# modelscope/FunASR

Hardware: AMD Instinct MI355X
Metric: audio-seconds/sec (RTF^-1) Paraformer-large 30s@bs64 (higher is better)
Workload: dtype f32 (GEMM / self-attention operands split into 2 fp16 planes, 3 fp16 MFMA products, f32 accumulate; all else f32)

## Files before the change

funasr_amd/_lib.py:

```python
from __future__ import annotations

import ctypes as C
import os
import subprocess
import threading

_HERE = os.path.dirname(os.path.abspath(__file__))
LIB_PATH = os.environ.get("PF_LIB_PATH") or os.path.join(_HERE, "libparaformer_hip.so")
CSRC_DIR = os.path.join(_HERE, "csrc")

ABI_VERSION = 5

_lock = threading.Lock()
_lib = None


class HipRuntimeError(RuntimeError):
    """A pf_* entry point returned a non-zero status."""


class pf_frontend_config(C.Structure):
    _fields_ = [
        ("sample_rate", C.c_int32), ("frame_length", C.c_int32), ("frame_shift", C.c_int32),
        ("n_mels", C.c_int32), ("lfr_m", C.c_int32), ("lfr_n", C.c_int32),
# ... 44 lines not shown
               [(n, C.c_double) for n in ("speech_2_noise_ratio", "snr_thres", "decibel_thres", "speech_noise_thres",
                                           "fe_prior_thres")]


class pf_campplus_config(C.Structure):
    _fields_ = [(n, C.c_int32) for n in ("feat_dim", "embedding_size", "growth_rate", "bn_size", "init_channels", "m_channels")] + \
               [("bn_eps", C.c_float)]


class pf_emotion2vec_config(C.Structure):
    _fields_ = [(n, C.c_int32) for n in ("embed_dim", "num_heads", "ffn_dim", "prenet_depth", "depth", "num_extra_tokens",
                                          "num_alibi_heads", "alibi_scale_layers", "alibi_scale_heads", "n_conv")] + \
               [("conv_kernel", C.c_int32 * 8), ("conv_stride", C.c_int32 * 8)] + \
               [(n, C.c_int32) for n in ("conv_pos_depth", "conv_pos_kernel", "conv_pos_groups", "vocab_size", "normalize", "precision")] + \
               [("norm_eps", C.c_float)]


class pf_conformer_config(C.Structure):
    _fields_ = [(n, C.c_int32) for n in ("input_dim", "d_model", "n_heads", "ffn_dim", "n_blocks", "kernel_size", "macaron", "legacy",
                                          "precision")] + [("ln_eps", C.c_float)]


class pf_tdecoder_config(C.Structure):
    _fields_ = [(n, C.c_int32) for n in ("vocab_size", "d_model", "n_heads", "ffn_dim", "n_blocks")] + [("ln_eps", C.c_float)]


class pf_stream_config(C.Structure):
    _fields_ = [(n, C.c_int32) for n in ("n_streams", "chunk_left", "chunk_cur", "chunk_right", "enc_look_back",
                                          "dec_look_back", "max_frames", "max_tokens", "use_graph")]


_vp, _i32, _i64, _f32 = C.c_void_p, C.c_int32, C.c_int64, C.c_float
_pi32 = C.POINTER(C.c_int32)

SIGNATURES = {
    "pf_last_error": (C.c_char_p, []),
    "pf_abi_version": (C.c_int, []),
    "pf_device_count": (C.c_int, []),
    "pf_set_concurrency_guard": (C.c_int, [_i32]),
    "pf_concurrency_guard": (C.c_int, []),
    "pf_frontend_create": (_vp, [C.POINTER(pf_frontend_config)]),
    "pf_frontend_destroy": (None, [_vp]),
    "pf_frontend_set_cmvn": (C.c_int, [_vp, _vp, _vp, _i32]),
    "pf_frontend_set_dither": (C.c_int, [_vp, _f32, C.c_uint64]),
    "pf_frontend_set_verify": (C.c_int, [_vp, _i32]),
    "pf_frontend_faults": (C.c_int, [_vp, C.POINTER(C.c_uint32)]),
    "pf_frontend_fault_log": (C.c_int, [_vp, C.POINTER(C.c_uint32)]),
    "pf_frontend_set_tables": (C.c_int, [_vp, _vp, _vp]),
    "pf_utterance_mvn": (C.c_int, [_vp, _vp, _i32, _i32, _i32, _i32, _i32, _f32, _vp]),
    "pf_global_mvn": (C.c_int, [_vp, _vp, _i32, _i32, _i32, _vp, _vp, _i32, _i32, _vp]),
    "pf_frontend_set_window": (C.c_int, [_vp, C.c_char_p, _f32]),
    "pf_frontend_set_snip_edges": (C.c_int, [_vp, _i32]),
    "pf_frontend_num_fbank_frames": (_i32, [_vp, _i64]),
    "pf_frontend_num_frames": (_i32, [_vp, _i64]),
    "pf_frontend_forward": (C.c_int, [_vp, _vp, _i64, _pi32, _i32, _vp, _i32, _pi32, _vp, _vp]),
    "pf_encoder_create": (_vp, [C.POINTER(pf_encoder_config)]),
    "pf_encoder_destroy": (None, [_vp]),
    "pf_encoder_set_tensor": (C.c_int, [_vp, C.c_char_p, _vp, _i64]),
    "pf_encoder_missing": (C.c_int, [_vp]),
    "pf_encoder_set_precision": (C.c_int, [_vp, _i32]),
    "pf_encoder_set_row_packing": (C.c_int, [_vp, _i32]),
    "pf_encoder_set_option": (C.c_int, [_vp, C.c_char_p, _i32]),
    "pf_encoder_debug_poison": (C.c_int, [_vp, _i32]),
    "pf_decoder_debug_poison": (C.c_int, [_vp, _i32]),
    "pf_predictor_debug_poison": (C.c_int, [_vp, _i32]),
    "pf_encoder_set_vad_mask": (C.c_int, [_vp, _vp, _i32]),
    "pf_encoder_forward": (C.c_int, [_vp, _vp, _pi32, _i32, _i32, _vp, _vp, _i32, _vp]),
    "pf_predictor_create": (_vp, [C.POINTER(pf_predictor_config)]),
    "pf_predictor_destroy": (None, [_vp]),
    "pf_predictor_set_tensor": (C.c_int, [_vp, C.c_char_p, _vp, _i64]),
    "pf_predictor_missing": (C.c_int, [_vp]),
    "pf_predictor_alphas": (C.c_int, [_vp, _vp, _pi32, _i32, _i32, _vp, _vp, _pi32, _vp]),
    "pf_predictor_embeds": (C.c_int, [_vp, _vp, _i32, _i32, _i32, _vp, _vp]),
    "pf_predictor_alphas_begin": (C.c_int, [_vp, _i32, _vp, _pi32, _i32, _i32, _vp, _vp, _vp, _vp]),
    "pf_predictor_embeds_slot": (C.c_int, [_vp, _i32, _vp, _i32, _i32, _i32, _vp, _vp]),
    "pf_predictor_create_v3": (_vp, [C.POINTER(pf_predictor_config), C.POINTER(pf_predictor_v3_config)]),
    "pf_predictor_timestamp": (C.c_int, [_vp, _vp, _pi32, _pi32, _i32, _i32, _vp, _vp, _vp]),
    "pf_decoder_create": (_vp, [C.POINTER(pf_decoder_config)]),
    "pf_decoder_destroy": (None, [_vp]),
    "pf_decoder_set_decoders2": (C.c_int, [_vp, _i32]),
    "pf_decoder_set_tensor": (C.c_int, [_vp, C.c_char_p, _vp, _i64]),
    "pf_decoder_missing": (C.c_int, [_vp]),
    "pf_decoder_set_precision": (C.c_int, [_vp, _i32]),
    "pf_decoder_forward": (C.c_int, [_vp, _vp, _pi32, _vp, _pi32, _i32, _i32, _i32, _vp, _vp, _vp, _vp]),
    "pf_decoder_create_contextual": (_vp, [C.POINTER(pf_decoder_config)]),
    "pf_decoder_forward_contextual": (C.c_int, [_vp, _vp, _pi32, _vp, _pi32, _vp, _i32, _f32, _i32, _i32, _i32, _vp, _vp, _vp, _vp]),
    "pf_decoder_asf_scores": (C.c_int, [_vp, _vp, _pi32, _vp, _pi32, _i32, _i32, _i32, _i32, _vp, _vp]),
    "pf_vad_create": (_vp, [C.POINTER(pf_vad_config)]),
    "pf_vad_destroy": (None, [_vp]),
    "pf_vad_set_tensor": (C.c_int, [_vp, C.c_char_p, _vp, _i64]),
    "pf_vad_missing": (C.c_int, [_vp]),
    "pf_vad_forward": (C.c_int, [_vp, _vp, _i32, _i32, _vp, _pi32, _i32, _vp, _vp, _i32, _vp]),
    "pf_vad_frame_decibel": (C.c_int, [_vp, _i64, _i32, _i32, _i32, _vp, _vp]),
    "pf_vad_decision_create": (_vp, [C.POINTER(pf_vad_options)]),
    "pf_vad_decision_destroy": (None, [_vp]),
    "pf_vad_decision_set_thresholds": (None, [_vp, C.c_double, C.c_double]),
    "pf_vad_decision_state": (C.c_int, [_vp]),
    "pf_vad_decision_push": (C.c_int, [_vp, _vp, _vp, _i32, _i32, _i32, _vp, _i32]),
    "pf_campplus_create": (_vp, [C.POINTER(pf_campplus_config)]),
    "pf_campplus_destroy": (None, [_vp]),
    "pf_campplus_set_tensor": (C.c_int, [_vp, C.c_char_p, _vp, _i64]),
    "pf_campplus_missing": (C.c_int, [_vp]),
    "pf_campplus_set_max_batch": (C.c_int, [_vp, _i32]),
    "pf_campplus_forward": (C.c_int, [_vp, _vp, _i32, _i32, _vp, _vp]),
    "pf_campplus_embed_chunks": (C.c_int, [_vp, _vp, _i64, C.POINTER(C.c_int64), _pi32, _i32, _i32, _vp, _vp]),
    "pf_emotion2vec_create": (_vp, [C.POINTER(pf_emotion2vec_config)]),
    "pf_emotion2vec_destroy": (None, [_vp]),
    "pf_emotion2vec_set_tensor": (C.c_int, [_vp, C.c_char_p, _vp, _i64]),
    "pf_emotion2vec_missing": (C.c_int, [_vp]),
    "pf_emotion2vec_set_label_mask": (C.c_int, [_vp, _pi32, _i32]),
    "pf_emotion2vec_set_max_samples": (C.c_int, [_vp, _i64]),
    "pf_emotion2vec_num_frames": (_i32, [_vp, _i64]),
    "pf_emotion2vec_forward": (C.c_int, [_vp, _vp, C.POINTER(C.c_int64), _i32, _vp, _vp, _vp, _vp]),
    "pf_conformer_create": (_vp, [C.POINTER(pf_conformer_config)]),
    "pf_conformer_destroy": (None, [_vp]),
    "pf_conformer_set_tensor": (C.c_int, [_vp, C.c_char_p, _vp, _i64]),
    "pf_conformer_missing": (C.c_int, [_vp]),
    "pf_conformer_set_precision": (C.c_int, [_vp, _i32]),
    "pf_conformer_num_frames": (_i32, [_vp, _i32, _i32]),
    "pf_conformer_forward": (C.c_int, [_vp, _vp, _pi32, _i32, _i32, _vp, _pi32, _vp]),
    "pf_tdecoder_create": (_vp, [C.POINTER(pf_tdecoder_config)]),
    "pf_tdecoder_destroy": (None, [_vp]),
    "pf_tdecoder_set_tensor": (C.c_int, [_vp, C.c_char_p, _vp, _i64]),
    "pf_tdecoder_missing": (C.c_int, [_vp]),
    "pf_tdecoder_begin": (C.c_int, [_vp, _vp, _i32, _i32, _i32, _vp]),
    "pf_tdecoder_step": (C.c_int, [_vp, _pi32, _i32, _i32, _vp, _vp]),
    "pf_tdecoder_reorder": (C.c_int, [_vp, _pi32, _i32, _vp]),
    "pf_k_relpos_attention": (C.c_int, [_vp, _vp, _vp, _vp, _vp, _i32, _i32, _i32, _i32, _vp, _vp]),
    "pf_k_conformer_glu_dw": (C.c_int, [_vp, _vp, _vp, _vp, _vp, _i32, _i32, _i32, _i32, _vp, _vp]),
    "pf_ctc_create": (_vp, [_i32, _i32]),
    "pf_ctc_destroy": (None, [_vp]),
    "pf_ctc_set_tensor": (C.c_int, [_vp, C.c_char_p, _vp, _i64]),
    "pf_ctc_missing": (C.c_int, [_vp]),
    "pf_ctc_greedy": (C.c_int, [_vp, _vp, _i32, _vp, _vp, _vp]),
    "pf_ctc_set_precision": (C.c_int, [_vp, _i32]),
    "pf_posterior_embed_create": (_vp, [_i32, _i32, _i32]),
    "pf_posterior_embed_destroy": (None, [_vp]),
    "pf_posterior_embed_set_tensor": (C.c_int, [_vp, C.c_char_p, _vp, _i64]),
    "pf_posterior_embed_missing": (C.c_int, [_vp]),
    "pf_posterior_embed_set_precision": (C.c_int, [_vp, _i32]),
    "pf_posterior_embed_set_chunk_rows": (C.c_int, [_vp, _i32]),
    "pf_posterior_embed_debug_poison": (C.c_int, [_vp, _i32]),
    "pf_posterior_embed_runs": (C.c_int, [_vp, _vp, _vp, _pi32, _i32, _i32, _pi32, _vp, _vp]),
    "pf_posterior_embed_embeds": (C.c_int, [_vp, _i32, _i32, _i32, _vp, _vp, _vp]),
    "pf_stream_create": (_vp, [_vp, _vp, _vp, C.POINTER(pf_stream_config)]),
    "pf_stream_destroy": (None, [_vp]),
    "pf_stream_set_pe": (C.c_int, [_vp, _vp, _i32]),
    "pf_stream_reset": (C.c_int, [_vp, _vp]),
    "pf_stream_set_option": (C.c_int, [_vp, C.c_char_p, _i32]),
    "pf_stream_step": (C.c_int, [_vp, _vp, _i32, _i32, _i32, _pi32, _pi32, _vp, _vp]),
    "pf_stream_step_begin": (C.c_int, [_vp, _vp, _i32, _i32, _i32, _vp, _vp]),
    "pf_stream_step_end": (C.c_int, [_vp, _pi32, _pi32]),
    "pf_stream_peek": (C.c_int, [_vp, _vp, _vp, _pi32]),
    "pf_frontend_fbank": (C.c_int, [_vp, _vp, _i64, _vp, _vp]),
    "pf_frontend_lfr_cmvn": (C.c_int, [_vp, _vp, _i32, _i32, _vp, _vp]),
    "pf_set_skinny_max_m": (C.c_int, [_i32]),
    "pf_measurement_build": (C.c_int, []),
    "pf_k_conv1d_gemm_f32": (C.c_int, [_vp, _vp, _vp, _vp, _i32, _i32, _i32, _i32, _i32, _i32, _i32, _vp, _vp]),
    "pf_k_gemm_f32": (C.c_int, [_vp, _i32, _vp, _i32, _vp, _vp, _i32, _vp, _i32, _vp, _i32, _i32, _i32, _i32, _i32, _vp]),
    "pf_k_gemm_bf16": (C.c_int, [_vp, _i32, _vp, _i32, _vp, _vp, _i32, _vp, _i32, _vp, _i32, _i32, _i32, _i32, _i32, _i32, _vp]),
    "pf_k_gemm_bf16_time": (C.c_int, [_vp, _i32, _vp, _i32, _vp, _vp, _i32, _i32, _i32, _i32, _i32, _i32, C.POINTER(C.c_float), _vp]),
    "pf_k_cast_bf16": (C.c_int, [_vp, _vp, _i64, _vp]),
    "pf_k_split3": (C.c_int, [_vp, _i32, _vp, _i32, _i64, _i32, _i32, _vp]),
    "pf_k_gemm_split3": (C.c_int, [_vp, _i32, _i64, _vp, _i32, _i64, _vp, _vp, _i32, _vp, _i32, _vp, _i32, _vp, _i32, _i64,
                                   _i32, _i32, _i32, _i32, _i32, C.POINTER(C.c_float), _vp]),
    "pf_k_split2": (C.c_int, [_vp, _i32, _vp, _i32, _i64, _i32, _i32, _f32, _vp]),
    "pf_k_gemm_f16x2": (C.c_int, [_vp, _i32, _i64, _vp, _i32, _i64, _f32, _vp, _vp, _i32, _vp, _i32, _vp, _i32, _vp, _i32, _i64,
                                  _f32, _i32, _i32, _i32, _i32, _i32, _i32, C.POINTER(C.c_float), _vp]),
    "pf_k_attention_f16x2": (C.c_int, [_vp, _i64, _vp, _i64, _vp, _i32, _i64, _vp, _i64, _vp, _i32, _i32, _i32, _i32, _f32, _f32,
                                       _i32, _i32, C.POINTER(C.c_float), _vp]),
    "pf_k_gemm_f16x2_row": (C.c_int, [_vp, _i32, _i64, _vp, _i32, _i64, _f32, _vp, _vp, _i32, _vp, _i32, _vp, _i32, _vp, _vp, _f32,
                                      _vp, _i64, _f32, _vp, _i32, _i32, _i32, _i32, _i32, C.POINTER(C.c_float), _vp]),
    "pf_k_gemm_skinny_ln": (C.c_int, [_vp, _i32, _vp, _i32, _vp, _vp, _i32, _vp, _i32, _i32, _i32, _i32, _i32, _vp, _vp, _vp, _vp, _f32, _vp, _vp, _vp, _vp]),
    "pf_k_ln_consts": (C.c_int, [_vp, _i32, _i32, _i32, _vp, _vp, _vp, _vp, _vp]),
    "pf_k_ffn_f16x2": (C.c_int, [_vp, _vp, _vp, _vp, _vp, _f32, _f32, _f32, _vp, _vp, _vp, _vp, _f32, _vp, _f32, _vp, _i32, _i32, _i32,
                                 C.POINTER(C.c_float), _vp]),
    "pf_k_gemm_f16x2_row_fsmn": (C.c_int, [_vp, _i32, _i64, _vp, _i32, _i64, _f32, _vp, _vp, _i32, _vp, _vp, _vp, _vp, _i32, _vp, _i32,
                                           _vp, _vp, _f32, _vp, _i64, _f32, _vp, _i32, _i32, _i32, _i32, C.POINTER(C.c_float), _vp]),
    "pf_k_layernorm_planes": (C.c_int, [_vp, _i32, _vp, _vp, _vp, _i32, _i64, _f32, _i32, _i32, _f32, _i32, C.POINTER(C.c_float), _vp]),
    "pf_k_gemm_f16x2_qkv": (C.c_int, [_vp, _i32, _i64, _vp, _i32, _i64, _f32, _vp, _i32, _i32, _i32, _i32, _vp, _vp, _i64, _vp, _vp,
                                      _i32, _i64, _f32, _f32, _f32, _i32, _i32, C.POINTER(C.c_float), _vp]),
    "pf_k_gemm_f16x2_argmax": (C.c_int, [_vp, _i32, _i64, _vp, _i32, _i64, _f32, _vp, _i32, _i32, _i32, _vp, _vp, _vp, _vp]),
    "pf_k_gemm_argmax_f32": (C.c_int, [_vp, _i32, _vp, _i32, _vp, _i32, _i32, _i32, _vp, _vp, _vp, _vp]),
    "pf_k_log_softmax": (C.c_int, [_vp, _i32, _vp, _i32, _i32, _i32, _vp]),
    "pf_k_layernorm": (C.c_int, [_vp, _i32, _vp, _vp, _vp, _i32, _i32, _i32, _i32, _f32, _vp]),
    "pf_k_fsmn": (C.c_int, [_vp, _i32, _vp, _vp, _i32, _vp, _i32, _vp, _i32, _i32, _i32, _i32, _i32, _vp]),
    "pf_k_attention_f32": (C.c_int, [_vp, _i32, _vp, _i32, _vp, _i32, _vp, _i32, _vp, _i32, _i32, _i32, _i32, _f32, _vp]),
    "pf_k_attention_f32_two_source": (C.c_int, [_vp, _i32, _vp, _i32, _vp, _i32, _vp, _i32, _vp, _i32, _vp, _i32, _vp, _i32,
                                                _i32, _i32, _i32, _i32, _i32, _i32, _f32, _vp]),
    "pf_k_attention_small": (C.c_int, [_vp, _i32, _vp, _i32, _vp, _i32, _vp, _i32, _vp, _i32, _i32, _i32, _i32, _i32, _f32, _vp]),
    "pf_k_gather_rows": (C.c_int, [_vp, _i32, _i32, _vp, _vp, _i32, _i32, _vp]),
    "pf_k_attention_split3": (C.c_int, [_vp, _i32, _vp, _i32, _vp, _i32, _vp, _i32, _vp, _i32, _i32, _i32, _i32, _f32, _vp]),
    "pf_k_attention_bf16": (C.c_int, [_vp, _i32, _vp, _i32, _vp, _i32, _vp, _i32, _vp, _i32, _i32, _i32, _i32, _f32, _vp]),
    "pf_k_lstm": (C.c_int, [_vp, _vp, _vp, _vp, _vp, _i32, _i32, _i32, _i32, _i32, _vp, _vp]),
    "pf_k_cif": (C.c_int, [_vp, _vp, _i32, _i32, _i32, _i32, _vp, _vp, _vp, _vp]),
    "pf_k_cif_tail": (C.c_int, [_vp, _vp, _vp, _i32, _i32, _i32, _i32, _f32, _i32, _i32, _vp, _vp, _vp, _vp, _vp, _vp]),
    "pf_k_ctc_runs": (C.c_int, [_vp, _pi32, _i32, _i32, _i32, _vp, _vp, _i32, _vp]),
    "pf_k_argmax_rows": (C.c_int, [_vp, _i32, _i32, _i32, _vp, _vp]),
    "pf_k_gemm_f32_time": (C.c_int, [_vp, _i32, _vp, _i32, _vp, _vp, _i32, _i32, _i32, _i32, _i32, C.POINTER(C.c_float), _vp]),
    "pf_dp_unique_id": (C.c_int, [_vp, _i32]),
    "pf_dp_create": (_vp, [_vp, _i32, _i32, _i32]),
    "pf_dp_destroy": (C.c_int, [_vp]),
    "pf_dp_world": (C.c_int, [_vp]),
    "pf_dp_rank": (C.c_int, [_vp]),
    "pf_dp_broadcast_encoder": (C.c_int, [_vp, _vp, _i32, _vp]),
    "pf_dp_broadcast_predictor": (C.c_int, [_vp, _vp, _i32, _vp]),
    "pf_dp_broadcast_decoder": (C.c_int, [_vp, _vp, _i32, _vp]),
    "pf_dp_broadcast_ctc": (C.c_int, [_vp, _vp, _i32, _vp]),
    "pf_paraformer_create": (_vp, [_vp, _vp, _vp]),
    "pf_paraformer_destroy": (None, [_vp]),
    "pf_paraformer_forward": (C.c_int, [_vp, _vp, _vp, _i32, _i32, _vp, _vp, _i32, _vp, _vp, _vp, _vp]),
    "pf_paraformer_begin": (C.c_int, [_vp, _vp, _vp, _i32, _i32, _vp, _vp]),
    "pf_paraformer_finish": (C.c_int, [_vp, _i32, _vp, _i32, _vp, _vp, _vp, _vp]),
    "pf_paraformer_encoder_out": (_vp, [_vp]),
    "pf_paraformer_embeds": (_vp, [_vp]),
    "pf_dp_gather_ids": (C.c_int, [_vp, _vp, _i64, _vp, _i32, _vp]),
    "pf_dp_broadcast_raw": (C.c_int, [_vp, _vp, _i64, _i32, _vp]),
    "pf_prof_enable": (C.c_int, [C.c_int]),
    "pf_prof_reset": (C.c_int, []),
    "pf_prof_read": (C.c_int, [C.c_int, C.POINTER(C.c_double), C.POINTER(C.c_double), C.POINTER(C.c_int64)]),
    "pf_prof_read_tags": (C.c_int, [C.c_int, C.POINTER(C.c_char_p), C.POINTER(C.c_int), C.POINTER(C.c_double), C.POINTER(C.c_double),
                                    C.POINTER(C.c_int64)]),
}


def build(verbose: bool = False) -> str:
    cmd = ["make", "-C", CSRC_DIR, "-j8"]
    res = subprocess.run(cmd, stdout=subprocess.PIPE, stderr=subprocess.STDOUT, text=True)
    if verbose:
        print(res.stdout)
    if res.returncode != 0:
        raise RuntimeError("building libparaformer_hip.so failed:\n" + res.stdout)
    return LIB_PATH


def load():
    global _lib
    with _lock:
        if _lib is not None:
            return _lib
        if not os.path.exists(LIB_PATH):
            raise ImportError(
                f"{LIB_PATH} not found: the HIP extension is the only implementation of this package. "
                f"Build it with `make -C {CSRC_DIR}` (or `python -c 'import __graft_entry__ as g; g.build()'`)."
            )
        lib = C.CDLL(LIB_PATH)
        for name, (res, args) in SIGNATURES.items():
            fn = getattr(lib, name)
            fn.restype = res
            fn.argtypes = args
        if lib.pf_abi_version() != ABI_VERSION:
            raise ImportError(f"{LIB_PATH} reports ABI version {lib.pf_abi_version()}, this package binds version {ABI_VERSION}: "
                              f"rebuild it (`make -C {CSRC_DIR}`)")
        _lib = lib
        return lib


def last_error() -> str:
    msg = load().pf_last_error()
    return msg.decode("utf-8", "replace") if msg else ""


def check(status: int, what: str) -> None:
    if status != 0:
        raise HipRuntimeError(f"{what} failed with status {status}: {last_error()}")


def check_handle(handle, what: str):
# ... 4 lines not shown
```

funasr_amd/csrc/common.h:

```cpp
#pragma once
#include <hip/hip_runtime.h>
#include <stdint.h>
#include <stdio.h>
#include <string>
#include <atomic>

typedef float floatx16 __attribute__((ext_vector_type(16)));
typedef float floatx4 __attribute__((ext_vector_type(4)));

namespace pf {

inline int current_device_slot() {
    int d = 0;
    if (hipGetDevice(&d) != hipSuccess || d < 0) d = 0;
    return d & 63;
}
struct PerDeviceOnce {
    std::atomic<bool> flag[64];
    PerDeviceOnce() { for (auto& f : flag) f.store(false, std::memory_order_relaxed); }
    bool done() const { return flag[current_device_slot()].load(std::memory_order_acquire); }
    void mark() { flag[current_device_slot()].store(true, std::memory_order_release); }
};
inline int device_cu_count() {
    static std::atomic<int> n[64];
// ... 234 lines not shown
    const float* ln_g; const float* ln_b; float ln_eps; float* ln_y; int ln_ldy; int ln_out; size_t ln_plane; float ln_oscale;
    int kslices;
};
int gemm_f16x2_argmax_parts(int M, int N);
int launch_gemm_f16x2(const Gemm2Args& a, hipStream_t stream);
bool gemm_f16x2_w4_ok(const Gemm2Args& a);
int launch_gemm_f16x2_w4(const Gemm2Args& a, int abl, hipStream_t stream);
bool gemm_f16x2_ps_ok(const Gemm2Args& a);
int launch_gemm_f16x2_ps(const Gemm2Args& a, hipStream_t stream);
struct GemmRowArgs;
bool gemm_f16x2_w4_row_ok(const GemmRowArgs& a);
int launch_gemm_f16x2_w4_row(const GemmRowArgs& a, hipStream_t stream);
struct GemmRowArgs {
    const unsigned short* A; int lda; size_t a_plane;
    const unsigned short* W; int ldw; size_t w_plane;
    float oscale; const float* oscale_dev;
    const float* bias;
    const float* R1; int ldr1;
    const float* R2; int ldr2;
    float* C; int ldc;
    const float* ln_g; const float* ln_b; float ln_eps;
    unsigned short* Y2; int ldy2; size_t y_plane; float yscale;
    float* Yf; int ldyf;
    int M, N, K;
    int relu;
    int a_nt;
    const float* fs_v; int ldfv; const float* fs_w; const int* fs_lo; const int* fs_hi;
    int block_rows;
};
struct FfnArgs {
    const unsigned short* X2; int ldx; size_t x_plane;
    const unsigned short* W1; int ldw1; size_t w1_plane;
    const unsigned short* W2; int ldw2; size_t w2_plane;
    const float* b1; const float* b2;
    float oscale1, hscale, oscale2;
    const float* R; int ldr;
    float* C; int ldc;
    const float* ln_g; const float* ln_b; float ln_eps;
    unsigned short* Y2; int ldy2; size_t y_plane; float yscale;
    float* Yf; int ldyf;
    int M, D, F;
    int abl;
    size_t x_kstep, w1_kstep, w2_kstep;
};
bool ffn_f16x2_applicable(int D, int F);
int launch_ffn_f16x2(const FfnArgs& a, hipStream_t stream);
int launch_gemm_f16x2_row8(const GemmRowArgs& a, int bm, hipStream_t stream);
bool gemm_f16x2_row_applicable(int N, int K);
int launch_gemm_f16x2_row(const GemmRowArgs& a, hipStream_t stream);
int launch_split2(const float* x, int ldx, unsigned short* y, int ldy, size_t plane, int M, int N, float scale,
                  hipStream_t stream, const float* scale_dev = nullptr, int seq_out = 0, int seq_in = 0);
int launch_kv_scales(const float* amax_dev, const float* l1_bmax_dev, int n_layers, float* out, hipStream_t stream);
int launch_pow2_scale(const float* amax_dev, float* sc, hipStream_t stream);
int launch_absmax(const float* x, size_t n, float* out_dev, hipStream_t stream);
int launch_rowl1_bound(const float* W, int rows, int cols, int ld, const float* bias, float in_bound, float* out_dev,
                       hipStream_t stream);

int launch_splitk_reduce_ln(const float* part, int slices, size_t slice_stride, int M, int D, const float* bias, int relu, const float* R1, int ldr1,
                            const float* R2, int ldr2, float* C, int ldc, const float* gamma, const float* beta, float eps, float* y, int ldy, int out_mode,
                            size_t plane, float oscale, hipStream_t stream);
int launch_layernorm(const float* x, int ldx, const float* gamma, const float* beta, float* y, int ldy,
                     int M, int D, int Dpad, float eps, hipStream_t stream, int out_mode = 0, int in_bf16 = 0,
                     size_t plane = 0, float oscale = 1.f, int seq_out = 0, int seq_in = 0, const int* out_map = nullptr);

int launch_scale_cols(float* x, int ld, int M, int N, float sc, hipStream_t stream);
int launch_log_softmax(const float* x, int ldx, float* y, int ldy, int M, int N, hipStream_t stream);
int launch_scale_add_pe(const float* x, const float* pe, float* y, int B, int T, int D, float scale,
                        hipStream_t stream, int Tp = 0);
int launch_scale_add_pe_rows(const float* x, const float* pe, float* y, const int* map, int M, int T, int D, float scale,
                             hipStream_t stream);

struct FsmnArgs {
    const float* in;  int ldin;
    const float* w;
    const float* R;   int ldr;
    float* out;       int ldo;
    const int* lens;
    int B, T, C, K, left_pad;
    int in_bf16;
    const int* offs;
};
int launch_fsmn(const FsmnArgs& a, hipStream_t stream);

struct AttnArgs {
    const float* Q; int ldq;
    const float* K; int ldk;
    const float* V; int ldv;
    float* O;       int ldo;
    const int* klens;
    int B, H, Tq, Tk;
    float scale;
    const float* K2; int ldk2;
    const float* V2; int ldv2;
    int T2, n2;
    const int* n1_dev; int n1_stride;
    unsigned short* O3; size_t o_plane;
    int few_q;
    int app_rows, app_r0; const int* app_wp; int app_wp_stride; const int* app_gate;
    int app_mod;
    int mask_mode; const int* vad_pos;
    const float* fs_in; int fs_ldin; const float* fs_w; float* fs_out; int fs_ldo; int fs_T;
    unsigned short* O2; int ldo2; size_t o2_plane; float o2_scale;
};
inline bool attention_takes_fewq(const AttnArgs& a) { return a.few_q && a.Tq <= 32 && !a.O3; }
inline bool attention_fuses_append(const AttnArgs& a) {
    return a.few_q && a.Tq <= 16 && !a.O3 && a.K2 && a.app_rows > 0 && (a.app_rows < a.Tk ? a.app_rows : a.Tk) <= 16;
}
int launch_attention_f32(const AttnArgs& a, hipStream_t stream);
int launch_attention_bf16(const AttnArgs& a, hipStream_t stream);
int launch_attention_split3(const AttnArgs& a, hipStream_t stream);
struct Attn2Args {
    const unsigned short* Q; int ldq; size_t q_plane;
    const unsigned short* K; int ldk; size_t k_plane;
    const unsigned short* VT; int ldvt; size_t vt_plane;
    unsigned short* O; int ldo; size_t o_plane;
    const int* klens;
    int B, H, Tp;
    int Tq;
    float sscale;
    const float* sscale_dev;
    float oscale;
    int variant;
    const int* qoffs;
    int xcd_nqb;
    const int* koffs;
};
int launch_attention_f16x2(const Attn2Args& a, hipStream_t stream);

int launch_asf_scores(const float* Q, int ldq, const float* K, int ldk, float* P_scratch, float* out, int H, int dk, int N, int T,
                      int klen, float scale, hipStream_t stream);
bool attention_small_applicable(const AttnArgs& a, int dk);
int launch_attention_small(const AttnArgs& a, int dk, hipStream_t stream);
int launch_scatter_i32(const int* in, const int* map, int* out, int n, hipStream_t stream);
int launch_gather_rows(const float* table, int ld, int rows, const int* ids, float* out, int n, int D, hipStream_t stream);

int launch_vad_fsmn(const float* x, int ldx, const float* w, const float* cache_in, float* cache_out, float* y, int ldy,
                    int B, int T, int C, int L, int S, hipStream_t stream);
int launch_vad_softmax_sil(const float* x, int ldx, int M, int N, const int* ids, int n_ids, float* p_sil, float* probs,
                           int ldp, hipStream_t stream);
int launch_frame_decibel(const float* wav, int n_frames, int flen, int shift, float* out, hipStream_t stream);

}
```

funasr_amd/csrc/engine_decoder.hip:

```cpp
#include "engine_internal.h"

namespace pf {

std::string dec_layer_prefix(bool contextual, int n_blocks, int i) {
    return (contextual && i == n_blocks - 1) ? std::string("last_decoder.") : "decoders." + std::to_string(i) + ".";
}


static int decoder_resolve(Decoder* d) {
    if (d->tt.require_all("decoder")) return -3;
    d->layers.clear();
    for (int i = 0; i < d->cfg.n_blocks; ++i) {
        const std::string p = dec_layer_prefix(d->contextual, d->cfg.n_blocks, i);
        DecLayerW w;
        w.n1g = d->tt.get(p + "norm1.weight"); w.n1b = d->tt.get(p + "norm1.bias");
        w.w1 = d->tt.get(p + "feed_forward.w_1.weight"); w.b1 = d->tt.get(p + "feed_forward.w_1.bias");
        w.fng = d->tt.get(p + "feed_forward.norm.weight"); w.fnb = d->tt.get(p + "feed_forward.norm.bias");
        w.w2 = d->tt.get(p + "feed_forward.w_2.weight");
        w.n2g = d->tt.get(p + "norm2.weight"); w.n2b = d->tt.get(p + "norm2.bias");
        w.fsmn_w = d->tt.get(p + "self_attn.fsmn_block.weight");
        w.n3g = d->tt.get(p + "norm3.weight"); w.n3b = d->tt.get(p + "norm3.bias");
        w.q_w = d->tt.get(p + "src_attn.linear_q.weight"); w.q_b = d->tt.get(p + "src_attn.linear_q.bias");
        w.kv_w = d->tt.get(p + "src_attn.linear_k_v.weight"); w.kv_b = d->tt.get(p + "src_attn.linear_k_v.bias");
        w.o_w = d->tt.get(p + "src_attn.linear_out.weight"); w.o_b = d->tt.get(p + "src_attn.linear_out.bias");
// ... 584 lines not shown
    for (int i = 0; i < c.n_blocks; ++i) {
        const std::string p = dec_layer_prefix(contextual, c.n_blocks, i);
        add_ffn(p);
        rc |= d->tt.add(p + "norm2.weight", D);
        rc |= d->tt.add(p + "norm2.bias", D);
        rc |= d->tt.add(p + "self_attn.fsmn_block.weight", (int64_t)D * c.kernel_size);
        rc |= d->tt.add(p + "norm3.weight", D);
        rc |= d->tt.add(p + "norm3.bias", D);
        rc |= d->tt.add(p + "src_attn.linear_q.weight", (int64_t)D * D);
        rc |= d->tt.add(p + "src_attn.linear_q.bias", D);
        rc |= d->tt.add(p + "src_attn.linear_k_v.weight", (int64_t)2 * D * D);
        rc |= d->tt.add(p + "src_attn.linear_k_v.bias", 2 * D);
        rc |= d->tt.add(p + "src_attn.linear_out.weight", (int64_t)D * D);
        rc |= d->tt.add(p + "src_attn.linear_out.bias", D);
    }
    if (contextual) {
        rc |= d->tt.add("bias_decoder.norm3.weight", D);
        rc |= d->tt.add("bias_decoder.norm3.bias", D);
        rc |= d->tt.add("bias_decoder.src_attn.linear_q.weight", (int64_t)D * D);
        rc |= d->tt.add("bias_decoder.src_attn.linear_q.bias", D);
        rc |= d->tt.add("bias_decoder.src_attn.linear_k_v.weight", (int64_t)2 * D * D);
        rc |= d->tt.add("bias_decoder.src_attn.linear_k_v.bias", 2 * D);
        rc |= d->tt.add("bias_decoder.src_attn.linear_out.weight", (int64_t)D * D);
        rc |= d->tt.add("bias_decoder.src_attn.linear_out.bias", D);
        rc |= d->tt.add("bias_output.weight", (int64_t)D * 2 * D);
    }
    add_ffn("decoders3.0.");
    rc |= d->tt.add("after_norm.weight", D);
    rc |= d->tt.add("after_norm.bias", D);
    if (c.vocab_size > 0) {
        rc |= d->tt.add("output_layer.weight", (int64_t)c.vocab_size * D);
        rc |= d->tt.add("output_layer.bias", c.vocab_size);
    }
    if (rc) return nullptr;
    return reinterpret_cast<pf_decoder*>(d.release());
}
void pf_decoder_destroy(pf_decoder* d) { delete reinterpret_cast<Decoder*>(d); }
int pf_decoder_set_decoders2(pf_decoder* dh, int32_t n_layers) {
    Decoder* d = reinterpret_cast<Decoder*>(dh);
    PF_REQUIRE(d && n_layers >= 0 && n_layers <= 64, "decoder_set_decoders2: null handle or layer count out of range");
    PF_REQUIRE(d->n_blocks2 == 0 || d->n_blocks2 == n_layers, "decoder_set_decoders2: already set");
    if (d->n_blocks2 == n_layers) return 0;
    const int D = d->cfg.d_model, F = d->cfg.ffn_dim;
    int rc = 0;
    for (int i = 0; i < n_layers; ++i) {
        const std::string p = "decoders2." + std::to_string(i) + ".";
        rc |= d->tt.add(p + "norm1.weight", D);
        rc |= d->tt.add(p + "norm1.bias", D);
        rc |= d->tt.add(p + "feed_forward.w_1.weight", (int64_t)F * D);
        rc |= d->tt.add(p + "feed_forward.w_1.bias", F);
        rc |= d->tt.add(p + "feed_forward.norm.weight", F);
        rc |= d->tt.add(p + "feed_forward.norm.bias", F);
        rc |= d->tt.add(p + "feed_forward.w_2.weight", (int64_t)D * F);
        rc |= d->tt.add(p + "norm2.weight", D);
        rc |= d->tt.add(p + "norm2.bias", D);
        rc |= d->tt.add(p + "self_attn.fsmn_block.weight", (int64_t)D * d->cfg.kernel_size);
    }
    if (rc) return -2;
    d->n_blocks2 = n_layers;
    ++d->tt.version;
    return 0;
}
int pf_decoder_set_tensor(pf_decoder* dh, const char* name, const float* data, int64_t numel) {
    Decoder* d = reinterpret_cast<Decoder*>(dh);
    PF_REQUIRE(d && name && data, "decoder_set_tensor: null");
    return d->tt.set(name, data, numel);
}
int pf_decoder_set_precision(pf_decoder* dh, int32_t mode) {
    Decoder* d = reinterpret_cast<Decoder*>(dh);
    PF_REQUIRE(d && mode >= 0 && mode <= 3, "decoder_set_precision: mode must be 0 (fp32 MFMA), 1 (bf16 operands), 2 (fp32 via bf16x3) or 3 (fp32 via f16x2)");
    PF_REQUIRE(mode == 0 || d->cfg.d_model / d->cfg.n_heads == 128, "decoder_set_precision: heads of d_k <= 64 exist in the fp32 mode only (attention_small.hip)");
    d->precision = mode;
    return 0;
}
int pf_decoder_missing(const pf_decoder* dh) {
    const Decoder* d = reinterpret_cast<const Decoder*>(dh);
    return d ? d->tt.missing() : -1;
}

static int decoder_forward_impl(Decoder* d, const float* memory, const int32_t* mem_lens, const float* embeds,
                                const int32_t* tok_lens, int32_t B, int32_t T, int32_t N, float* logits, int32_t* ids,
                                float* hidden_out, hipStream_t s, int asf_layer, float* asf_scores, const DecCtxArgs* cx = nullptr);

int pf_decoder_forward(pf_decoder* dh, const float* memory, const int32_t* mem_lens, const float* embeds,
                       const int32_t* tok_lens, int32_t B, int32_t T, int32_t N, float* logits, int32_t* ids,
                       float* hidden_out, void* stream) {
    return decoder_forward_impl(reinterpret_cast<Decoder*>(dh), memory, mem_lens, embeds, tok_lens, B, T, N, logits, ids,
                                hidden_out, reinterpret_cast<hipStream_t>(stream), -1, nullptr);
}
int pf_decoder_asf_scores(pf_decoder* dh, const float* memory, const int32_t* mem_lens, const float* embeds,
                          const int32_t* tok_lens, int32_t B, int32_t T, int32_t N, int32_t n_blocks_before,
                          float* scores_dev, void* stream) {
    Decoder* d = reinterpret_cast<Decoder*>(dh);
    PF_REQUIRE(d && scores_dev && n_blocks_before >= 0 && n_blocks_before < d->cfg.n_blocks, "decoder_asf_scores: bad block index");
    return decoder_forward_impl(d, memory, mem_lens, embeds, tok_lens, B, T, N, nullptr, nullptr, nullptr,
                                reinterpret_cast<hipStream_t>(stream), n_blocks_before, scores_dev);
}

int pf_decoder_forward_contextual(pf_decoder* dh, const float* memory, const int32_t* mem_lens, const float* embeds,
                                  const int32_t* tok_lens, const float* contextual_dev, int32_t n_hot, float clas_scale,
                                  int32_t B, int32_t T, int32_t N, float* logits, int32_t* ids, float* hidden_out, void* stream) {
    Decoder* d = reinterpret_cast<Decoder*>(dh);
    PF_REQUIRE(d && d->contextual && contextual_dev && n_hot >= 1, "decoder_forward_contextual: needs a contextual decoder and >= 1 hotword row");
    DecCtxArgs cx{contextual_dev, n_hot, clas_scale};
    return decoder_forward_impl(d, memory, mem_lens, embeds, tok_lens, B, T, N, logits, ids, hidden_out,
                                reinterpret_cast<hipStream_t>(stream), -1, nullptr, &cx);
}

static int decoder_forward_impl(Decoder* d, const float* memory, const int32_t* mem_lens, const float* embeds,
                                const int32_t* tok_lens, int32_t B, int32_t T, int32_t N, float* logits, int32_t* ids,
                                float* hidden_out, hipStream_t s, int asf_layer, float* asf_scores, const DecCtxArgs* cx) {
    PF_REQUIRE(d && memory && mem_lens && embeds && tok_lens && B > 0 && T > 0 && N > 0, "decoder_forward: null/empty");
    for (int b = 0; b < B; ++b) {
        PF_REQUIRE(mem_lens[b] >= 1 && mem_lens[b] <= T, "decoder_forward: memory lens out of range");
        PF_REQUIRE(tok_lens[b] >= 0 && tok_lens[b] <= N, "decoder_forward: token lens out of range");
    }
    PF_REQUIRE(d->precision == 0 || d->cfg.d_model / d->cfg.n_heads == 128, "decoder_forward: heads of d_k <= 64 exist in the fp32 mode only");
    int rc;
    if ((rc = decoder_prepare(d, d->precision == 3 && asf_layer < 0 && !cx, s))) return rc;
    const pf_decoder_config& c = d->cfg;
    const int D = c.d_model, F = c.ffn_dim, V = c.vocab_size;
    int Mq = B * N;
    const int Mq_pad = B * N, Mk = B * T;
    if (d->x.ensure(sizeof(float) * (size_t)Mq * D) || d->t1.ensure(sizeof(float) * (size_t)Mq * D) ||
        d->t2.ensure(sizeof(float) * (size_t)Mq * D) || d->ffn.ensure(sizeof(float) * (size_t)Mq * F) ||
        d->ffn2.ensure(sizeof(float) * (size_t)Mq * F) || d->q.ensure(sizeof(float) * (size_t)Mq * D) ||
        d->kv.ensure(sizeof(float) * (size_t)Mk * 2 * D) || d->ctx.ensure(sizeof(float) * (size_t)Mq * D) ||
        d->hid.ensure(sizeof(float) * (size_t)Mq * D))
        return -2;
    if ((rc = upload_lens(d->mem_lens, mem_lens, B, s))) return rc;
    if ((rc = upload_lens(d->tok_lens, tok_lens, B, s))) return rc;
    float* x = d->x.as<float>();
    float* t1 = d->t1.as<float>();
    float* t2 = d->t2.as<float>();
    const bool may_pack = d->precision == 3 && asf_layer < 0 && !cx && ids && !logits && !hidden_out && V > 0;
    if (!may_pack) PF_HIP_TRY(hipMemcpyAsync(x, embeds, sizeof(float) * (size_t)Mq * D, hipMemcpyDeviceToDevice, s));
    const int left_pad = (c.kernel_size - 1) / 2 + (c.sanm_shift > 0 ? c.sanm_shift : 0);
    if (V == 0 && asf_layer < 0) PF_REQUIRE(!logits && !ids && hidden_out && d->precision != 1,
                           "decoder_forward: a decoder without output layer returns hidden states only (fp32 / bf16x3)");
    if (d->precision == 1 && !logits && asf_layer < 0 && !cx) return decoder_forward_bf16(d, memory, B, T, N, ids, hidden_out, s);
    PF_REQUIRE(d->contextual == (cx != nullptr) || asf_layer >= 0, "decoder_forward: a contextual decoder runs through pf_decoder_forward_contextual");
    const bool x3 = d->precision == 2 && asf_layer < 0 && !cx;
    const bool x2 = d->precision == 3 && asf_layer < 0 && !cx;
    const int Tp = round_up(T, 16), Mkp = B * Tp;
    double mem_rows = 0, tok_mem = 0;
    for (int b = 0; b < B; ++b) { mem_rows += mem_lens[b]; tok_mem += (double)mem_lens[b] * tok_lens[b]; }
    const unsigned short* mem3 = nullptr;
    const unsigned short* mem2 = nullptr;
    float* dsc = nullptr;
    if (x2) {
        const size_t cap_k = d->k2.cap, cap_v = d->vt2.cap;
        if (d->t16.ensure(sizeof(unsigned short) * 2 * (size_t)Mq * D) || d->ffn16.ensure(sizeof(unsigned short) * 2 * (size_t)Mq * F) ||
            d->q16.ensure(sizeof(unsigned short) * 2 * (size_t)Mq * D) || d->ctx16.ensure(sizeof(unsigned short) * 2 * (size_t)Mq * D) ||
            d->mem16.ensure(sizeof(unsigned short) * 2 * (size_t)Mkp * D) || d->dsc.ensure(sizeof(float) * 4) ||
            d->k2.ensure(sizeof(unsigned short) * 2 * ((size_t)Mkp + 32) * D) || d->vt2.ensure(sizeof(unsigned short) * 2 * D * ((size_t)Mkp + 64)) ||
            d->dscl.ensure(sizeof(float) * 4 * c.n_blocks))
            return -2;
        if (d->k2.cap != cap_k) PF_HIP_TRY(hipMemsetAsync(d->k2.p, 0, d->k2.cap, s));
        if (d->vt2.cap != cap_v) PF_HIP_TRY(hipMemsetAsync(d->vt2.p, 0, d->vt2.cap, s));
        dsc = d->dsc.as<float>();
        if ((rc = launch_absmax(memory, (size_t)Mk * D, dsc, s))) return rc;
        if ((rc = launch_pow2_scale(dsc, dsc + 1, s))) return rc;
        if ((rc = launch_kv_scales(dsc, d->dlb.as<float>(), c.n_blocks, d->dscl.as<float>(), s))) return rc;
        if ((rc = launch_split2(memory, D, d->mem16.as<unsigned short>(), D, (size_t)Mkp * D, Mkp, D, 1.f, s, dsc + 1, Tp, T))) return rc;
        mem2 = d->mem16.as<unsigned short>();
    }
    bool pack = false;
    const int* offs_dev = nullptr;
    if (may_pack) {
        int total = 0;
        d->h_offs.assign((size_t)B + 1, 0);
        for (int b = 0; b < B; ++b) { d->h_offs[b] = total; total += tok_lens[b]; }
        d->h_offs[B] = total;
        if (total > 0 && total < Mq_pad) {
            d->h_map.resize((size_t)total);
            for (int b = 0; b < B; ++b) for (int t = 0; t < tok_lens[b]; ++t) d->h_map[(size_t)d->h_offs[b] + t] = b * N + t;
            if (d->offs_dev.ensure(sizeof(int32_t) * ((size_t)B + 1)) || d->map_dev.ensure(sizeof(int32_t) * (size_t)Mq_pad) ||
                d->ids_packed.ensure(sizeof(int32_t) * (size_t)Mq_pad)) return -2;
            if (upload_h2d(d->offs_dev.p, d->h_offs.data(), sizeof(int32_t) * ((size_t)B + 1), s) ||
                upload_h2d(d->map_dev.p, d->h_map.data(), sizeof(int32_t) * (size_t)total, s)) return -2;
            if ((rc = launch_gather_rows(embeds, D, Mq_pad, d->map_dev.as<int>(), x, total, D, s))) return rc;
            pack = true; offs_dev = d->offs_dev.as<int>(); Mq = total;
        }
    }
    if (may_pack && !pack) PF_HIP_TRY(hipMemcpyAsync(x, embeds, sizeof(float) * (size_t)Mq * D, hipMemcpyDeviceToDevice, s));
    if (x3) {
        if (d->t16.ensure(sizeof(unsigned short) * 3 * (size_t)Mq * D) || d->mem16.ensure(sizeof(unsigned short) * 3 * (size_t)Mk * D))
            return -2;
        if ((rc = launch_split3(memory, D, d->mem16.as<unsigned short>(), D, (size_t)Mk * D, Mk, D, s))) return rc;
        mem3 = d->mem16.as<unsigned short>();
    }
    auto w3 = [&](const std::string& name, int rows, int cols) { return x3 ? d->tt.get_split3(name, rows, cols, s) : nullptr; };
    for (int l = 0; l < c.n_blocks; ++l) {
        const DecLayerW& w = d->layers[l];
        const std::string lp = dec_layer_prefix(d->contextual, c.n_blocks, l);
        const unsigned short* w1_3 = w3(lp + "feed_forward.w_1.weight", F, D);
        if (x3 && !w1_3) return -2;
        if (x2) rc = dec_ffn_x2(d, w, x, t2, Mq, s);
        else rc = dec_ffn(d, w, x, t2, Mq, s, w1_3);
        if (rc) return rc;
        if ((rc = layernorm(t2, D, w.n2g, w.n2b, t1, D, Mq, D, D, c.ln_eps, s))) return rc;
        FsmnArgs fa{};
        fa.in = t1; fa.ldin = D; fa.w = w.fsmn_w; fa.R = x; fa.ldr = D; fa.out = x; fa.ldo = D;
        fa.lens = d->tok_lens.as<int>(); fa.B = B; fa.T = N; fa.C = D; fa.K = c.kernel_size; fa.left_pad = left_pad;
        fa.offs = offs_dev;
        if ((rc = fsmn(fa, s))) return rc;
        if (x2) {
            unsigned short* t2p = d->t16.as<unsigned short>();
            {
                ProfScope ps(PROF_LN, 8.0 * Mq * (double)D, s);
                if ((rc = launch_layernorm(x, D, w.n3g, w.n3b, reinterpret_cast<float*>(t2p), D, Mq, D, D, c.ln_eps, s, 3, 0,
                                           (size_t)Mq * D, pow2f(w.e_n3)))) return rc;
            }
            Gemm2Args g{};
            g.A = t2p; g.lda = D; g.a_plane = (size_t)Mq * D; g.W = w.q_2; g.ldw = D; g.w_plane = (size_t)D * D;
            g.oscale = pow2f(-(w.e_n3 + w.ew_q)); g.bias = w.q_b; g.C2 = d->q16.as<unsigned short>(); g.ldc2 = D;
            g.c_plane = (size_t)Mq * D; g.cscale = powf((float)(D / c.n_heads), -0.5f) * pow2f(w.e_q);
            g.M = Mq; g.N = D; g.K = D;
            ProfScope ps(PROF_GEMM3, 2.0 * Mq * (double)D * D, s);
            if ((rc = launch_gemm_f16x2(g, s))) return rc;
        } else {
            if ((rc = layernorm(x, D, w.n3g, w.n3b, t1, D, Mq, D, D, c.ln_eps, s))) return rc;
            if ((rc = gemm_simple(t1, D, w.q_w, D, w.q_b, d->q.as<float>(), D, Mq, D, D, 0, nullptr, 0, nullptr, 0, s)))
                return rc;
        }
        if (x2) {
            const float* lsc = d->dscl.as<float>() + 4 * l;
            unsigned short* k2 = d->k2.as<unsigned short>();
            unsigned short* vt2 = d->vt2.as<unsigned short>();
            {
                Gemm2Args g{};
                g.A = mem2; g.lda = D; g.a_plane = (size_t)Mkp * D; g.W = w.kv_2; g.ldw = D; g.w_plane = (size_t)2 * D * D;
                g.oscale = pow2f(-w.ew_kv); g.oscale_dev = dsc + 2; g.bias = w.kv_b; g.M = Mkp; g.N = 2 * D; g.K = D;
                g.qkv_D = D; g.kv_form = 1; g.Kp = k2; g.qk_plane = ((size_t)Mkp + 32) * D; g.VT = vt2; g.ldvt = Mkp + 64;
                g.vt_plane = (size_t)D * (Mkp + 64); g.k_mul = 1.f; g.v_mul = 1.f; g.kv_mul_dev = lsc;
                ProfScope ps(PROF_GEMM3, 2.0 * mem_rows * 2.0 * D * D, s);
                if ((rc = launch_gemm_f16x2(g, s))) return rc;
            }
            {
                Attn2Args aa{};
                aa.Q = d->q16.as<unsigned short>(); aa.ldq = D; aa.q_plane = (size_t)Mq * D;
                aa.K = k2; aa.ldk = D; aa.k_plane = ((size_t)Mkp + 32) * D; aa.VT = vt2; aa.ldvt = Mkp + 64;
                aa.vt_plane = (size_t)D * (Mkp + 64); aa.O = d->ctx16.as<unsigned short>(); aa.ldo = D; aa.o_plane = (size_t)Mq * D;
                aa.klens = d->mem_lens.as<int>(); aa.B = B; aa.H = c.n_heads; aa.Tp = Tp; aa.Tq = N; aa.qoffs = offs_dev;
                aa.sscale = pow2f(-w.e_q); aa.sscale_dev = lsc + 2; aa.oscale = pow2f(-10);
                aa.variant = 3;
                ProfScope ps(PROF_ATTN, 4.0 * tok_mem * D, s);
                if ((rc = launch_attention_f16x2(aa, s))) return rc;
            }
            if ((rc = gemm2_simple(d->ctx16.as<unsigned short>(), D, Mq, 0, w.o_2, w.ew_o, w.o_b, x, D, D, D, 0, x, D, s, lsc + 3)))
                return rc;
            continue;
        } else if (x3) {
            if ((rc = gemm3_simple(mem3, D, Mk, w3(lp + "src_attn.linear_k_v.weight", 2 * D, D), w.kv_b, d->kv.as<float>(),
                                   2 * D, 2 * D, D, 0, s))) return rc;
        } else if ((rc = gemm_simple(memory, D, w.kv_w, D, w.kv_b, d->kv.as<float>(), 2 * D, Mk, 2 * D, D, 0, nullptr, 0,
                                     nullptr, 0, s))) return rc;
        const bool ctx_block = cx && l == c.n_blocks - 1;
        if (ctx_block) {
            if (d->xself.ensure(sizeof(float) * (size_t)Mq * D) || d->xcat.ensure(sizeof(float) * (size_t)Mq * 2 * D)) return -2;
            PF_HIP_TRY(hipMemcpyAsync(d->xself.p, x, sizeof(float) * (size_t)Mq * D, hipMemcpyDeviceToDevice, s));
        }
        if (l == asf_layer) {
            if (d->asf_p.ensure(sizeof(float) * (size_t)c.n_heads * N * T)) return -2;
            return launch_asf_scores(d->q.as<float>(), D, d->kv.as<float>(), 2 * D, d->asf_p.as<float>(), asf_scores, c.n_heads,
                                     D / c.n_heads, N, T, mem_lens[0], powf((float)(D / c.n_heads), -0.5f), s);
        }
        AttnArgs aa{};
        aa.Q = d->q.as<float>(); aa.ldq = D; aa.K = d->kv.as<float>(); aa.ldk = 2 * D;
        aa.V = d->kv.as<float>() + D; aa.ldv = 2 * D; aa.O = d->ctx.as<float>(); aa.ldo = D;
        aa.klens = d->mem_lens.as<int>(); aa.B = B; aa.H = c.n_heads; aa.Tq = N; aa.Tk = T;
        aa.scale = powf((float)(D / c.n_heads), -0.5f);
        if ((rc = attention(aa, 4.0 * B * (double)N * T * D, s, false, D / c.n_heads))) return rc;
        if (ctx_block) {
            float* xcat = d->xcat.as<float>();
            const float* xs = d->xself.as<float>();
            if ((rc = gemm_simple(d->ctx.as<float>(), D, w.o_w, D, w.o_b, xcat, 2 * D, Mq, D, D, 0, nullptr, 0, nullptr, 0, s)))
                return rc;
            const int Mh = B * cx->n_hot;
            if (d->kv.ensure(sizeof(float) * (size_t)(Mh > Mk ? Mh : Mk) * 2 * D)) return -2;
            std::vector<int32_t> hl((size_t)B, cx->n_hot);
            if ((rc = upload_lens(d->ctx_lens, hl.data(), B, s))) return rc;
            PF_HIP_TRY(hipStreamSynchronize(s));
            if ((rc = layernorm(xs, D, d->tt.get("bias_decoder.norm3.weight"), d->tt.get("bias_decoder.norm3.bias"), t1, D, Mq, D, D,
                                c.ln_eps, s))) return rc;
            if ((rc = gemm_simple(t1, D, d->tt.get("bias_decoder.src_attn.linear_q.weight"), D,
                                  d->tt.get("bias_decoder.src_attn.linear_q.bias"), d->q.as<float>(), D, Mq, D, D, 0, nullptr, 0, nullptr, 0, s))) return rc;
            if ((rc = gemm_simple(cx->info, D, d->tt.get("bias_decoder.src_attn.linear_k_v.weight"), D,
                                  d->tt.get("bias_decoder.src_attn.linear_k_v.bias"), d->kv.as<float>(), 2 * D, Mh, 2 * D, D, 0, nullptr, 0,
                                  nullptr, 0, s))) return rc;
            AttnArgs ab{};
            ab.Q = d->q.as<float>(); ab.ldq = D; ab.K = d->kv.as<float>(); ab.ldk = 2 * D; ab.V = d->kv.as<float>() + D; ab.ldv = 2 * D;
// ... 127 lines not shown
```

funasr_amd/csrc/engine_internal.h:

```cpp
#pragma once
#include <math.h>
#include <string.h>

#include <cmath>
#include <map>
#include <memory>
#include <mutex>
#include <string>
#include <vector>

#include "../../include/paraformer_hip.h"
#include "cif.h"
#include "lstm.h"
#include "common.h"
#include "frontend.h"
#include "stream.h"
#include "engine_tables.h"


namespace pf {

void set_error(const std::string& msg);
const char* get_error();

// ... 352 lines not shown
    DevBuf fs_grp;
    std::vector<int32_t> h_fs;
    const int* cur_fs = nullptr; int cur_fs_groups = 0;
    int attn_variant = 3;
    int row_nt = 1;
    double prof_rows = 0, prof_sq = 0;
    int gemm_tile = 0;
};


static inline int exp_for_bound(float bound) {
    if (!(bound > 0.f)) return 15;
    int e = (int)floorf(log2f(32768.f / bound));
    return e > 15 ? 15 : e;
}
static inline float pow2f(int e) { return ldexpf(1.f, e); }

static inline bool encoder_w2_row_form(const Encoder* e, int M) {
    if (e->w2_row != 2) return e->w2_row == 1;
    const int n_cu = device_cu_count();
    const int blocks = ceil_div(M, 256) * (e->cfg.d_model / 256), rounds = ceil_div(blocks, n_cu);
    return !(e->cfg.d_model % 256 == 0 && blocks >= (int)(0.65 * rounds * n_cu));
}

void note_concurrent_streams();

struct EncChunkCtx {
    float* ring; int cap; const StreamDev* st; int append_rows;
    const int* lens;
    int mod = 0;
    bool x2 = false;
    float* ln_stats = nullptr;
    bool ln_in_ready = false;
    const float* ln_c_qkv = nullptr;
    const float* ln_c_w1 = nullptr;
    const EncLayerW* x2_out_next = nullptr;
    bool x2_in_ready = false;
    int x2_short_k = 0;
    bool x2_fold = false;
    bool x2_attn_planes = false;
    bool fsmn_rides = false;
    const EncLayerW* next = nullptr;
};

struct Predictor {
    pf_predictor_config cfg;
    TensorTable tt;
    DevBuf col, conv, zero_row;
    struct CifState { DevBuf lens, alphas, peaks, rems, flags, nfires, curs, ntok; int B = 0, T = 0; } st[2];
    bool v3 = false;
    pf_predictor_v3_config c3{};
    DevBuf up, x_tm, pre, lstm_out, h_a, h_b, cell, tok_dev, ulens, pack, ts_lens;
    unsigned long long packed_for = TensorTable::NOT_PREPARED;
    std::vector<int32_t> ul_host;
};

int predictor_alphas_enqueue(Predictor* p, int slot, const float* hidden, const int32_t* lens_host, int B, int T, hipStream_t s);
const int32_t* predictor_counts_dev(Predictor* p, int slot);
const float* predictor_alphas_dev(Predictor* p, int slot);
const float* predictor_peaks_dev(Predictor* p, int slot);
int predictor_embeds_slot(Predictor* p, int slot, const float* hidden, int B, int T, int N, float* embeds, hipStream_t s);

struct DecLayerW {
    const float *n1g, *n1b, *w1, *b1, *fng, *fnb, *w2, *n2g, *n2b, *fsmn_w, *n3g, *n3b, *q_w, *q_b, *kv_w, *kv_b,
        *o_w, *o_b;
    const unsigned short *w1_2 = nullptr, *w2_2 = nullptr, *q_2 = nullptr, *kv_2 = nullptr, *o_2 = nullptr;
    int ew_1 = 0, ew_2 = 0, ew_q = 0, ew_kv = 0, ew_o = 0, e_n1 = 0, e_fn = 0, e_n3 = 0, e_q = 0;
    float kv_l1b[4] = {0.f, 0.f, 0.f, 0.f};
};


struct Decoder {
    pf_decoder_config cfg;
    bool contextual = false;
    DevBuf xself, xcat, ctx_lens;
    TensorTable tt;
    std::vector<DecLayerW> layers;
    int n_blocks2 = 0;
    std::vector<DecLayerW> layers2;
    DecLayerW last;
    unsigned long long resolved_for = TensorTable::NOT_PREPARED, x2_for = TensorTable::NOT_PREPARED;
    DevBuf x, t1, t2, ffn, ffn2, q, kv, ctx, mem_lens, tok_lens, pval, pidx, hid;
    int precision = 0;
    DevBuf t16, ffn16, ffn2_16, q16, kv16, ctx16, mem16, hid16;
    DevBuf dsc;
    DevBuf dscl, dlb;
    DevBuf k2, vt2;
    DevBuf splitk;
    int e_an = 0;
    DevBuf asf_p;
    DevBuf offs_dev, map_dev, ids_packed;
    std::vector<int32_t> h_offs, h_map;
};


struct Ctc {
    int d_model, vocab;
    TensorTable tt;
    DevBuf pval, pidx;
    int precision = 0;
    DevBuf h2, dsc;
};

struct Stream {
    Encoder* e = nullptr; Predictor* p = nullptr; Decoder* d = nullptr;
    pf_stream_config cfg{};
    int S = 1, keep = 5, Wmax = 0, Nmax = 0, enc_cap = 0, dec_cap = 0, pe_rows = 0;
    int enc_mod = 0;
    DevBuf dev_state, cache_feats, feats_in, win, enc_ring, dec_ring, dec_fsmn, cif_hidden, cif_alpha, dec_valid, dec_wp,
        n_fired, pe, lensW, enc_out, embeds, ids, alphas;
    int32_t* h_ids = nullptr; int32_t* h_n = nullptr;
    hipStream_t stream = nullptr;
    hipEvent_t ev = nullptr;
    int start_idx = 0;
    std::map<int, hipGraphExec_t> graphs;
    std::map<int, int> seen;
    unsigned long long graph_epoch = 0;
    bool use_graph = true;
    bool x2 = false;
    int ln_carry = 2;
    bool fsmn_rides = true;
    DevBuf ln_stats;
    bool pending = false; int pending_rows = 0;
    bool wide_k = false;
    DevBuf ws_part, ws_count;
    DevBuf ln_consts;
    unsigned long long ln_ver_e = TensorTable::NOT_PREPARED, ln_ver_d = TensorTable::NOT_PREPARED;
    DevBuf dec_ln_a, dec_ln_b, dec_ln_f;
    int short_k = 3;
    bool ln_folded = true;
    DevBuf kvcat_w, kvcat_b, kvcat_2;
    int kvcat_e = 0;
    bool kv_batched = true;
    unsigned long long ver_e = TensorTable::NOT_PREPARED, ver_d = TensorTable::NOT_PREPARED;
    int e_mem = 0;
    std::vector<int> e_ctx;
    DevBuf mem2;
    ~Stream() {
        for (auto& kv : graphs) (void)hipGraphExecDestroy(kv.second);
        if (h_ids) (void)hipHostFree(h_ids);
        if (h_n) (void)hipHostFree(h_n);
        if (ev) (void)hipEventDestroy(ev);
        if (stream) (void)hipStreamDestroy(stream);
    }
};

struct Vad {
    pf_vad_config cfg;
    TensorTable tt;
    DevBuf a, b, c, cache_tmp, ids;
    size_t zeroed_for = 0;
};
static inline int vad_pad(int k) { return round_up(k, 32); }
struct LstmW { const float* w_ih[2]; const float* w_hh; const float* b_ih; const float* b_hh; };
struct DecCtxArgs { const float* info; int n_hot; float clas_scale; };

int check_device();
int upload_h2d(void* dst, const void* src, size_t bytes, hipStream_t s);
int upload_lens(DevBuf& buf, const int32_t* host, int B, hipStream_t s);
int gemm(const GemmArgs& a, hipStream_t s);
int gemm_simple(const float* A, int lda, const float* W, int ldw, const float* bias, float* C, int ldc,
                       int M, int N, int K, int relu, const float* R1, int ldr1, const float* R2, int ldr2,
                       hipStream_t s);
int layernorm(const float* x, int ldx, const float* g, const float* b, float* y, int ldy, int M, int D,
                     int Dpad, float eps, hipStream_t s);
int fsmn(const FsmnArgs& a, hipStream_t s);
// ... 48 lines not shown
```

funasr_amd/csrc/engine_kernels.hip:

```cpp
#include "engine_internal.h"

using namespace pf;

extern "C" {

int pf_k_gemm_skinny_ln(const float* A, int32_t lda, const float* W, int32_t ldw, const float* bias, const float* R2, int32_t ldr2,
                        float* Cout, int32_t ldc, int32_t M, int32_t N, int32_t K, int32_t relu, float* stats_out,
                        const float* stats_in, const float* ln_g, const float* ln_c, float ln_eps, const float* out_gamma, float* ws_part,
                        int32_t* ws_count, void* stream) {
    GemmArgs g{};
    g.ws_part = ws_part; g.ws_count = ws_count; g.ln_c1 = ln_c; g.ln_c2 = ln_c ? ln_c + N : nullptr; g.out_gamma = out_gamma;
    g.A = A; g.lda = lda; g.W = W; g.ldw = ldw; g.bias = bias; g.R2 = R2; g.ldr2 = ldr2; g.C = Cout; g.ldc = ldc;
    g.M = M; g.N = N; g.K = K; g.relu = relu; g.ln_stats_out = stats_out; g.ln_stats_in = stats_in; g.ln_g = ln_g; g.ln_eps = ln_eps;
    PF_REQUIRE(gemm_skinny_applicable(g), "gemm_skinny_ln: K % 16");
    return launch_gemm_skinny(g, reinterpret_cast<hipStream_t>(stream));
}
int pf_k_ln_consts(const float* W, int32_t ldw, int32_t N, int32_t K, const float* gamma, const float* beta, const float* bias, float* c,
                   void* stream) {
    return launch_ln_consts(W, ldw, N, K, gamma, beta, bias, c, c + N, reinterpret_cast<hipStream_t>(stream));
}
int pf_set_skinny_max_m(int32_t m) { g_skinny_max_m = m; return 0; }

int pf_k_gemm_f32(const float* A, int32_t lda, const float* W, int32_t ldw, const float* bias, const float* R1,
                  int32_t ldr1, const float* R2, int32_t ldr2, float* C, int32_t ldc, int32_t M, int32_t N, int32_t K,
// ... 191 lines not shown
    set_error("pf_k_ffn_f16x2: the one-launch feed-forward is in the measurement library only (make -C funasr_amd/csrc measure)");
    return -1;
}
#endif
int pf_k_gemm_f16x2_row_fsmn(const void* A2, int32_t lda, int64_t a_plane, const void* W2, int32_t ldw, int64_t w_plane, float oscale,
                             const float* bias, const float* fs_v, int32_t ldfv, const float* fs_w, const int32_t* fs_lo,
                             const int32_t* fs_hi, const float* R2, int32_t ldr2, float* C, int32_t ldc, const float* ln_g,
                             const float* ln_b, float ln_eps, void* Y2, int64_t y_plane, float yscale, float* Yf, int32_t M, int32_t K,
                             int32_t a_nt, int32_t iters, float* ms_out, void* stream) {
    hipStream_t s = reinterpret_cast<hipStream_t>(stream);
    GemmRowArgs g{};
    g.A = reinterpret_cast<const unsigned short*>(A2); g.lda = lda; g.a_plane = (size_t)a_plane;
    g.W = reinterpret_cast<const unsigned short*>(W2); g.ldw = ldw; g.w_plane = (size_t)w_plane; g.oscale = oscale;
    g.bias = bias; g.fs_v = fs_v; g.ldfv = ldfv; g.fs_w = fs_w; g.fs_lo = fs_lo; g.fs_hi = fs_hi; g.R2 = R2; g.ldr2 = ldr2;
    g.C = C; g.ldc = ldc; g.ln_g = ln_g; g.ln_b = ln_b; g.ln_eps = ln_eps; g.Y2 = reinterpret_cast<unsigned short*>(Y2); g.ldy2 = 512;
    g.y_plane = (size_t)y_plane; g.yscale = yscale; g.Yf = Yf; g.ldyf = 512; g.M = M; g.N = 512; g.K = K;
    g.a_nt = a_nt & 3; g.block_rows = a_nt >> 8;
    if (iters <= 0 || !ms_out) return launch_gemm_f16x2_row(g, s);
    return time_launches([&] { return launch_gemm_f16x2_row(g, s); }, iters, ms_out, s);
}
int pf_k_layernorm_planes(const float* x, int32_t ldx, const float* gamma, const float* beta, void* y2, int32_t ldy, int64_t plane,
                          float scale, int32_t M, int32_t D, float eps, int32_t iters, float* ms_out, void* stream) {
    hipStream_t s = reinterpret_cast<hipStream_t>(stream);
    auto fn = [&] { return launch_layernorm(x, ldx, gamma, beta, reinterpret_cast<float*>(y2), ldy, M, D, ldy, eps, s, 3, 0, (size_t)plane, scale); };
    if (iters <= 0 || !ms_out) return fn();
    return time_launches(fn, iters, ms_out, s);
}
int pf_k_gemm_f16x2_qkv(const void* A2, int32_t lda, int64_t a_plane, const void* W2, int32_t ldw, int64_t w_plane, float oscale,
                        const float* bias, int32_t M, int32_t D, int32_t K, int32_t kv_form, void* Qp, void* Kp, int64_t qk_plane,
                        float* Vf, void* VT, int32_t ldvt, int64_t vt_plane, float q_mul, float k_mul, float v_mul, int32_t tile,
                        int32_t iters, float* ms_out, void* stream) {
    hipStream_t s = reinterpret_cast<hipStream_t>(stream);
    Gemm2Args g{};
    g.A = reinterpret_cast<const unsigned short*>(A2); g.lda = lda; g.a_plane = (size_t)a_plane;
    g.W = reinterpret_cast<const unsigned short*>(W2); g.ldw = ldw; g.w_plane = (size_t)w_plane; g.oscale = oscale; g.bias = bias;
    g.C = Vf; g.ldc = D; g.M = M; g.N = (kv_form ? 2 : 3) * D; g.K = K; g.qkv_D = D; g.kv_form = kv_form;
    g.Qp = reinterpret_cast<unsigned short*>(Qp); g.Kp = reinterpret_cast<unsigned short*>(Kp); g.qk_plane = (size_t)qk_plane;
    g.VT = reinterpret_cast<unsigned short*>(VT); g.ldvt = ldvt; g.vt_plane = (size_t)vt_plane;
    g.q_mul = q_mul; g.k_mul = k_mul; g.v_mul = v_mul; g.tile = tile;
    if (iters <= 0 || !ms_out) return launch_gemm_f16x2(g, s);
    return time_launches([&] { return launch_gemm_f16x2(g, s); }, iters, ms_out, s);
}
int pf_k_gemm_f16x2_argmax(const void* A2, int32_t lda, int64_t a_plane, const void* W2, int32_t ldw, int64_t w_plane, float oscale,
                           const float* bias, int32_t M, int32_t N, int32_t K, int32_t* ids, float* sval, int32_t* sidx,
                           void* stream) {
    hipStream_t s = reinterpret_cast<hipStream_t>(stream);
    PF_REQUIRE(ids && sval && sidx, "gemm_f16x2_argmax: scratch required");
    Gemm2Args g{};
    g.A = reinterpret_cast<const unsigned short*>(A2); g.lda = lda; g.a_plane = (size_t)a_plane;
    g.W = reinterpret_cast<const unsigned short*>(W2); g.ldw = ldw; g.w_plane = (size_t)w_plane; g.oscale = oscale; g.bias = bias;
    g.M = M; g.N = N; g.K = K; g.amax_val = sval; g.amax_idx = sidx; g.amax_ld = gemm_f16x2_argmax_parts(M, N);
    int rc;
    if ((rc = launch_gemm_f16x2(g, s))) return rc;
    return launch_argmax_reduce(sval, sidx, g.amax_ld, g.amax_ld, ids, nullptr, M, s);
}
int pf_k_cast_bf16(const float* x, void* y, int64_t n, void* stream) {
    return launch_cast_bf16(x, reinterpret_cast<unsigned short*>(y), (size_t)n, reinterpret_cast<hipStream_t>(stream));
}
int pf_k_gemm_argmax_f32(const float* A, int32_t lda, const float* W, int32_t ldw, const float* bias, int32_t M,
                         int32_t N, int32_t K, int32_t* ids, float* sval, int32_t* sidx, void* stream) {
    hipStream_t s = reinterpret_cast<hipStream_t>(stream);
    PF_REQUIRE(ids && sval && sidx, "gemm_argmax: scratch [M, 2*ceil(N/128)] required");
    const int nparts = 2 * ceil_div(N, 128);
    GemmArgs g{};
    g.A = A; g.lda = lda; g.W = W; g.ldw = ldw; g.bias = bias; g.M = M; g.N = N; g.K = K;
    g.amax_val = sval; g.amax_idx = sidx; g.amax_ld = nparts;
    int rc;
    if ((rc = gemm(g, s))) return rc;
    return launch_argmax_reduce(sval, sidx, nparts, nparts, ids, nullptr, M, s);
}
int pf_k_log_softmax(const float* x, int32_t ldx, float* y, int32_t ldy, int32_t M, int32_t N, void* stream) {
    return launch_log_softmax(x, ldx, y, ldy, M, N, reinterpret_cast<hipStream_t>(stream));
}
int pf_k_layernorm(const float* x, int32_t ldx, const float* gamma, const float* beta, float* y, int32_t ldy,
                   int32_t M, int32_t D, int32_t Dpad, float eps, void* stream) {
    return layernorm(x, ldx, gamma, beta, y, ldy, M, D, Dpad, eps, reinterpret_cast<hipStream_t>(stream));
}
int pf_k_fsmn(const float* in, int32_t ldin, const float* w, const float* R, int32_t ldr, float* out, int32_t ldo,
              const int32_t* lens_dev, int32_t B, int32_t T, int32_t C, int32_t K, int32_t left_pad, void* stream) {
    FsmnArgs fa{};
    fa.in = in; fa.ldin = ldin; fa.w = w; fa.R = R; fa.ldr = ldr; fa.out = out; fa.ldo = ldo; fa.lens = lens_dev;
    fa.B = B; fa.T = T; fa.C = C; fa.K = K; fa.left_pad = left_pad;
    return fsmn(fa, reinterpret_cast<hipStream_t>(stream));
}
int pf_k_attention_f32(const float* Q, int32_t ldq, const float* K, int32_t ldk, const float* V, int32_t ldv,
                       float* O, int32_t ldo, const int32_t* klens_dev, int32_t B, int32_t H, int32_t Tq, int32_t Tk,
                       float scale, void* stream) {
    AttnArgs aa{};
    aa.Q = Q; aa.ldq = ldq; aa.K = K; aa.ldk = ldk; aa.V = V; aa.ldv = ldv; aa.O = O; aa.ldo = ldo;
    aa.klens = klens_dev; aa.B = B; aa.H = H; aa.Tq = Tq; aa.Tk = Tk; aa.scale = scale;
    return attention(aa, 4.0 * B * (double)Tq * Tk * H * 128, reinterpret_cast<hipStream_t>(stream));
}
int pf_k_attention_f32_two_source(const float* Q, int32_t ldq, const float* K, int32_t ldk, const float* V, int32_t ldv,
                                  const float* K2, int32_t ldk2, const float* V2, int32_t ldv2, float* O, int32_t ldo,
                                  const int32_t* n1_dev, int32_t n1_stride, int32_t B, int32_t H, int32_t Tq, int32_t Tk,
                                  int32_t T2, int32_t n2, float scale, void* stream) {
    PF_REQUIRE(K2 && V2 && n1_dev && n2 > 0 && n2 <= T2 && ldk2 % 4 == 0 && ldv2 % 4 == 0, "attention_two_source: bad second source");
    AttnArgs aa{};
    aa.Q = Q; aa.ldq = ldq; aa.K = K; aa.ldk = ldk; aa.V = V; aa.ldv = ldv; aa.O = O; aa.ldo = ldo;
    aa.K2 = K2; aa.ldk2 = ldk2; aa.V2 = V2; aa.ldv2 = ldv2; aa.T2 = T2; aa.n2 = n2; aa.n1_dev = n1_dev; aa.n1_stride = n1_stride;
    aa.B = B; aa.H = H; aa.Tq = Tq; aa.Tk = Tk; aa.scale = scale;
    return attention(aa, 4.0 * B * (double)Tq * (Tk + n2) * H * 128, reinterpret_cast<hipStream_t>(stream));
}
int pf_k_attention_split3(const float* Q, int32_t ldq, const float* K, int32_t ldk, const float* V, int32_t ldv, float* O,
                          int32_t ldo, const int32_t* klens_dev, int32_t B, int32_t H, int32_t Tq, int32_t Tk, float scale,
                          void* stream) {
    AttnArgs aa{};
    aa.Q = Q; aa.ldq = ldq; aa.K = K; aa.ldk = ldk; aa.V = V; aa.ldv = ldv; aa.O = O; aa.ldo = ldo; aa.klens = klens_dev;
    aa.B = B; aa.H = H; aa.Tq = Tq; aa.Tk = Tk; aa.scale = scale;
    return launch_attention_split3(aa, reinterpret_cast<hipStream_t>(stream));
}
int pf_k_attention_small(const float* Q, int32_t ldq, const float* K, int32_t ldk, const float* V, int32_t ldv, float* O,
                         int32_t ldo, const int32_t* klens_dev, int32_t B, int32_t H, int32_t d_k, int32_t Tq, int32_t Tk,
                         float scale, void* stream) {
    AttnArgs aa{};
    aa.Q = Q; aa.ldq = ldq; aa.K = K; aa.ldk = ldk; aa.V = V; aa.ldv = ldv; aa.O = O; aa.ldo = ldo; aa.klens = klens_dev;
    aa.B = B; aa.H = H; aa.Tq = Tq; aa.Tk = Tk; aa.scale = scale;
    return launch_attention_small(aa, d_k, reinterpret_cast<hipStream_t>(stream));
}
int pf_k_gather_rows(const float* table, int32_t ld, int32_t rows, const int32_t* ids_dev, float* out, int32_t n, int32_t D,
                     void* stream) {
    PF_REQUIRE(table && ids_dev && out, "gather_rows: null");
    return launch_gather_rows(table, ld, rows, ids_dev, out, n, D, reinterpret_cast<hipStream_t>(stream));
}
int pf_k_lstm(const float* x, const float* w_ih, const float* w_hh, const float* b_ih, const float* b_hh, int32_t B, int32_t T,
              int32_t D, int32_t H, int32_t ndir, float* out, void* stream) {
    hipStream_t s = reinterpret_cast<hipStream_t>(stream);
    PF_REQUIRE(x && w_ih && w_hh && b_ih && b_hh && out && B > 0 && T > 0 && D > 0 && H > 0 && (ndir == 1 || ndir == 2),
               "k_lstm: null/empty argument");
    if (check_device()) return -2;
    DevBuf x_tm, pre, h_a, h_b, cell;
    if (x_tm.ensure(sizeof(float) * (size_t)B * T * D)) return -2;
    int rc;
    if ((rc = launch_rows_bt_to_tb(x, x_tm.as<float>(), B, T, D, s))) return rc;
    LstmW w{};
    w.w_ih[0] = w_ih; w.w_ih[1] = w_ih + (size_t)4 * H * D; w.w_hh = w_hh; w.b_ih = b_ih; w.b_hh = b_hh;
    if ((rc = lstm_forward(w, x_tm.as<float>(), T, B, D, H, ndir, out, 0, pre, h_a, h_b, cell, s))) return rc;
    PF_HIP_TRY(hipStreamSynchronize(s));
    return 0;
}
int pf_k_attention_bf16(const void* Q, int32_t ldq, const void* K, int32_t ldk, const void* V, int32_t ldv, void* O,
                        int32_t ldo, const int32_t* klens_dev, int32_t B, int32_t H, int32_t Tq, int32_t Tk, float scale,
                        void* stream) {
    AttnArgs aa{};
    aa.Q = reinterpret_cast<const float*>(Q); aa.ldq = ldq; aa.K = reinterpret_cast<const float*>(K); aa.ldk = ldk;
    aa.V = reinterpret_cast<const float*>(V); aa.ldv = ldv; aa.O = reinterpret_cast<float*>(O); aa.ldo = ldo;
    aa.klens = klens_dev; aa.B = B; aa.H = H; aa.Tq = Tq; aa.Tk = Tk; aa.scale = scale;
    return launch_attention_bf16(aa, reinterpret_cast<hipStream_t>(stream));
}
int pf_k_cif(const float* alphas, const float* hidden, int32_t B, int32_t T, int32_t D, int32_t N, float* peaks,
             int32_t* n_fires, float* embeds, void* stream) {
    hipStream_t s = reinterpret_cast<hipStream_t>(stream);
    PF_REQUIRE(alphas && hidden && peaks && n_fires && embeds && B > 0 && T > 0 && D > 0, "k_cif: null/empty");
    static DevBuf al, pk, rm, ff, ln;
    const int Te = T + 1;
    if (al.ensure(sizeof(float) * (size_t)B * Te) || pk.ensure(sizeof(float) * (size_t)B * Te) ||
        rm.ensure(sizeof(float) * (size_t)B * Te) || ff.ensure(sizeof(int) * (size_t)B * Te) ||
        ln.ensure(sizeof(int) * (size_t)B)) return -2;
    std::vector<int> lens(B, T);
    if (upload_h2d(ln.p, lens.data(), sizeof(int) * B, s)) return -2;
    PF_HIP_TRY(hipMemcpy2DAsync(al.p, sizeof(float) * Te, alphas, sizeof(float) * T, sizeof(float) * T, B,
                                hipMemcpyDeviceToDevice, s));
    CifScanArgs sa{};
    sa.alphas = al.as<float>(); sa.peaks = pk.as<float>(); sa.rems = rm.as<float>(); sa.fire_flag = ff.as<int>();
    sa.n_fires = n_fires; sa.lens = ln.as<int>(); sa.B = B; sa.T = T; sa.tail_threshold = 0.f; sa.tail_mask = 1;
    int rc;
// ... 73 lines not shown
```

funasr_amd/csrc/gemm_f16x2.hip:

```cpp
#include "common.h"
#include <cstdlib>
#include <type_traits>
#include "gemm_f16x2_epilogue.h"

namespace pf {

namespace {

typedef _Float16 f16x8 __attribute__((ext_vector_type(8)));

template <int WM, int WN, int WGM = 4, int KS_ = 32> struct Geo2 {
    static constexpr int NW = WGM * 2;
    static constexpr int BM = WGM * WM * 32, BN = 2 * WN * 32;
    static constexpr int KS = KS_, ROWB = 2 * KS, CPR = ROWB / 16, RPP = 1024 / ROWB;
    static constexpr int SWZ = CPR == 4 ? 2 : 3;
    static constexpr int A_PLANE_B = BM * ROWB, B_PLANE_B = BN * ROWB;
    static constexpr int STAGE_B = 2 * (A_PLANE_B + B_PLANE_B);
    static constexpr int NSTG = KS == 16 ? (WGM == 4 ? (163840 / STAGE_B > 6 ? 6 : 163840 / STAGE_B) : 3) : 2;
    static constexpr int NPIECE = STAGE_B / 1024;
    static constexpr int A_PIECES = 2 * BM / RPP;
    static constexpr int PPW = NPIECE / NW;
    static constexpr int ELD = WN * 32 + 4;
    static constexpr int SLAB_B = NW * 32 * ELD * 4;
    static constexpr int LDS_B = NSTG * STAGE_B > SLAB_B ? NSTG * STAGE_B : SLAB_B;
// ... 204 lines not shown
            PF_LOAD(0)
            {
#define a a1
#define b b1
                PF_LOAD(1)
#undef a
#undef b
            }
            if constexpr (SCHED == 2) { PF_PIECE(0); PF_PIECE(1); PF_PIECE(2); PF_PIECE(3); }
            PF_PROD(1, 0); if constexpr (SCHED == 1) { PF_PIECE(0); PF_PIECE(1); } else { PF_PIECE(4); PF_PIECE(5); }
            PF_PROD(0, 1); if constexpr (SCHED == 1) { PF_PIECE(2); PF_PIECE(3); } else { PF_PIECE(6); PF_PIECE(7); }
            PF_PROD(0, 0); if constexpr (SCHED == 1) { PF_PIECE(4); }
#define a a1
#define b b1
            PF_PROD(1, 0); if constexpr (SCHED == 1) { PF_PIECE(5); PF_PIECE(6); }
            PF_PROD(0, 1); if constexpr (SCHED == 1) { PF_PIECE(7); }
            PF_PROD(0, 0);
#undef a
#undef b
        }
#undef PF_PROD
#undef PF_LOAD
#undef PF_PIECE
    }
    }

    gemm2_epilogue<WM, WN, G::NW, MODE, OUT, ABL>(p, acc, smem, m0, n0, nblk, wave, wr, wc, lane);
}
template <int WM, int WN, int MODE, int OUT, int ABL = 0, int SCHED = 0, int WGM = 4, int KS_ = 32>
__global__ __launch_bounds__(WGM * 128, 2) void gemm_f16x2_kernel(Gemm2Args p, int nM, int nN) {
    typedef Geo2<WM, WN, WGM, KS_> G;
    constexpr int BM = G::BM, BN = G::BN;
    extern __shared__ __attribute__((aligned(16))) unsigned char smem[];

    const int L = blockIdx.x;
    const int xcd = L & 7, j8 = L >> 3;
    const int mblk = (j8 / nN) * 8 + xcd, nblk = j8 % nN;
    if (mblk >= nM) return;
    const int m0 = mblk * BM, n0 = nblk * BN;
    if constexpr (OUT == 0 && MODE == 0) {
        if (p.kslices > 1) {
            const size_t z = blockIdx.y;
            p.A += z * (size_t)p.K;
            p.W += z * (size_t)p.K;
            p.C += z * (size_t)p.M * (size_t)p.ldc;
        }
    }

    gemm2_tile_body<WM, WN, MODE, OUT, ABL, SCHED, WGM, KS_>(p, m0, n0, nblk, smem);
}


__global__ __launch_bounds__(256) void split2_kernel(const float* __restrict__ x, int ldx, unsigned short* __restrict__ y,
                                                     int ldy, size_t plane, int M, int N, float scale,
                                                     const float* __restrict__ scale_dev, int seq_out, int seq_in) {
    if (scale_dev) scale *= *scale_dev;
    const int c4n = ldy >> 2;
    const size_t total = (size_t)M * c4n;
    const bool wide_st = ldy % 8 == 0 && plane % 8 == 0 && ((uintptr_t)y & 15) == 0;
    for (size_t i = (size_t)blockIdx.x * 256 + threadIdx.x; i < total; i += (size_t)gridDim.x * 256) {
        const int row = (int)(i / c4n), c = (int)(i % c4n) * 4;
        int xrow = row;
        bool pad = false;
        if (seq_out > 0) {
            const int b = row / seq_out, t = row % seq_out;
            pad = t >= seq_in;
            xrow = b * seq_in + t;
        }
        float v[4] = {0.f, 0.f, 0.f, 0.f};
        if (pad) {
        } else if (c + 3 < N) {
            const float4 t = *reinterpret_cast<const float4*>(x + (size_t)xrow * ldx + c);
            v[0] = t.x; v[1] = t.y; v[2] = t.z; v[3] = t.w;
        } else {
#pragma unroll
            for (int e = 0; e < 4; ++e) if (c + e < N) v[e] = x[(size_t)xrow * ldx + c + e];
        }
        if (wide_st) store_split2x4_pair(y + (size_t)row * ldy + c, plane, v, scale, threadIdx.x);
        else store_split2x4(y + (size_t)row * ldy + c, plane, v, scale);
    }
}

__global__ __launch_bounds__(256) void absmax_kernel(const float* __restrict__ x, size_t n, unsigned* __restrict__ out) {
    float m = 0.f;
    for (size_t i = (size_t)blockIdx.x * 256 + threadIdx.x; i < n; i += (size_t)gridDim.x * 256) m = fmaxf(m, fabsf(x[i]));
    m = wave_max(m);
    if ((threadIdx.x & 63) == 0) atomicMax(out, __builtin_bit_cast(unsigned, m));
}

__global__ __launch_bounds__(256) void rowl1_bound_kernel(const float* __restrict__ W, int rows, int cols, int ld,
                                                          const float* __restrict__ bias, float in_bound, unsigned* __restrict__ out) {
    const int row = blockIdx.x * 4 + (threadIdx.x >> 6), lane = threadIdx.x & 63;
    if (row >= rows) return;
    float a = 0.f;
    for (int k = lane; k < cols; k += 64) a += fabsf(W[(size_t)row * ld + k]);
    a = wave_sum(a);
    const float bnd = (in_bound * a) * 1.0001f + (bias ? fabsf(bias[row]) : 0.f);
    if (lane == 0) atomicMax(out, __builtin_bit_cast(unsigned, bnd));
}

__global__ __launch_bounds__(256) void splitk_reduce_kernel(const float* __restrict__ part, int slices, size_t slice_stride, int M, int N,
                                                            const float* __restrict__ bias, int relu, const float* R1, int ldr1,
                                                            const float* R2, int ldr2, float* C, int ldc, unsigned short* C2, int ldc2,
                                                            size_t c_plane, float cscale) {
    const int n4 = N >> 2;
    const size_t total = (size_t)M * n4;
    for (size_t i = (size_t)blockIdx.x * 256 + threadIdx.x; i < total; i += (size_t)gridDim.x * 256) {
        const int row = (int)(i / n4), col = (int)(i % n4) * 4;
        const float* src = part + (size_t)row * N + col;
        float4 v = *reinterpret_cast<const float4*>(src);
        for (int z = 1; z < slices; ++z) {
            const float4 t = *reinterpret_cast<const float4*>(src + (size_t)z * slice_stride);
            v.x += t.x; v.y += t.y; v.z += t.z; v.w += t.w;
        }
        if (bias) {
            const float4 b = *reinterpret_cast<const float4*>(bias + col);
            v.x += b.x; v.y += b.y; v.z += b.z; v.w += b.w;
        }
        if (relu) { v.x = fmaxf(v.x, 0.f); v.y = fmaxf(v.y, 0.f); v.z = fmaxf(v.z, 0.f); v.w = fmaxf(v.w, 0.f); }
        if (R1) {
            const float4 r = *reinterpret_cast<const float4*>(R1 + (size_t)row * ldr1 + col);
            v.x = v.x + r.x; v.y = v.y + r.y; v.z = v.z + r.z; v.w = v.w + r.w;
        }
        if (R2) {
            const float4 r = *reinterpret_cast<const float4*>(R2 + (size_t)row * ldr2 + col);
            v.x = r.x + v.x; v.y = r.y + v.y; v.z = r.z + v.z; v.w = r.w + v.w;
        }
        if (C2) {
            const float o[4] = {v.x, v.y, v.z, v.w};
            store_split2x4(C2 + (size_t)row * ldc2 + col, c_plane, o, cscale);
        } else {
            *reinterpret_cast<float4*>(C + (size_t)row * ldc + col) = v;
        }
    }
}

template <int WM, int WN, int MODE, int OUT, int ABL = 0, int SCHED = 0, int WGM = 4, int KS_ = 32>
int launch_tile(const Gemm2Args& a, hipStream_t stream) {
    typedef Geo2<WM, WN, WGM, KS_> G;
    static PerDeviceOnce configured;
    if (!configured.done()) {
        PF_HIP_TRY(hipFuncSetAttribute(reinterpret_cast<const void*>(&gemm_f16x2_kernel<WM, WN, MODE, OUT, ABL, SCHED, WGM, KS_>),
                                       hipFuncAttributeMaxDynamicSharedMemorySize, G::LDS_B));
        configured.mark();
    }
    const int nM = ceil_div(a.M, G::BM), nN = ceil_div(a.N, G::BN);
    const int nMpad = (nM + 7) / 8 * 8;
    const unsigned gy = (OUT == 0 && MODE == 0 && a.kslices > 1) ? (unsigned)a.kslices : 1u;
    hipLaunchKernelGGL((gemm_f16x2_kernel<WM, WN, MODE, OUT, ABL, SCHED, WGM, KS_>), dim3((unsigned)nMpad * nN, gy), dim3(WGM * 128), G::LDS_B, stream, a, nM, nN);
    PF_HIP_TRY(hipGetLastError());
    return 0;
}
#if defined(PF_MEASUREMENT_KERNELS)
template <int MODE, int OUT>
int launch_pair(const Gemm2Args& a, hipStream_t stream) { return launch_tile<2, 4, MODE, OUT, 0, 0, 2, 16>(a, stream); }
template <int MODE, int OUT>
int launch_ring(const Gemm2Args& a, hipStream_t stream) { return launch_tile<2, 4, MODE, OUT, 0, 0, 4, 16>(a, stream); }
#endif
template <int MODE, int OUT>
int launch_one(const Gemm2Args& a, hipStream_t stream) {
    if constexpr (OUT == 1) {
        if (a.tile == 3) return launch_tile<2, 2, MODE, 1, 0, 0, 2>(a, stream);
    }
    if constexpr (OUT == 0) {
        if (a.tile == 3) return launch_tile<2, 2, MODE, 0, 0, 0, 2>(a, stream);
    }
#if defined(PF_MEASUREMENT_KERNELS)
    if constexpr (OUT == 0) {
        if (a.tile >= 256) return (a.tile >> 8) == 1 ? launch_tile<2, 4, MODE, 0, 0, 1>(a, stream) : launch_tile<2, 4, MODE, 0, 0, 2>(a, stream);
    }
    if constexpr (MODE == 0 && OUT == 0) {
        if (a.tile == 0x82) return launch_tile<2, 2, 0, 0, 2, 0, 2>(a, stream);
        if (a.tile == 0x83) return launch_tile<2, 2, 0, 0, 3, 0, 2>(a, stream);
        if (a.tile >= 16) {
            switch (a.tile >> 4) {
                case 1: return launch_tile<2, 4, 0, 0, 1>(a, stream);
                case 2: return launch_tile<2, 4, 0, 0, 2>(a, stream);
                case 3: return launch_tile<2, 4, 0, 0, 3>(a, stream);
                default: return launch_tile<2, 4, 0, 0, 4>(a, stream);
            }
        }
    }
#endif
    const int n_cu = device_cu_count();
    const long m_tiles = ceil_div(a.M, 256);
    const long wide_blocks = m_tiles * (a.N / 256), narrow_blocks = m_tiles * ceil_div(a.N, 128);
    const double cost_wide = (double)((wide_blocks + n_cu - 1) / n_cu), cost_narrow = 0.57 * (double)((narrow_blocks + n_cu - 1) / n_cu);
    const bool wide = a.tile == 2 || a.tile == 8 || a.tile == 9 || (a.tile == 0 && a.N % 256 == 0 && cost_wide <= cost_narrow);
    if constexpr (OUT == 0) {
        const long small_blocks = (long)ceil_div(a.M, 128) * ceil_div(a.N, 128);
        const double cost_small = 0.55 * (double)((small_blocks + 2 * n_cu - 1) / (2 * n_cu));
        if (a.tile == 0 && cost_small < (wide ? cost_wide : cost_narrow)) return launch_tile<2, 2, MODE, 0, 0, 0, 2>(a, stream);
    }
    if constexpr (OUT == 1) {
        if (a.tile == 0 && 2 * narrow_blocks <= n_cu) return launch_tile<2, 2, MODE, 1, 0, 0, 2>(a, stream);
    }
#if defined(PF_MEASUREMENT_KERNELS)
    if (wide && a.tile == 8) return launch_tile<2, 4, MODE, OUT, 0, 2>(a, stream);
    if (wide && a.tile == 9) return launch_tile<2, 4, MODE, OUT, 0, 3>(a, stream);
#endif
    return wide ? launch_tile<2, 4, MODE, OUT, 0, 0>(a, stream) : launch_tile<2, 2, MODE, OUT>(a, stream);
}

}

__global__ void pow2_scale_kernel(const float* __restrict__ amax, float* __restrict__ sc) {
    const float a = *amax;
    int e = a > 0.f ? (int)floorf(log2f(32768.f / a)) : 0;
    e = e > 100 ? 100 : (e < -100 ? -100 : e);
    sc[0] = ldexpf(1.f, e);
    sc[1] = ldexpf(1.f, -e);
}

int launch_pow2_scale(const float* amax_dev, float* sc, hipStream_t stream) {
    hipLaunchKernelGGL(pow2_scale_kernel, dim3(1), dim3(1), 0, stream, amax_dev, sc);
    PF_HIP_TRY(hipGetLastError());
    return 0;
}

__global__ void kv_scales_kernel(const float* __restrict__ amax, const float* __restrict__ lb, int n, float* __restrict__ out) {
    const int i = blockIdx.x * 64 + threadIdx.x;
    if (i >= 2 * n) return;
    const float bound = *amax * lb[2 * i] + lb[2 * i + 1];
    int e = bound > 0.f ? (int)floorf(log2f(32768.f / bound)) : 0;
    e = e > 60 ? 60 : (e < -60 ? -60 : e);
    out[4 * (i >> 1) + (i & 1)] = ldexpf(1.f, e);
    out[4 * (i >> 1) + 2 + (i & 1)] = ldexpf(1.f, -e);
}

int launch_kv_scales(const float* amax_dev, const float* l1_bmax_dev, int n_layers, float* out, hipStream_t stream) {
    hipLaunchKernelGGL(kv_scales_kernel, dim3(ceil_div(2 * n_layers, 64)), dim3(64), 0, stream, amax_dev, l1_bmax_dev, n_layers, out);
    PF_HIP_TRY(hipGetLastError());
    return 0;
}

int launch_split2(const float* x, int ldx, unsigned short* y, int ldy, size_t plane, int M, int N, float scale,
                  hipStream_t stream, const float* scale_dev, int seq_out, int seq_in) {
    PF_REQUIRE(M > 0 && N > 0 && ldy >= N && ldy % 4 == 0, "split2: ldy must cover N and be a multiple of 4");
    PF_REQUIRE(ldx % 4 == 0 && ((uintptr_t)x & 15) == 0 && ((uintptr_t)y & 7) == 0 && plane % 4 == 0, "split2: alignment");
    const size_t total = (size_t)M * (ldy >> 2);
    const unsigned blocks = (unsigned)((total + 255) / 256 < 8192 ? (total + 255) / 256 : 8192);
    hipLaunchKernelGGL(split2_kernel, dim3(blocks), dim3(256), 0, stream, x, ldx, y, ldy, plane, M, N, scale, scale_dev, seq_out, seq_in);
    PF_HIP_TRY(hipGetLastError());
    return 0;
}

int launch_absmax(const float* x, size_t n, float* out_dev, hipStream_t stream) {
    PF_HIP_TRY(hipMemsetAsync(out_dev, 0, sizeof(float), stream));
    const unsigned blocks = (unsigned)((n + 255) / 256 < 2048 ? (n + 255) / 256 : 2048);
    hipLaunchKernelGGL(absmax_kernel, dim3(blocks ? blocks : 1), dim3(256), 0, stream, x, n, reinterpret_cast<unsigned*>(out_dev));
    PF_HIP_TRY(hipGetLastError());
    return 0;
}

int launch_rowl1_bound(const float* W, int rows, int cols, int ld, const float* bias, float in_bound, float* out_dev,
                       hipStream_t stream) {
    PF_HIP_TRY(hipMemsetAsync(out_dev, 0, sizeof(float), stream));
    hipLaunchKernelGGL(rowl1_bound_kernel, dim3(ceil_div(rows, 4)), dim3(256), 0, stream, W, rows, cols, ld, bias, in_bound,
                       reinterpret_cast<unsigned*>(out_dev));
    PF_HIP_TRY(hipGetLastError());
    return 0;
}

static bool qkv_form_prefers_ps(const Gemm2Args& a) {
    static const int mode = [] { const char* e = getenv("PF_QKV_PS"); return e ? atoi(e) : 2; }();
    if (mode == 0 || !gemm_f16x2_ps_ok(a)) return false;
    if (mode == 1) return true;
    const int n_cu = device_cu_count();
    const long blocks = (long)ceil_div(a.M, 256) * (a.N / 256);
    if (blocks < n_cu) return false;
    const double rounds = (double)blocks / n_cu, whole = (double)((blocks + n_cu - 1) / n_cu);
    return whole / rounds > 1.15;
}

int gemm_f16x2_argmax_parts(int M, int N) { (void)M; return 2 * ceil_div(N, 256); }

int launch_gemm_f16x2(const Gemm2Args& a, hipStream_t stream) {
    PF_REQUIRE(a.M > 0 && a.N > 0 && a.K > 0, "gemm_f16x2: empty problem");
    if (a.ksplit > 1) {
        PF_REQUIRE((a.C || a.C2 || a.ln_g) && a.part && !a.amax_val && a.qkv_D <= 0 && a.a_kstep <= 0 && a.w_kstep <= 0 &&
                   a.K % (32 * a.ksplit) == 0 && a.N % 4 == 0 && ((uintptr_t)a.part & 15) == 0,
                   "gemm_f16x2: the split-K form needs K % (32 ksplit) == 0 and a partial buffer [ksplit][M][N]");
        if (a.C2) PF_REQUIRE(!a.ln_g && a.ldc2 % 4 == 0 && a.c_plane % 4 == 0 && ((uintptr_t)a.C2 & 7) == 0, "gemm_f16x2: split-K plane output alignment");
        else PF_REQUIRE((a.ln_g && !a.C) || (a.ldc % 4 == 0 && ((uintptr_t)a.C & 15) == 0), "gemm_f16x2: split-K output alignment");
        PF_REQUIRE(a.lda % 8 == 0 && a.ldw % 8 == 0 && a.a_plane % 8 == 0 && a.w_plane % 8 == 0 && ((uintptr_t)a.A & 15) == 0 &&
                   ((uintptr_t)a.W & 15) == 0 && (a.K / a.ksplit) % 8 == 0, "gemm_f16x2: operand alignment");
        if (a.bias) PF_REQUIRE(((uintptr_t)a.bias & 15) == 0, "gemm_f16x2: bias alignment");
        if (a.R1) PF_REQUIRE(a.ldr1 % 4 == 0 && ((uintptr_t)a.R1 & 15) == 0, "gemm_f16x2: R1 alignment");
        if (a.R2) PF_REQUIRE(a.ldr2 % 4 == 0 && ((uintptr_t)a.R2 & 15) == 0, "gemm_f16x2: R2 alignment");
        Gemm2Args p = a;
        p.ksplit = 0; p.kslices = a.ksplit; p.K = a.K / a.ksplit;
        p.C = a.part; p.ldc = a.N; p.C2 = nullptr; p.bias = nullptr; p.relu = 0; p.R1 = nullptr; p.R2 = nullptr; p.tile = 0;
        int rc = launch_tile<2, 2, 0, 0, 0, 0, 2>(p, stream);
        if (rc) return rc;
        if (a.ln_g) {
            PF_REQUIRE(a.ln_b && a.ln_y, "gemm_f16x2: the split-K + LayerNorm form needs beta and an output");
            return launch_splitk_reduce_ln(a.part, a.ksplit, (size_t)a.M * a.N, a.M, a.N, a.bias, a.relu, a.R1, a.ldr1, a.R2, a.ldr2, a.C, a.ldc, a.ln_g, a.ln_b,
                                           a.ln_eps, a.ln_y, a.ln_ldy, a.ln_out, a.ln_plane, a.ln_oscale, stream);
        }
        const size_t total = (size_t)a.M * (a.N >> 2);
        const unsigned blocks = (unsigned)((total + 255) / 256 < 4096 ? (total + 255) / 256 : 4096);
        hipLaunchKernelGGL(splitk_reduce_kernel, dim3(blocks), dim3(256), 0, stream, a.part, a.ksplit, (size_t)a.M * a.N, a.M, a.N,
                           a.bias, a.relu, a.R1, a.ldr1, a.R2, a.ldr2, a.C, a.ldc, a.C2, a.ldc2, a.c_plane, a.cscale);
        PF_HIP_TRY(hipGetLastError());
        return 0;
    }
    if (a.amax_val) {
        PF_REQUIRE(a.amax_idx && a.amax_ld >= gemm_f16x2_argmax_parts(a.M, a.N) && !a.R1 && !a.R2 && !a.relu && a.qkv_D <= 0,
                   "gemm_f16x2: the arg-max form takes bias only and needs amax_ld >= 2 ceil(N / 256)");
        PF_REQUIRE(a.K % 32 == 0 && a.lda % 8 == 0 && a.ldw % 8 == 0 && ((uintptr_t)a.A & 15) == 0 && ((uintptr_t)a.W & 15) == 0,
                   "gemm_f16x2: operand alignment");
        return launch_tile<2, 4, 0, 3, 0, 0>(a, stream);
    }
    PF_REQUIRE(a.K % 32 == 0, "gemm_f16x2: K must be a multiple of 32 (pad the planes with zeros)");
    PF_REQUIRE(a.lda % 8 == 0 && a.ldw % 8 == 0 && a.a_plane % 8 == 0 && a.w_plane % 8 == 0, "gemm_f16x2: operand strides % 8");
    PF_REQUIRE(((uintptr_t)a.A & 15) == 0 && ((uintptr_t)a.W & 15) == 0, "gemm_f16x2: operands must be 16-B aligned");
    PF_REQUIRE(a.N % 4 == 0, "gemm_f16x2: N % 4");
    if (a.C2 && a.qkv_D <= 0) PF_REQUIRE(a.ldc2 % 4 == 0 && a.c_plane % 4 == 0 && ((uintptr_t)a.C2 & 7) == 0, "gemm_f16x2: plane output alignment");
    else if (a.qkv_D <= 0 || a.C) PF_REQUIRE(a.C && a.ldc % 4 == 0 && ((uintptr_t)a.C & 15) == 0, "gemm_f16x2: output alignment");
    if (a.bias) PF_REQUIRE(((uintptr_t)a.bias & 15) == 0, "gemm_f16x2: bias alignment");
    if (a.R1) PF_REQUIRE(a.ldr1 % 4 == 0 && ((uintptr_t)a.R1 & 15) == 0, "gemm_f16x2: R1 alignment");
    if (a.R2) PF_REQUIRE(a.ldr2 % 4 == 0 && ((uintptr_t)a.R2 & 15) == 0, "gemm_f16x2: R2 alignment");
    const int mode = (a.R1 ? 1 : 0) | (a.R2 ? 2 : 0);
    if (a.qkv_D > 0) {
        PF_REQUIRE(mode == 0 && !a.relu && a.N == (a.kv_form ? 2 : 3) * a.qkv_D && a.qkv_D % 256 == 0 && a.M % 16 == 0,
                   "gemm_f16x2: the QKV / KV form needs N == 3 D (2 D), D % 256 == 0, M % 16 == 0, no residuals");
        PF_REQUIRE((a.kv_form || (a.Qp && a.C)) && a.Kp && a.VT && a.ldvt % 8 == 0 && a.vt_plane % 8 == 0 && a.qk_plane % 8 == 0 &&
                   ((uintptr_t)a.Qp & 15) == 0 && ((uintptr_t)a.Kp & 15) == 0 && ((uintptr_t)a.VT & 15) == 0,
                   "gemm_f16x2: QKV outputs");
    }
    if ((a.tile & 15) == 10 || (a.tile & 15) == 12) {
        if (gemm_f16x2_ps_ok(a)) return launch_gemm_f16x2_ps(a, stream);
// ... 89 lines not shown
```

funasr_amd/csrc/rowwise.hip:

```cpp
#include "common.h"

namespace pf {

namespace {

__device__ __forceinline__ float4 load4(const float* base, size_t off, bool bf16) {
    if (!bf16) return *reinterpret_cast<const float4*>(base + off);
    const uint2 u = *reinterpret_cast<const uint2*>(reinterpret_cast<const unsigned short*>(base) + off);
    float4 v;
    v.x = bf16_to_f32((unsigned short)(u.x & 0xffffu)); v.y = bf16_to_f32((unsigned short)(u.x >> 16));
    v.z = bf16_to_f32((unsigned short)(u.y & 0xffffu)); v.w = bf16_to_f32((unsigned short)(u.y >> 16));
    return v;
}

template <int NV, int OUT>
__global__ __launch_bounds__(256) void layernorm_kernel(const float* __restrict__ x, int ldx,
                                                        const float* __restrict__ gamma,
                                                        const float* __restrict__ beta, float* __restrict__ y,
                                                        int ldy, int M, int D, int Dpad, float eps, int in_bf16,
                                                        size_t plane, float oscale, int seq_out, int seq_in,
                                                        const int* __restrict__ out_map) {
    const int lane = threadIdx.x & 63;
    const int xr0 = blockIdx.x * 4 + (threadIdx.x >> 6);
    if (xr0 >= M) return;
// ... 204 lines not shown
            o.y = __fadd_rn(__fmul_rn(a.y, scale), p.y);
            o.z = __fadd_rn(__fmul_rn(a.z, scale), p.z);
            o.w = __fadd_rn(__fmul_rn(a.w, scale), p.w);
        }
        reinterpret_cast<float4*>(y)[i] = o;
    }
}

__global__ __launch_bounds__(256) void scale_add_pe_rows_kernel(const float* __restrict__ x, const float* __restrict__ pe,
                                                                float* __restrict__ y, const int* __restrict__ map, int T,
                                                                int D4, float scale, size_t total4) {
    size_t i = (size_t)blockIdx.x * 256 + threadIdx.x;
    const size_t stride = (size_t)gridDim.x * 256;
    for (; i < total4; i += stride) {
        const int r = (int)(i / D4), c = (int)(i % D4);
        const int src = map[r];
        float4 o = make_float4(0.f, 0.f, 0.f, 0.f);
        if (src >= 0) {
            const float4 a = reinterpret_cast<const float4*>(x)[(size_t)src * D4 + c];
            const float4 p = reinterpret_cast<const float4*>(pe)[(size_t)(src % T) * D4 + c];
            o.x = __fadd_rn(__fmul_rn(a.x, scale), p.x);
            o.y = __fadd_rn(__fmul_rn(a.y, scale), p.y);
            o.z = __fadd_rn(__fmul_rn(a.z, scale), p.z);
            o.w = __fadd_rn(__fmul_rn(a.w, scale), p.w);
        }
        reinterpret_cast<float4*>(y)[i] = o;
    }
}

constexpr int FSMN_TT = 8;
template <int KS, int LP>
__global__ __launch_bounds__(256) void fsmn_kernel(FsmnArgs p) {
    const int b = blockIdx.y;
    const int t0 = blockIdx.x * FSMN_TT;
    const int c4 = threadIdx.x;
    if (c4 * 4 >= p.C) return;
    const int len = p.lens[b];
    const size_t base = p.offs ? (size_t)p.offs[b] : (size_t)b * p.T;
    const int rows = p.offs ? p.offs[b + 1] - p.offs[b] : p.T;
    if (t0 >= rows) return;
    float4 w[KS];
    {
        const float* wp = p.w + (size_t)c4 * 4 * KS;
#pragma unroll
        for (int j = 0; j < KS; ++j) {
            w[j].x = wp[j];
            w[j].y = wp[KS + j];
            w[j].z = wp[2 * KS + j];
            w[j].w = wp[3 * KS + j];
        }
    }
    float4 win[KS + FSMN_TT - 1];
#pragma unroll
    for (int i = 0; i < KS + FSMN_TT - 1; ++i) {
        const int tt = t0 - LP + i;
        if (tt >= 0 && tt < p.T && tt < len)
            win[i] = load4(p.in, (base + tt) * p.ldin + c4 * 4, p.in_bf16 != 0);
        else
            win[i] = make_float4(0.f, 0.f, 0.f, 0.f);
    }
#pragma unroll
    for (int i = 0; i < FSMN_TT; ++i) {
        const int t = t0 + i;
        if (t < rows) {
            float4 o = make_float4(0.f, 0.f, 0.f, 0.f);
            if (t < len) {
                float4 acc = make_float4(0.f, 0.f, 0.f, 0.f);
#pragma unroll
                for (int j = 0; j < KS; ++j) {
                    acc.x = fmaf(w[j].x, win[i + j].x, acc.x);
                    acc.y = fmaf(w[j].y, win[i + j].y, acc.y);
                    acc.z = fmaf(w[j].z, win[i + j].z, acc.z);
                    acc.w = fmaf(w[j].w, win[i + j].w, acc.w);
                }
                const float4 c = win[i + LP];
                o.x = acc.x + c.x; o.y = acc.y + c.y; o.z = acc.z + c.z; o.w = acc.w + c.w;
            }
            const size_t row = base + t;
            if (p.R) {
                const float4 r = *reinterpret_cast<const float4*>(p.R + row * p.ldr + c4 * 4);
                o.x = r.x + o.x; o.y = r.y + o.y; o.z = r.z + o.z; o.w = r.w + o.w;
            }
            *reinterpret_cast<float4*>(p.out + row * p.ldo + c4 * 4) = o;
        }
    }
}

__global__ __launch_bounds__(256) void cast_bf16_kernel(const float* __restrict__ x, unsigned short* __restrict__ y, size_t n4) {
    for (size_t i = (size_t)blockIdx.x * 256 + threadIdx.x; i < n4; i += (size_t)gridDim.x * 256) {
        const float4 v = reinterpret_cast<const float4*>(x)[i];
        uint2 pk;
        pk.x = (unsigned)f32_to_bf16(v.x) | ((unsigned)f32_to_bf16(v.y) << 16);
        pk.y = (unsigned)f32_to_bf16(v.z) | ((unsigned)f32_to_bf16(v.w) << 16);
        reinterpret_cast<uint2*>(y)[i] = pk;
    }
}

}

int launch_cast_bf16(const float* x, unsigned short* y, size_t n, hipStream_t stream) {
    PF_REQUIRE(n % 4 == 0, "cast_bf16: n % 4");
    const size_t n4 = n / 4;
    const int blocks = (int)((n4 + 255) / 256 < 8192 ? (n4 + 255) / 256 : 8192);
    hipLaunchKernelGGL(cast_bf16_kernel, dim3(blocks > 0 ? blocks : 1), dim3(256), 0, stream, x, y, n4);
    PF_HIP_TRY(hipGetLastError());
    return 0;
}

int launch_layernorm(const float* x, int ldx, const float* gamma, const float* beta, float* y, int ldy, int M,
                     int D, int Dpad, float eps, hipStream_t stream, int out_mode, int in_bf16, size_t plane,
                     float oscale, int seq_out, int seq_in, const int* out_map) {
    PF_REQUIRE(M > 0 && D > 0 && D % 4 == 0 && D <= 2048, "layernorm: D must be a multiple of 4 and <= 2048");
    PF_REQUIRE(Dpad >= D && Dpad % 4 == 0 && Dpad <= 2048 && ldy >= Dpad, "layernorm: bad Dpad/ldy");
    PF_REQUIRE(ldx % 4 == 0 && ldy % 4 == 0, "layernorm: strides must be multiples of 4");
    PF_REQUIRE(((uintptr_t)y & 15) == 0, "layernorm: output must be 16-B aligned");
    dim3 grid(ceil_div(M, 4)), block(256);
    const int nv = ceil_div(Dpad / 4, 64);
#define PF_LN(NV_)                                                                                                 \
    do {                                                                                                          \
        if (out_mode == 3) hipLaunchKernelGGL((layernorm_kernel<NV_, 3>), grid, block, 0, stream, x, ldx, gamma, beta, y, ldy, M, D, Dpad, eps, in_bf16, plane, oscale, seq_out, seq_in, out_map); \
        else if (out_mode == 2) hipLaunchKernelGGL((layernorm_kernel<NV_, 2>), grid, block, 0, stream, x, ldx, gamma, beta, y, ldy, M, D, Dpad, eps, in_bf16, plane, oscale, seq_out, seq_in, out_map); \
        else if (out_mode == 1) hipLaunchKernelGGL((layernorm_kernel<NV_, 1>), grid, block, 0, stream, x, ldx, gamma, beta, y, ldy, M, D, Dpad, eps, in_bf16, plane, oscale, seq_out, seq_in, out_map); \
        else hipLaunchKernelGGL((layernorm_kernel<NV_, 0>), grid, block, 0, stream, x, ldx, gamma, beta, y, ldy, M, D, Dpad, eps, in_bf16, plane, oscale, seq_out, seq_in, out_map);         \
    } while (0)
    if (nv <= 2) PF_LN(2);
    else if (nv <= 3) PF_LN(3);
    else PF_LN(8);
#undef PF_LN
    PF_HIP_TRY(hipGetLastError());
    return 0;
}

int launch_splitk_reduce_ln(const float* part, int slices, size_t slice_stride, int M, int D, const float* bias, int relu, const float* R1, int ldr1,
                            const float* R2, int ldr2, float* C, int ldc, const float* gamma, const float* beta, float eps, float* y, int ldy,
                            int out_mode, size_t plane, float oscale, hipStream_t stream) {
    PF_REQUIRE(M > 0 && D > 0 && D % 4 == 0 && D <= 2048 && slices >= 1 && part && y && gamma && beta, "splitk_reduce_ln: D % 4, D <= 2048");
    PF_REQUIRE((!C || ldc % 4 == 0) && ldy % 4 == 0 && (!R2 || ldr2 % 4 == 0) && (!R1 || (ldr1 % 4 == 0 && ((uintptr_t)R1 & 15) == 0)) &&
                   slice_stride % 4 == 0 && (out_mode == 0 || out_mode == 3),
               "splitk_reduce_ln: strides % 4; fp32 or two-plane output");
    PF_REQUIRE(((uintptr_t)part & 15) == 0 && ((uintptr_t)C & 15) == 0 && ((uintptr_t)y & 15) == 0 && (!bias || ((uintptr_t)bias & 15) == 0) &&
               (!R2 || ((uintptr_t)R2 & 15) == 0), "splitk_reduce_ln: operands must be 16-B aligned");
    dim3 grid(ceil_div(M, 4)), block(256);
#define PF_RLN(NV_, OUT_) hipLaunchKernelGGL((splitk_reduce_ln_kernel<NV_, OUT_>), grid, block, 0, stream, part, slices, slice_stride, M, D, bias, relu, \
                                             R1, ldr1, R2, ldr2, C, ldc, gamma, beta, eps, y, ldy, plane, oscale)
    const int nv = ceil_div(D / 4, 64);
    PF_REQUIRE(nv <= 2 || nv > 3, "splitk_reduce_ln: widths of 513 .. 768 columns are not instantiated");
    if (nv <= 2) { if (out_mode == 3) PF_RLN(2, 3); else PF_RLN(2, 0); }
    else { if (out_mode == 3) PF_RLN(8, 3); else PF_RLN(8, 0); }
#undef PF_RLN
    PF_HIP_TRY(hipGetLastError());
    return 0;
}

int launch_ln_consts(const float* W, int ldw, int N, int K, const float* gamma, const float* beta, const float* bias, float* c1, float* c2,
                     hipStream_t stream) {
    PF_REQUIRE(W && gamma && beta && c1 && c2 && N > 0 && K > 0 && K % 4 == 0 && ldw % 4 == 0 && ((uintptr_t)W & 15) == 0 &&
               ((uintptr_t)gamma & 15) == 0 && ((uintptr_t)beta & 15) == 0, "ln_consts: K % 4, 16-B aligned operands");
    hipLaunchKernelGGL(ln_consts_kernel, dim3(ceil_div(N, 4)), dim3(256), 0, stream, W, ldw, N, K, gamma, beta, bias, c1, c2);
    PF_HIP_TRY(hipGetLastError());
    return 0;
}

__global__ __launch_bounds__(256) void scale_cols_kernel(float* __restrict__ x, int ld, int M, int N4, float sc) {
    const size_t total = (size_t)M * N4;
    for (size_t i = (size_t)blockIdx.x * 256 + threadIdx.x; i < total; i += (size_t)gridDim.x * 256) {
        float4* p = reinterpret_cast<float4*>(x + (i / N4) * (size_t)ld) + i % N4;
        float4 v = *p;
        v.x *= sc; v.y *= sc; v.z *= sc; v.w *= sc;
        *p = v;
    }
}
int launch_scale_cols(float* x, int ld, int M, int N, float sc, hipStream_t stream) {
    PF_REQUIRE(M > 0 && N > 0 && N % 4 == 0 && ld % 4 == 0 && ((uintptr_t)x & 15) == 0, "scale_cols: alignment");
    const size_t total = (size_t)M * (N / 4);
    const unsigned blocks = (unsigned)((total + 255) / 256 < 2048 ? (total + 255) / 256 : 2048);
    hipLaunchKernelGGL(scale_cols_kernel, dim3(blocks), dim3(256), 0, stream, x, ld, M, N / 4, sc);
    PF_HIP_TRY(hipGetLastError());
    return 0;
}

__global__ __launch_bounds__(256) void scatter_i32_kernel(const int* __restrict__ in, const int* __restrict__ map, int* __restrict__ out, int n) {
    const int i = blockIdx.x * 256 + threadIdx.x;
    if (i < n) out[map[i]] = in[i];
}
int launch_scatter_i32(const int* in, const int* map, int* out, int n, hipStream_t stream) {
    if (n <= 0) return 0;
    hipLaunchKernelGGL(scatter_i32_kernel, dim3(ceil_div(n, 256)), dim3(256), 0, stream, in, map, out, n);
    PF_HIP_TRY(hipGetLastError());
    return 0;
}

int launch_log_softmax(const float* x, int ldx, float* y, int ldy, int M, int N, hipStream_t stream) {
    PF_REQUIRE(M > 0 && N > 0 && ldx >= N && ldy >= N, "log_softmax: bad shape");
    hipLaunchKernelGGL(log_softmax_kernel, dim3(ceil_div(M, 4)), dim3(256), 0, stream, x, ldx, y, ldy, M, N);
    PF_HIP_TRY(hipGetLastError());
    return 0;
}

int launch_scale_add_pe(const float* x, const float* pe, float* y, int B, int T, int D, float scale,
                        hipStream_t stream, int Tp) {
    PF_REQUIRE(B > 0 && T > 0 && D % 4 == 0, "scale_add_pe: D must be a multiple of 4");
    if (Tp > T) {
        const size_t tot = (size_t)B * Tp * (D / 4);
        const int nb = (int)((tot + 255) / 256 < 4096 ? (tot + 255) / 256 : 4096);
        hipLaunchKernelGGL(scale_add_pe_pad_kernel, dim3(nb), dim3(256), 0, stream, x, pe, y, T, Tp, D / 4, scale, tot);
        PF_HIP_TRY(hipGetLastError());
        return 0;
    }
    const size_t total4 = (size_t)B * T * (D / 4);
    const int blocks = (int)((total4 + 255) / 256 < 4096 ? (total4 + 255) / 256 : 4096);
    hipLaunchKernelGGL(scale_add_pe_kernel, dim3(blocks), dim3(256), 0, stream, x, pe, y, T, D / 4, scale, total4);
    PF_HIP_TRY(hipGetLastError());
    return 0;
}

int launch_scale_add_pe_rows(const float* x, const float* pe, float* y, const int* map, int M, int T, int D, float scale,
                             hipStream_t stream) {
    PF_REQUIRE(M > 0 && T > 0 && D % 4 == 0 && map, "scale_add_pe_rows: bad arguments");
    const size_t tot = (size_t)M * (D / 4);
    const int nb = (int)((tot + 255) / 256 < 4096 ? (tot + 255) / 256 : 4096);
    hipLaunchKernelGGL(scale_add_pe_rows_kernel, dim3(nb), dim3(256), 0, stream, x, pe, y, map, T, D / 4, scale, tot);
    PF_HIP_TRY(hipGetLastError());
    return 0;
}

int launch_fsmn(const FsmnArgs& a, hipStream_t stream) {
    PF_REQUIRE(a.B > 0 && a.T > 0 && a.C % 4 == 0 && a.C <= 1024, "fsmn: C must be a multiple of 4 and <= 1024");
    PF_REQUIRE(a.ldin % 4 == 0 && a.ldo % 4 == 0 && (a.R == nullptr || a.ldr % 4 == 0), "fsmn: strides % 4");
    dim3 grid(ceil_div(a.T, FSMN_TT), a.B), block(a.C / 4);
    if (a.K == 11 && a.left_pad == 5)
        hipLaunchKernelGGL((fsmn_kernel<11, 5>), grid, block, 0, stream, a);
    else if (a.K == 11 && a.left_pad == 10)
        hipLaunchKernelGGL((fsmn_kernel<11, 10>), grid, block, 0, stream, a);
    else if (a.K == 21 && a.left_pad == 10)
        hipLaunchKernelGGL((fsmn_kernel<21, 10>), grid, block, 0, stream, a);
    else {
        set_error("fsmn: built for kernel_size 11 with left padding 5 (offline) or 10 (sanm_shfit 5) and kernel_size 21 "
                  "with left padding 10");
        return -1;
    }
    PF_HIP_TRY(hipGetLastError());
    return 0;
}

}
```

funasr_amd/ops.py:

```python
from __future__ import annotations

import ctypes as C

import torch

from . import _lib


def _stream() -> int:
    return torch.cuda.current_stream().cuda_stream


def _ptr(t):
    return None if t is None else t.data_ptr()


def _f32c(t: torch.Tensor, name: str) -> torch.Tensor:
    if not t.is_cuda:
        raise RuntimeError(f"{name}: expected a tensor in GPU memory (there is no CPU path)")
    if t.dtype != torch.float32:
        raise TypeError(f"{name}: expected float32, got {t.dtype}")
    return t


# ... 383 lines not shown
        else:
            yf = torch.empty(M, 512, device=dev, dtype=torch.float32)
    ms = C.c_float(0)
    _lib.check(lib.pf_k_gemm_f16x2_row(_ptr(a2), K, M * K, _ptr(w2), K, 512 * K, float(2.0 ** -scale_exp), _ptr(bias),
                                       _ptr(add1), add1.stride(0) if add1 is not None else 0,
                                       _ptr(add2), add2.stride(0) if add2 is not None else 0,
                                       _ptr(c), 512, _ptr(g), _ptr(b), float(eps), _ptr(y2), M * 512, float(2.0 ** out_scale_exp),
                                       _ptr(yf), M, K, int(relu), (int(a_nt) & 3) | (int(block_rows) << 8), int(time_iters),
                                       C.byref(ms), _stream()),
               "pf_k_gemm_f16x2_row")
    y = y2 if y2 is not None else yf
    return (c, y, float(ms.value)) if time_iters > 0 else (c, y)


def ffn_f16x2(x2: torch.Tensor, w1: torch.Tensor, w2: torch.Tensor, b1: torch.Tensor, b2, resid: torch.Tensor, e_x: int, e_w1: int,
              e_h: int, e_w2: int, ln=None, out_scale_exp: int = 0, ln_planes: bool = True, want_c: bool = True,
              in_place: bool = False, time_iters: int = 0, abl: int = 0, w_kblocked: bool = False):
    lib = _lib.load()
    for t_ in (x2, w1, w2):
        assert t_.dtype == torch.float16 and t_.is_contiguous()
    _, M, D = x2.shape
    if w_kblocked:
        F = w1.shape[2]
        assert D == 512 and tuple(w1.shape) == (2, 16, F, 32) and tuple(w2.shape) == (2, F // 32, 512, 32)
    else:
        F = w1.shape[1]
        assert D == 512 and tuple(w1.shape) == (2, F, 512) and tuple(w2.shape) == (2, 512, F)
    assert resid.dtype == torch.float32 and tuple(resid.shape) == (M, 512) and resid.is_contiguous()
    dev = x2.device
    c = resid if in_place else (torch.empty(M, 512, device=dev, dtype=torch.float32) if (want_c or ln is None) else None)
    y2 = yf = g = b = None
    eps = 0.0
    if ln is not None:
        g, b, eps = ln
        if ln_planes:
            y2 = torch.empty(2, M, 512, device=dev, dtype=torch.float16)
        else:
            yf = torch.empty(M, 512, device=dev, dtype=torch.float32)
    ms = C.c_float(0)
    _lib.check(lib.pf_k_ffn_f16x2(_ptr(x2), _ptr(w1), _ptr(w2), _ptr(b1), _ptr(b2), float(2.0 ** -(e_x + e_w1)), float(2.0 ** e_h),
                                  float(2.0 ** -(e_h + e_w2)), _ptr(resid), _ptr(c), _ptr(g), _ptr(b), float(eps), _ptr(y2),
                                  float(2.0 ** out_scale_exp), _ptr(yf), M, F | (int(abl) << 24) | (int(bool(w_kblocked)) << 28), int(time_iters), C.byref(ms), _stream()),
               "pf_k_ffn_f16x2")
    y = y2 if y2 is not None else yf
    return (c, y, float(ms.value)) if time_iters > 0 else (c, y)


def gemm_f16x2_row_fsmn(a2: torch.Tensor, w2: torch.Tensor, bias, v: torch.Tensor, taps: torch.Tensor, lo: torch.Tensor,
                        hi: torch.Tensor, add2=None, scale_exp: int = 0, ln=None, out_scale_exp: int = 0, ln_planes: bool = True,
                        want_c: bool = True, a_nt: bool = False, time_iters: int = 0, block_rows: int = 0):
    lib = _lib.load()
    assert a2.dtype == torch.float16 and w2.dtype == torch.float16 and a2.is_contiguous() and w2.is_contiguous()
    _, M, K = a2.shape
    assert w2.shape[1] == 512 and w2.shape[2] == K and M % 16 == 0 and ln is not None
    assert v.dtype == torch.float32 and v.shape == (M, 512) and v.stride(1) == 1 and taps.shape == (512, 11) and taps.is_contiguous()
    assert lo.dtype == torch.int32 and hi.dtype == torch.int32 and lo.numel() == M // 16 and hi.numel() == M // 16
    dev = a2.device
    c = torch.empty(M, 512, device=dev, dtype=torch.float32) if want_c else None
    g, b, eps = ln
    y2 = torch.empty(2, M, 512, device=dev, dtype=torch.float16) if ln_planes else None
    yf = None if ln_planes else torch.empty(M, 512, device=dev, dtype=torch.float32)
    ms = C.c_float(0)
    _lib.check(lib.pf_k_gemm_f16x2_row_fsmn(_ptr(a2), K, M * K, _ptr(w2), K, 512 * K, float(2.0 ** -scale_exp), _ptr(bias),
                                            _ptr(v), v.stride(0), _ptr(taps), _ptr(lo), _ptr(hi),
                                            _ptr(add2), add2.stride(0) if add2 is not None else 0, _ptr(c), 512, _ptr(g), _ptr(b),
                                            float(eps), _ptr(y2), M * 512, float(2.0 ** out_scale_exp), _ptr(yf), M, K,
                                            (int(a_nt) & 3) | (int(block_rows) << 8), int(time_iters), C.byref(ms), _stream()),
               "pf_k_gemm_f16x2_row_fsmn")
    y = y2 if y2 is not None else yf
    return (c, y, float(ms.value)) if time_iters > 0 else (c, y)


def layernorm_planes(x: torch.Tensor, gamma, beta, eps: float, scale_exp: int = 0, time_iters: int = 0):
    lib = _lib.load()
    M, D = x.shape
    assert x.stride(1) == 1
    y = torch.empty(2, M, D, device=x.device, dtype=torch.float16)
    ms = C.c_float(0)
    _lib.check(lib.pf_k_layernorm_planes(_ptr(x), x.stride(0), _ptr(gamma), _ptr(beta), _ptr(y), D, M * D, float(2.0 ** scale_exp),
                                         M, D, float(eps), int(time_iters), C.byref(ms), _stream()), "pf_k_layernorm_planes")
    return (y, float(ms.value)) if time_iters > 0 else y


def vt_columns(m: torch.Tensor) -> torch.Tensor:
    return (m & ~12) | ((m & 4) << 1) | ((m & 8) >> 1)


def gemm_f16x2_qkv(a2: torch.Tensor, w2: torch.Tensor, bias, D: int, scale_exp: int, q_mul: float, k_mul: float, v_mul: float,
                   kv_form: bool = False, tile: int = 0, time_iters: int = 0):
    lib = _lib.load()
    _, M, K = a2.shape
    dev = a2.device
    nseg = 2 if kv_form else 3
    assert w2.shape[1] == nseg * D and M % 16 == 0
    q2 = None if kv_form else torch.zeros(2, M + 32, D, device=dev, dtype=torch.float16)
    k2 = torch.zeros(2, M + 32, D, device=dev, dtype=torch.float16)
    v = None if kv_form else torch.empty(M, D, device=dev, dtype=torch.float32)
    ldvt = M + 64
    vt = torch.zeros(2, D, ldvt, device=dev, dtype=torch.float16)
    ms = C.c_float(0)
    _lib.check(lib.pf_k_gemm_f16x2_qkv(_ptr(a2), K, M * K, _ptr(w2), K, nseg * D * K, float(2.0 ** -scale_exp), _ptr(bias), M, D, K,
                                       int(kv_form), _ptr(q2), _ptr(k2), (M + 32) * D, _ptr(v), _ptr(vt), ldvt, D * ldvt,
                                       float(q_mul), float(k_mul), float(v_mul), int(tile), int(time_iters), C.byref(ms), _stream()),
               "pf_k_gemm_f16x2_qkv")
    out = dict(q2=q2, k2=k2, v=v, vt=vt)
    if time_iters > 0:
        out["ms"] = float(ms.value)
    return out


def gemm_f16x2_argmax(a2: torch.Tensor, w2: torch.Tensor, bias, scale_exp: int = 0) -> torch.Tensor:
    lib = _lib.load()
    _, M, K = a2.shape
    N = w2.shape[1]
    nparts = 2 * ((N + 255) // 256)
    dev = a2.device
    ids = torch.empty(M, device=dev, dtype=torch.int32)
    sval = torch.empty(M, nparts, device=dev, dtype=torch.float32)
    sidx = torch.empty(M, nparts, device=dev, dtype=torch.int32)
    _lib.check(lib.pf_k_gemm_f16x2_argmax(_ptr(a2), K, M * K, _ptr(w2), K, N * K, float(2.0 ** -scale_exp), _ptr(bias), M, N, K,
                                          _ptr(ids), _ptr(sval), _ptr(sidx), _stream()), "pf_k_gemm_f16x2_argmax")
    return ids


def attention_f16x2(q, k, v, klens, n_heads: int, scale: float, eq: int = 6, ek: int = 6, ev: int = 6, variant: int = 0,
                    time_iters: int = 0):
    lib = _lib.load()
    B, Tq, D = q.shape
    Tp = k.shape[1]
    assert Tp % 16 == 0 and D == n_heads * 128
    dev = q.device
    q2 = split2((q * scale).reshape(B * Tq, D).contiguous(), eq)
    k2 = torch.zeros(2, B * Tp + 32, D, device=dev, dtype=torch.float16)
    k2[:, : B * Tp] = split2(k.reshape(B * Tp, D).contiguous(), ek)
    v2 = split2(v.reshape(B * Tp, D).contiguous(), ev)
    col = vt_columns(torch.arange(B * Tp, device=dev))
    ldvt = B * Tp + 64
    vt = torch.zeros(2, D, ldvt, device=dev, dtype=torch.float16)
    vt[:, :, col] = v2.transpose(1, 2)
    o2 = torch.empty(2, B * Tq, D, device=dev, dtype=torch.float16)
    ms = C.c_float(0)
    _lib.check(lib.pf_k_attention_f16x2(_ptr(q2), B * Tq * D, _ptr(k2), (B * Tp + 32) * D, _ptr(vt), ldvt, D * ldvt, _ptr(o2), B * Tq * D,
                                        _ptr(klens), B, n_heads, Tp, Tq, float(2.0 ** -(eq + ek)), float(2.0 ** -10), int(variant),
                                        int(time_iters), C.byref(ms), _stream()), "pf_k_attention_f16x2")
    out = ((o2[0].float() + o2[1].float()) * 2.0 ** -ev).view(B, Tq, D)
    return (out, float(ms.value)) if time_iters > 0 else out


def attention_bf16(q, k, v, klens, n_heads: int, scale: float):
    lib = _lib.load()
    B, Tq, D = q.shape
    Tk = k.shape[1]
    assert q.dtype == torch.bfloat16 and q.stride(2) == 1 and k.stride(2) == 1 and v.stride(2) == 1
    out = torch.empty(B, Tq, D, device=q.device, dtype=torch.bfloat16)
    _lib.check(lib.pf_k_attention_bf16(_ptr(q), q.stride(1), _ptr(k), k.stride(1), _ptr(v), v.stride(1), _ptr(out), D,
                                       _ptr(klens), B, n_heads, Tq, Tk, float(scale), _stream()), "pf_k_attention_bf16")
    return out
```

funasr_amd/paraformer_decoder.py:

```python
from __future__ import annotations

from typing import List

import torch
import torch.nn as nn

from . import _lib
from .hip_module import Holder, HipModule, ParamHolder, depthwise, device_lens, host_i32, layer_norm, linear, stream_ptr
from .register import tables


def _ffn(block, d_model, ffn):
    block.norm1 = layer_norm(d_model)
    block.feed_forward = Holder()
    block.feed_forward.w_1 = linear(ffn, d_model)
    block.feed_forward.norm = layer_norm(ffn)
    block.feed_forward.w_2 = linear(d_model, ffn, bias=False)


def _block2(d_model, ffn, kernel_size):
    b = Holder()
    _ffn(b, d_model, ffn)
    b.norm2 = layer_norm(d_model)
    b.self_attn = Holder()
    b.self_attn.fsmn_block = depthwise(d_model, kernel_size)
    return b


def _block(d_model, ffn, kernel_size):
    b = Holder()
    _ffn(b, d_model, ffn)
    b.norm2 = layer_norm(d_model)
    b.self_attn = Holder()
    b.self_attn.fsmn_block = depthwise(d_model, kernel_size)
    b.norm3 = layer_norm(d_model)
    b.src_attn = Holder()
    b.src_attn.linear_q = linear(d_model, d_model)
    b.src_attn.linear_k_v = linear(2 * d_model, d_model)
    b.src_attn.linear_out = linear(d_model, d_model)
    return b


@tables.register("decoder_classes", "ParaformerSANMDecoder")
class ParaformerSANMDecoder(HipModule):
    _prefix = "pf_decoder"
    _skip_keys = ("embed.",)

    def __init__(self, vocab_size: int, encoder_output_size: int, attention_heads: int = 4, linear_units: int = 2048,
                 num_blocks: int = 6, dropout_rate: float = 0.1, positional_dropout_rate: float = 0.1,
                 self_attention_dropout_rate: float = 0.0, src_attention_dropout_rate: float = 0.0,
                 input_layer: str = "embed", use_output_layer: bool = True, wo_input_layer: bool = False,
                 pos_enc_class=None, normalize_before: bool = True, concat_after: bool = False,
                 att_layer_num: int = 6, kernel_size: int = 21, sanm_shfit: int = 0, lora_list: List[str] = None,
                 lora_rank: int = 8, lora_alpha: int = 16, lora_dropout: float = 0.1,
                 chunk_multiply_factor: tuple = (1,), tf2torch_tensor_name_prefix_torch: str = "decoder",
                 tf2torch_tensor_name_prefix_tf: str = "seq2seq/decoder", **kwargs):
        super().__init__()
        if not normalize_before or concat_after or lora_list:
            raise NotImplementedError("ParaformerSANMDecoder(HIP): normalize_before, no concat_after, no LoRA is built")
        if sanm_shfit is None:
            sanm_shfit = (kernel_size - 1) // 2
        D = encoder_output_size
        self.vocab_size, self.d_model, self.attention_heads, self.linear_units = vocab_size, D, attention_heads, linear_units
        self.att_layer_num, self.num_blocks, self.kernel_size, self.sanm_shfit = att_layer_num, num_blocks, kernel_size, sanm_shfit
        if not wo_input_layer and input_layer == "embed":
            self.embed = nn.ModuleList([ParamHolder((vocab_size, D), None)])
        self.decoders = nn.ModuleList([_block(D, linear_units, kernel_size) for _ in range(att_layer_num)])
        self.decoders2 = (nn.ModuleList([_block2(D, linear_units, kernel_size) for _ in range(num_blocks - att_layer_num)])
                          if num_blocks - att_layer_num > 0 else None)
        last = Holder()
        _ffn(last, D, linear_units)
        self.decoders3 = nn.ModuleList([last])
        self.after_norm = layer_norm(D)
        self.output_layer = linear(vocab_size, D) if use_output_layer else None

    def _default_precision(self) -> str:
        ok = self.d_model % 256 == 0 and self.d_model // self.attention_heads == 128 and self.linear_units % 256 == 0
        return "f16x2" if ok else "fp32"

    def _mode(self) -> str:
        return getattr(self, "_precision", None) or self._default_precision()

    def set_precision(self, mode=None):
        if mode is not None and mode not in ("fp32", "bf16", "bf16x3", "f16x2"):
            raise ValueError("precision must be 'fp32', 'bf16', 'bf16x3' or 'f16x2'")
        self._precision = mode
        return self

    def _make_config(self):
        return _lib.pf_decoder_config(self.vocab_size if self.output_layer is not None else 0, self.d_model, self.attention_heads, self.linear_units,
                                      self.att_layer_num, self.kernel_size, self.sanm_shfit, 1e-12)

    def _after_create(self, lib, handle):
        if self.decoders2 is not None:
            _lib.check(lib.pf_decoder_set_decoders2(handle, len(self.decoders2)), "pf_decoder_set_decoders2")

    def _apply_settings(self):
        lib, h = self._ensure_handle()
        _lib.check(lib.pf_decoder_set_precision(h, {"fp32": 0, "bf16": 1, "bf16x3": 2, "f16x2": 3}[self._mode()]),
                   "pf_decoder_set_precision")
        return lib, h

    def _run(self, hs_pad, hlens, ys_in_pad, ys_in_lens, want_logits: bool, want_ids: bool, want_hidden: bool = False):
        lib, h = self._apply_settings()
        dev = self._handle_device
        mem = hs_pad.to(device=dev, dtype=torch.float32).contiguous()
        emb = ys_in_pad.to(device=dev, dtype=torch.float32).contiguous()
        B, T, D = mem.shape
        N = emb.shape[1]
        mlen_c, _ = host_i32(hlens, B)
        tlen_c, tlens = host_i32(ys_in_lens, B)
        logits = torch.empty(B, N, self.vocab_size, device=dev, dtype=torch.float32) if want_logits else None
        ids = torch.empty(B, N, device=dev, dtype=torch.int32) if want_ids else None
        hid = torch.empty(B, N, D, device=dev, dtype=torch.float32) if want_hidden else None
        with torch.cuda.device(dev):
            _lib.check(lib.pf_decoder_forward(h, mem.data_ptr(), mlen_c, emb.data_ptr(), tlen_c, B, T, N,
                                              logits.data_ptr() if want_logits else None,
                                              ids.data_ptr() if want_ids else None,
                                              hid.data_ptr() if want_hidden else None, stream_ptr()),
                       "pf_decoder_forward")
        olens = device_lens(tlens, dev, torch.int64)
        return logits, ids, hid, olens

    def forward_asf6(self, hs_pad, hlens, ys_in_pad, ys_in_lens, n_blocks_before: int = 5) -> torch.Tensor:
        lib, h = self._ensure_handle()
        dev = self._handle_device
        mem = hs_pad.to(device=dev, dtype=torch.float32).contiguous()
        emb = ys_in_pad.to(device=dev, dtype=torch.float32).contiguous()
        B, T, _ = mem.shape
        N = emb.shape[1]
        mlen_c, _ = host_i32(hlens, B)
        tlen_c, _ = host_i32(ys_in_lens, B)
        scores = torch.empty(T, device=dev, dtype=torch.float32)
        with torch.cuda.device(dev):
            _lib.check(lib.pf_decoder_asf_scores(h, mem.data_ptr(), mlen_c, emb.data_ptr(), tlen_c, B, T, N, n_blocks_before,
                                                 scores.data_ptr(), stream_ptr()), "pf_decoder_asf_scores")
        return scores

    def forward(self, hs_pad, hlens, ys_in_pad, ys_in_lens, chunk_mask=None, return_hidden: bool = False,
                return_both: bool = False):
        if chunk_mask is not None:
            raise NotImplementedError("chunk_mask is a training/streaming feature")
        if self.output_layer is None:
            _, _, hid, olens = self._run(hs_pad, hlens, ys_in_pad, ys_in_lens, want_logits=False, want_ids=False, want_hidden=True)
            return hid, olens
        logits, _, hid, olens = self._run(hs_pad, hlens, ys_in_pad, ys_in_lens, want_logits=not return_hidden or return_both,
                                          want_ids=False, want_hidden=return_hidden or return_both)
        if return_both:
            return logits, hid, olens
        if return_hidden:
            return hid, olens
        return logits, olens

    def greedy(self, hs_pad, hlens, ys_in_pad, ys_in_lens):
        _, ids, _, olens = self._run(hs_pad, hlens, ys_in_pad, ys_in_lens, want_logits=False, want_ids=True)
        return ids, olens
```

include/paraformer_hip.h:

```cpp
#ifndef PARAFORMER_HIP_H_
#define PARAFORMER_HIP_H_

#include <stdint.h>

#ifdef __cplusplus
extern "C" {
#endif

#define PF_ABI_VERSION 5

const char* pf_last_error(void);
int pf_abi_version(void);
int pf_device_count(void);

int pf_set_concurrency_guard(int32_t on);
int pf_concurrency_guard(void);

typedef struct pf_frontend pf_frontend;

typedef struct pf_frontend_config {
    int32_t sample_rate;
    int32_t frame_length;
    int32_t frame_shift;
    int32_t n_mels;
// ... 28 lines not shown

typedef struct pf_encoder pf_encoder;

typedef struct pf_encoder_config {
    int32_t input_dim;
    int32_t d_model;
    int32_t n_heads;
    int32_t ffn_dim;
    int32_t n_blocks;
    int32_t tp_blocks;
    int32_t kernel_size;
    int32_t sanm_shift;
    float ln_eps;
} pf_encoder_config;

pf_encoder* pf_encoder_create(const pf_encoder_config* cfg);
void pf_encoder_destroy(pf_encoder* e);
int pf_encoder_set_tensor(pf_encoder* e, const char* name, const float* data, int64_t numel);
int pf_encoder_missing(const pf_encoder* e);
int pf_encoder_set_precision(pf_encoder* e, int32_t mode);
int pf_encoder_set_row_packing(pf_encoder* e, int32_t extra_rows);
int pf_encoder_set_option(pf_encoder* e, const char* key, int32_t value);
int pf_encoder_set_vad_mask(pf_encoder* e, const int32_t* vad_pos_host, int32_t B);
int pf_encoder_forward(pf_encoder* e, const float* xs_dev, const int32_t* lens_host, int32_t B, int32_t T,
                       const float* pe_dev, float* out_dev, int32_t run_blocks, void* stream);

typedef struct pf_predictor pf_predictor;

typedef struct pf_predictor_config {
    int32_t d_model;
    int32_t l_order;
    int32_t r_order;
    float threshold;
    float smooth_factor;
    float noise_threshold;
    float tail_threshold;
    int32_t tail_mask;
} pf_predictor_config;

pf_predictor* pf_predictor_create(const pf_predictor_config* cfg);
void pf_predictor_destroy(pf_predictor* p);
int pf_predictor_set_tensor(pf_predictor* p, const char* name, const float* data, int64_t numel);
int pf_predictor_missing(const pf_predictor* p);
int pf_predictor_alphas(pf_predictor* p, const float* hidden_dev, const int32_t* lens_host, int32_t B, int32_t T,
                        float* alphas_dev, float* peaks_dev, int32_t* token_num_host, void* stream);
int pf_predictor_embeds(pf_predictor* p, const float* hidden_dev, int32_t B, int32_t T, int32_t N,
                        float* embeds_dev, void* stream);
int pf_predictor_alphas_begin(pf_predictor* p, int32_t slot, const float* hidden_dev, const int32_t* lens_host, int32_t B, int32_t T,
                              float* alphas_dev, float* peaks_dev, int32_t* counts_pinned_host, void* stream);
int pf_predictor_embeds_slot(pf_predictor* p, int32_t slot, const float* hidden_dev, int32_t B, int32_t T, int32_t N,
                             float* embeds_dev, void* stream);

typedef struct pf_predictor_v3_config {
    int32_t upsample_times;
    int32_t upsample_type;
    int32_t use_cif1_cnn;
    float smooth_factor2;
    float noise_threshold2;
} pf_predictor_v3_config;
pf_predictor* pf_predictor_create_v3(const pf_predictor_config* cfg, const pf_predictor_v3_config* cfg3);
int pf_predictor_timestamp(pf_predictor* p, const float* hidden_dev, const int32_t* lens_host,
                           const int32_t* token_num_host, int32_t B, int32_t T, float* us_alphas_dev, float* us_peaks_dev,
                           void* stream);

typedef struct pf_decoder pf_decoder;

typedef struct pf_decoder_config {
    int32_t vocab_size;
    int32_t d_model;
    int32_t n_heads;
    int32_t ffn_dim;
    int32_t n_blocks;
    int32_t kernel_size;
    int32_t sanm_shift;
    float ln_eps;
} pf_decoder_config;

pf_decoder* pf_decoder_create(const pf_decoder_config* cfg);
void pf_decoder_destroy(pf_decoder* d);
int pf_decoder_set_decoders2(pf_decoder* d, int32_t n_layers);
int pf_decoder_set_tensor(pf_decoder* d, const char* name, const float* data, int64_t numel);
int pf_decoder_missing(const pf_decoder* d);
int pf_decoder_set_precision(pf_decoder* d, int32_t mode);
int pf_decoder_forward(pf_decoder* d, const float* memory_dev, const int32_t* mem_lens_host,
                       const float* embeds_dev, const int32_t* tok_lens_host, int32_t B, int32_t T, int32_t N,
                       float* logits_dev, int32_t* ids_dev, float* hidden_dev, void* stream);
typedef struct pf_paraformer pf_paraformer;
pf_paraformer* pf_paraformer_create(pf_encoder* e, pf_predictor* p, pf_decoder* d);
void pf_paraformer_destroy(pf_paraformer* m);
int pf_paraformer_forward(pf_paraformer* m, const float* feats_dev, const int32_t* lens_host, int32_t B, int32_t T,
                          const float* pe_dev, int32_t* ids_dev, int32_t ids_ld, int32_t* token_num_host,
                          float* alphas_dev, float* peaks_dev, void* stream);
int pf_paraformer_begin(pf_paraformer* m, const float* feats_dev, const int32_t* lens_host, int32_t B, int32_t T,
                        const float* pe_dev, void* stream);
int pf_paraformer_finish(pf_paraformer* m, int32_t ticket, int32_t* ids_dev, int32_t ids_ld, int32_t* token_num_host,
                         float* alphas_dev, float* peaks_dev, void* stream);
const float* pf_paraformer_encoder_out(const pf_paraformer* m);
const float* pf_paraformer_embeds(const pf_paraformer* m);

int pf_decoder_asf_scores(pf_decoder* d, const float* memory_dev, const int32_t* mem_lens_host, const float* embeds_dev,
                          const int32_t* tok_lens_host, int32_t B, int32_t T, int32_t N, int32_t n_blocks_before,
                          float* scores_dev, void* stream);
pf_decoder* pf_decoder_create_contextual(const pf_decoder_config* cfg);
int pf_decoder_forward_contextual(pf_decoder* d, const float* memory_dev, const int32_t* mem_lens_host, const float* embeds_dev,
                                  const int32_t* tok_lens_host, const float* contextual_dev, int32_t n_hot, float clas_scale,
                                  int32_t B, int32_t T, int32_t N, float* logits_dev, int32_t* ids_dev, float* hidden_dev,
                                  void* stream);

typedef struct pf_vad pf_vad;
typedef struct pf_vad_config {
    int32_t input_dim, input_affine_dim, fsmn_layers, linear_dim, proj_dim, lorder, rorder, lstride, rstride,
        output_affine_dim, output_dim;
} pf_vad_config;
pf_vad* pf_vad_create(const pf_vad_config* cfg);
void pf_vad_destroy(pf_vad* v);
int pf_vad_set_tensor(pf_vad* v, const char* name, const float* data, int64_t numel);
int pf_vad_missing(const pf_vad* v);
int pf_vad_forward(pf_vad* v, const float* feats_dev, int32_t B, int32_t T, float* cache_dev, const int32_t* sil_ids_host,
                   int32_t n_sil, float* p_sil_dev, float* probs_dev, int32_t small_m, void* stream);
int pf_vad_frame_decibel(const float* wav_dev, int64_t n_samples, int32_t n_frames, int32_t frame_len, int32_t frame_shift,
                         float* out_dev, void* stream);

typedef struct pf_vad_decision pf_vad_decision;
typedef struct pf_vad_options {
    int32_t sample_rate, detect_mode, max_end_silence_time, max_start_silence_time, window_size_ms,
        sil_to_speech_time_thres, speech_to_sil_time_thres, do_extend, lookback_time_start_point,
        lookahead_time_end_point, max_single_segment_time, noise_frame_num_used_for_snr, frame_in_ms, frame_length_ms;
    double speech_2_noise_ratio, snr_thres, decibel_thres, speech_noise_thres, fe_prior_thres;
} pf_vad_options;
pf_vad_decision* pf_vad_decision_create(const pf_vad_options* opts);
void pf_vad_decision_destroy(pf_vad_decision* d);
void pf_vad_decision_set_thresholds(pf_vad_decision* d, double max_end_sil_ms, double speech_noise_thres);
int pf_vad_decision_state(const pf_vad_decision* d);
int pf_vad_decision_push(pf_vad_decision* d, const float* sil_scores, const float* decibels, int32_t n_frames,
                         int32_t is_final, int32_t streaming_events, int32_t* segments_out, int32_t capacity);

typedef struct pf_campplus pf_campplus;
typedef struct pf_campplus_config {
    int32_t feat_dim, embedding_size, growth_rate, bn_size, init_channels, m_channels;
    float bn_eps;
} pf_campplus_config;
pf_campplus* pf_campplus_create(const pf_campplus_config* cfg);
void pf_campplus_destroy(pf_campplus* h);
int pf_campplus_set_tensor(pf_campplus* h, const char* name, const float* data, int64_t numel);
int pf_campplus_missing(const pf_campplus* h);
int pf_campplus_set_max_batch(pf_campplus* h, int32_t max_chunks);
int pf_campplus_forward(pf_campplus* h, const float* feats_dev, int32_t B, int32_t T, float* emb_dev, void* stream);
int pf_campplus_embed_chunks(pf_campplus* h, const float* wav_dev, int64_t n_samples, const int64_t* starts_host,
                             const int32_t* valid_host, int32_t N, int32_t chunk_len, float* emb_dev, void* stream);

typedef struct pf_emotion2vec pf_emotion2vec;
typedef struct pf_emotion2vec_config {
    int32_t embed_dim, num_heads, ffn_dim, prenet_depth, depth;
    int32_t num_extra_tokens, num_alibi_heads;
    int32_t alibi_scale_layers;
    int32_t alibi_scale_heads;
    int32_t n_conv, conv_kernel[8], conv_stride[8];
    int32_t conv_pos_depth, conv_pos_kernel, conv_pos_groups;
    int32_t vocab_size;
    int32_t normalize;
    int32_t precision;
    float norm_eps;
} pf_emotion2vec_config;
pf_emotion2vec* pf_emotion2vec_create(const pf_emotion2vec_config* cfg);
void pf_emotion2vec_destroy(pf_emotion2vec* h);
int pf_emotion2vec_set_tensor(pf_emotion2vec* h, const char* name, const float* data, int64_t numel);
// ... 87 lines not shown
int pf_stream_peek(pf_stream* s, float* cif_alpha_host, float* cif_hidden_host, int32_t* start_idx_host);

typedef struct pf_dp pf_dp;
int pf_dp_unique_id(void* id_out, int32_t cap);
pf_dp* pf_dp_create(const void* unique_id, int32_t id_bytes, int32_t world, int32_t rank);
int pf_dp_destroy(pf_dp* dp);
int pf_dp_world(const pf_dp* dp);
int pf_dp_rank(const pf_dp* dp);
int pf_dp_broadcast_encoder(pf_dp* dp, pf_encoder* e, int32_t root, void* stream);
int pf_dp_broadcast_predictor(pf_dp* dp, pf_predictor* p, int32_t root, void* stream);
int pf_dp_broadcast_decoder(pf_dp* dp, pf_decoder* d, int32_t root, void* stream);
int pf_dp_broadcast_ctc(pf_dp* dp, pf_ctc* c, int32_t root, void* stream);
int pf_dp_broadcast_raw(pf_dp* dp, void* buf_dev, int64_t bytes, int32_t root, void* stream);
int pf_dp_gather_ids(pf_dp* dp, const int32_t* ids_dev, int64_t count, int32_t* out_dev, int32_t root, void* stream);

int pf_frontend_fbank(pf_frontend* f, const float* wav_dev, int64_t n_samples, float* fbank_dev, void* stream);
int pf_frontend_lfr_cmvn(pf_frontend* f, const float* frames_dev, int32_t T, int32_t rows, float* out_dev, void* stream);

int pf_encoder_debug_poison(pf_encoder* e, int32_t byte);
int pf_decoder_debug_poison(pf_decoder* d, int32_t byte);
int pf_predictor_debug_poison(pf_predictor* p, int32_t byte);
int pf_k_gemm_skinny_ln(const float* A, int32_t lda, const float* W, int32_t ldw, const float* bias, const float* R2, int32_t ldr2,
                        float* Cout, int32_t ldc, int32_t M, int32_t N, int32_t K, int32_t relu, float* stats_out,
                        const float* stats_in, const float* ln_g, const float* ln_c, float ln_eps, const float* out_gamma, float* ws_part,
                        int32_t* ws_count, void* stream);
int pf_k_ln_consts(const float* W, int32_t ldw, int32_t N, int32_t K, const float* gamma, const float* beta, const float* bias, float* c,
                   void* stream);
int pf_set_skinny_max_m(int32_t m);
int pf_k_gemm_f32(const float* A, int32_t lda, const float* W, int32_t ldw, const float* bias, const float* R1,
                  int32_t ldr1, const float* R2, int32_t ldr2, float* C, int32_t ldc, int32_t M, int32_t N,
                  int32_t K, int32_t relu, void* stream);
int pf_measurement_build(void);
int pf_k_conv1d_gemm_f32(const float* hidden, const float* W, const float* bias, float* C, int32_t B, int32_t T, int32_t D,
                         int32_t N, int32_t taps, int32_t left, int32_t relu, const float* zero_dev, void* stream);
int pf_k_gemm_bf16(const void* A, int32_t lda, const void* W, int32_t ldw, const float* bias, const float* R1,
                   int32_t ldr1, const float* R2, int32_t ldr2, void* C, int32_t ldc, int32_t M, int32_t N, int32_t K,
                   int32_t relu, int32_t c_bf16, void* stream);
int pf_k_gemm_bf16_time(const void* A, int32_t lda, const void* W, int32_t ldw, const float* bias, void* C, int32_t ldc,
                        int32_t M, int32_t N, int32_t K, int32_t c_bf16, int32_t iters, float* ms_out, void* stream);
int pf_k_split3(const float* x, int32_t ldx, void* y3, int32_t ldy, int64_t plane, int32_t M, int32_t N, void* stream);
int pf_k_gemm_split3(const void* A3, int32_t lda, int64_t a_plane, const void* W3, int32_t ldw, int64_t w_plane,
                     const float* bias, const float* R1, int32_t ldr1, const float* R2, int32_t ldr2, float* C,
                     int32_t ldc, void* C3, int32_t ldc3, int64_t c_plane, int32_t M, int32_t N, int32_t K,
                     int32_t relu, int32_t iters, float* ms_out, void* stream);
int pf_k_gemm_f16x2_row(const void* A2, int32_t lda, int64_t a_plane, const void* W2, int32_t ldw, int64_t w_plane, float oscale,
                        const float* bias, const float* R1, int32_t ldr1, const float* R2, int32_t ldr2, float* C, int32_t ldc,
                        const float* ln_g, const float* ln_b, float ln_eps, void* Y2, int64_t y_plane, float yscale, float* Yf,
                        int32_t M, int32_t K, int32_t relu, int32_t a_nt, int32_t iters, float* ms_out, void* stream);
int pf_k_ffn_f16x2(const void* X2, const void* W1, const void* W2, const float* b1, const float* b2, float oscale1, float hscale,
                   float oscale2, const float* R, float* Cout, const float* ln_g, const float* ln_b, float ln_eps, void* Y2,
                   float yscale, float* Yf, int32_t M, int32_t F, int32_t iters, float* ms_out, void* stream);
int pf_k_gemm_f16x2_row_fsmn(const void* A2, int32_t lda, int64_t a_plane, const void* W2, int32_t ldw, int64_t w_plane, float oscale,
                             const float* bias, const float* fs_v, int32_t ldfv, const float* fs_w, const int32_t* fs_lo,
                             const int32_t* fs_hi, const float* R2, int32_t ldr2, float* C, int32_t ldc, const float* ln_g,
                             const float* ln_b, float ln_eps, void* Y2, int64_t y_plane, float yscale, float* Yf, int32_t M, int32_t K,
                             int32_t a_nt, int32_t iters, float* ms_out, void* stream);
int pf_k_layernorm_planes(const float* x, int32_t ldx, const float* gamma, const float* beta, void* y2, int32_t ldy, int64_t plane,
                          float scale, int32_t M, int32_t D, float eps, int32_t iters, float* ms_out, void* stream);
int pf_k_gemm_f16x2_qkv(const void* A2, int32_t lda, int64_t a_plane, const void* W2, int32_t ldw, int64_t w_plane, float oscale,
                        const float* bias, int32_t M, int32_t D, int32_t K, int32_t kv_form, void* Qp, void* Kp, int64_t qk_plane,
                        float* Vf, void* VT, int32_t ldvt, int64_t vt_plane, float q_mul, float k_mul, float v_mul, int32_t tile,
                        int32_t iters, float* ms_out, void* stream);
int pf_k_gemm_f16x2_argmax(const void* A2, int32_t lda, int64_t a_plane, const void* W2, int32_t ldw, int64_t w_plane, float oscale,
                           const float* bias, int32_t M, int32_t N, int32_t K, int32_t* ids, float* scratch_val,
                           int32_t* scratch_idx, void* stream);
int pf_k_split2(const float* x, int32_t ldx, void* y2, int32_t ldy, int64_t plane, int32_t M, int32_t N, float scale,
                void* stream);
int pf_k_gemm_f16x2(const void* A2, int32_t lda, int64_t a_plane, const void* W2, int32_t ldw, int64_t w_plane,
                    float oscale, const float* bias, const float* R1, int32_t ldr1, const float* R2, int32_t ldr2,
                    float* C, int32_t ldc, void* C2, int32_t ldc2, int64_t c_plane, float cscale, int32_t M, int32_t N,
                    int32_t K, int32_t relu, int32_t tile, int32_t iters, float* ms_out, void* stream);
int pf_k_attention_f16x2(const void* Q2, int64_t q_plane, const void* K2, int64_t k_plane, const void* VT2, int32_t ldvt,
                         int64_t vt_plane, void* O2, int64_t o_plane, const int32_t* klens_dev, int32_t B, int32_t H,
                         int32_t Tp, int32_t Tq, float sscale, float oscale, int32_t variant, int32_t iters, float* ms_out,
                         void* stream);
int pf_k_cast_bf16(const float* x, void* y, int64_t n, void* stream);
int pf_k_gemm_argmax_f32(const float* A, int32_t lda, const float* W, int32_t ldw, const float* bias, int32_t M,
                         int32_t N, int32_t K, int32_t* ids, float* scratch_val, int32_t* scratch_idx, void* stream);
int pf_k_log_softmax(const float* x, int32_t ldx, float* y, int32_t ldy, int32_t M, int32_t N, void* stream);
int pf_k_layernorm(const float* x, int32_t ldx, const float* gamma, const float* beta, float* y, int32_t ldy,
                   int32_t M, int32_t D, int32_t Dpad, float eps, void* stream);
int pf_k_fsmn(const float* in, int32_t ldin, const float* w, const float* R, int32_t ldr, float* out, int32_t ldo,
              const int32_t* lens_dev, int32_t B, int32_t T, int32_t C, int32_t K, int32_t left_pad, void* stream);
int pf_k_attention_f32(const float* Q, int32_t ldq, const float* K, int32_t ldk, const float* V, int32_t ldv,
                       float* O, int32_t ldo, const int32_t* klens_dev, int32_t B, int32_t H, int32_t Tq,
                       int32_t Tk, float scale, void* stream);
int pf_k_attention_f32_two_source(const float* Q, int32_t ldq, const float* K, int32_t ldk, const float* V, int32_t ldv,
                                  const float* K2, int32_t ldk2, const float* V2, int32_t ldv2, float* O, int32_t ldo,
                                  const int32_t* n1_dev, int32_t n1_stride, int32_t B, int32_t H, int32_t Tq,
                                  int32_t Tk, int32_t T2, int32_t n2, float scale, void* stream);
int pf_k_attention_small(const float* Q, int32_t ldq, const float* K, int32_t ldk, const float* V, int32_t ldv,
                         float* O, int32_t ldo, const int32_t* klens_dev, int32_t B, int32_t H, int32_t d_k,
                         int32_t Tq, int32_t Tk, float scale, void* stream);
int pf_k_gather_rows(const float* table, int32_t ld, int32_t rows, const int32_t* ids_dev, float* out, int32_t n,
                     int32_t D, void* stream);
int pf_k_attention_split3(const float* Q, int32_t ldq, const float* K, int32_t ldk, const float* V, int32_t ldv,
                          float* O, int32_t ldo, const int32_t* klens_dev, int32_t B, int32_t H, int32_t Tq,
                          int32_t Tk, float scale, void* stream);
int pf_k_attention_bf16(const void* Q, int32_t ldq, const void* K, int32_t ldk, const void* V, int32_t ldv, void* O,
                        int32_t ldo, const int32_t* klens_dev, int32_t B, int32_t H, int32_t Tq, int32_t Tk, float scale,
                        void* stream);
int pf_k_lstm(const float* x, const float* w_ih, const float* w_hh, const float* b_ih, const float* b_hh, int32_t B, int32_t T,
              int32_t D, int32_t H, int32_t ndir, float* out, void* stream);
int pf_k_cif(const float* alphas, const float* hidden, int32_t B, int32_t T, int32_t D, int32_t N, float* peaks,
             int32_t* n_fires, float* embeds, void* stream);
int pf_k_cif_tail(const float* alphas, const float* hidden, const int32_t* lens_host, int32_t B, int32_t T, int32_t D, int32_t N,
                  float tail_threshold, int32_t tail_mask, int32_t loop, float* alphas_out, float* peaks, int32_t* n_fires,
                  int32_t* n_tok, float* embeds, void* stream);
int pf_k_ctc_runs(const int32_t* ids_dev, const int32_t* lens_host, int32_t B, int32_t T, int32_t blank, int32_t* counts_dev,
                  int32_t* ranges_dev, int32_t ld, void* stream);
int pf_k_argmax_rows(const float* x, int32_t ldx, int32_t M, int32_t N, int32_t* ids, void* stream);
int pf_k_gemm_f32_time(const float* A, int32_t lda, const float* W, int32_t ldw, const float* bias, float* C,
                       int32_t ldc, int32_t M, int32_t N, int32_t K, int32_t iters, float* ms_out, void* stream);

#ifdef __cplusplus
}
#endif
#endif
```

Baseline: 38140.

## Fuse decoder LayerNorm, FSMN and next LayerNorm into one row-tiled kernel

Replaces the decoder's separate LayerNorm, FSMN memory block and following LayerNorm+fp16-plane split with a single kernel. Each wave handles an 8-row tile plus its 10-row halo, normalizes in registers, applies the depthwise conv with residual, then normalizes again and writes the split fp16 planes. This removes two launches and the intermediate global-memory round trips. The cost is recomputing LayerNorm on halo rows and high register pressure. Separately, the absmax reduction is vectorized to float4 with one atomic per block and a grid sized from the CU count.

```diff
diff --git a/funasr_amd/_lib.py b/funasr_amd/_lib.py
--- a/funasr_amd/_lib.py
+++ b/funasr_amd/_lib.py
@@ -150,6 +150,7 @@
     "pf_decoder_set_tensor": (C.c_int, [_vp, C.c_char_p, _vp, _i64]),
     "pf_decoder_missing": (C.c_int, [_vp]),
     "pf_decoder_set_precision": (C.c_int, [_vp, _i32]),
+    "pf_decoder_set_option": (C.c_int, [_vp, C.c_char_p, _i32]),
     "pf_decoder_forward": (C.c_int, [_vp, _vp, _pi32, _vp, _pi32, _i32, _i32, _i32, _vp, _vp, _vp, _vp]),
     "pf_decoder_create_contextual": (_vp, [C.POINTER(pf_decoder_config)]),
     "pf_decoder_forward_contextual": (C.c_int, [_vp, _vp, _pi32, _vp, _pi32, _vp, _i32, _f32, _i32, _i32, _i32, _vp, _vp, _vp, _vp]),
@@ -252,6 +253,9 @@
     "pf_k_gemm_argmax_f32": (C.c_int, [_vp, _i32, _vp, _i32, _vp, _i32, _i32, _i32, _vp, _vp, _vp, _vp]),
     "pf_k_log_softmax": (C.c_int, [_vp, _i32, _vp, _i32, _i32, _i32, _vp]),
     "pf_k_layernorm": (C.c_int, [_vp, _i32, _vp, _vp, _vp, _i32, _i32, _i32, _i32, _f32, _vp]),
+    "pf_k_ln_fsmn_ln": (C.c_int, [_vp, _i32, _vp, _vp, _vp, _vp, _i32, _vp, _i32, _vp, _vp, _vp, _i32, _i64, _f32, _vp, _vp, _i32, _i32, _i32,
+                                  _i32, _i32, _i32, _f32, _i32, C.POINTER(C.c_float), _vp]),
+    "pf_k_absmax": (C.c_int, [_vp, _i64, _vp, _vp]),
     "pf_k_fsmn": (C.c_int, [_vp, _i32, _vp, _vp, _i32, _vp, _i32, _vp, _i32, _i32, _i32, _i32, _i32, _vp]),
     "pf_k_attention_f32": (C.c_int, [_vp, _i32, _vp, _i32, _vp, _i32, _vp, _i32, _vp, _i32, _i32, _i32, _i32, _f32, _vp]),
     "pf_k_attention_f32_two_source": (C.c_int, [_vp, _i32, _vp, _i32, _vp, _i32, _vp, _i32, _vp, _i32, _vp, _i32, _vp, _i32,
diff --git a/funasr_amd/csrc/common.h b/funasr_amd/csrc/common.h
--- a/funasr_amd/csrc/common.h
+++ b/funasr_amd/csrc/common.h
@@ -340,6 +340,23 @@
 };
 int launch_fsmn(const FsmnArgs& a, hipStream_t stream);
 
+struct LnFsmnLnArgs {
+    const float* in;  int ldin;
+    const float* g2;  const float* b2;
+    const float* w;
+    const float* R;   int ldr;
+    float* out;       int ldo;
+    const float* g3;  const float* b3;
+    unsigned short* y2; int ldy; size_t y_plane; float yscale;
+    const int* lens;
+    const int* offs;
+    int B, T, C, K, left_pad;
+    int M;
+    float eps;
+};
+bool ln_fsmn_ln_applicable(int C, int K, int left_pad);
+int launch_ln_fsmn_ln(const LnFsmnLnArgs& a, hipStream_t stream);
+
 struct AttnArgs {
     const float* Q; int ldq;
     const float* K; int ldk;
diff --git a/funasr_amd/csrc/engine_decoder.hip b/funasr_amd/csrc/engine_decoder.hip
--- a/funasr_amd/csrc/engine_decoder.hip
+++ b/funasr_amd/csrc/engine_decoder.hip
@@ -690,6 +690,15 @@
                                 const int32_t* tok_lens, int32_t B, int32_t T, int32_t N, float* logits, int32_t* ids,
                                 float* hidden_out, hipStream_t s, int asf_layer, float* asf_scores, const DecCtxArgs* cx = nullptr);
 
+int pf_decoder_set_option(pf_decoder* dh, const char* key, int32_t value) {
+    Decoder* d = reinterpret_cast<Decoder*>(dh);
+    PF_REQUIRE(d && key, "decoder_set_option: null");
+    const std::string k(key);
+    if (k == "fuse_rows") { PF_REQUIRE(value == 0 || value == 1, "decoder_set_option: fuse_rows is 0 or 1"); d->fuse_rows = value; return 0; }
+    set_error("decoder_set_option: unknown key " + k);
+    return -1;
+}
+
 int pf_decoder_forward(pf_decoder* dh, const float* memory, const int32_t* mem_lens, const float* embeds,
                        const int32_t* tok_lens, int32_t B, int32_t T, int32_t N, float* logits, int32_t* ids,
                        float* hidden_out, void* stream) {
@@ -807,15 +816,26 @@
         if (x2) rc = dec_ffn_x2(d, w, x, t2, Mq, s);
         else rc = dec_ffn(d, w, x, t2, Mq, s, w1_3);
         if (rc) return rc;
-        if ((rc = layernorm(t2, D, w.n2g, w.n2b, t1, D, Mq, D, D, c.ln_eps, s))) return rc;
-        FsmnArgs fa{};
-        fa.in = t1; fa.ldin = D; fa.w = w.fsmn_w; fa.R = x; fa.ldr = D; fa.out = x; fa.ldo = D;
-        fa.lens = d->tok_lens.as<int>(); fa.B = B; fa.T = N; fa.C = D; fa.K = c.kernel_size; fa.left_pad = left_pad;
-        fa.offs = offs_dev;
-        if ((rc = fsmn(fa, s))) return rc;
+        const bool fused_rows = x2 && d->fuse_rows && ln_fsmn_ln_applicable(D, c.kernel_size, left_pad);
+        if (fused_rows) {
+            LnFsmnLnArgs la{};
+            la.in = t2; la.ldin = D; la.g2 = w.n2g; la.b2 = w.n2b; la.w = w.fsmn_w; la.R = x; la.ldr = D; la.out = x; la.ldo = D;
+            la.g3 = w.n3g; la.b3 = w.n3b; la.y2 = d->t16.as<unsigned short>(); la.ldy = D; la.y_plane = (size_t)Mq * D;
+            la.yscale = pow2f(w.e_n3); la.lens = d->tok_lens.as<int>(); la.offs = offs_dev; la.B = B; la.T = N; la.C = D;
+            la.K = c.kernel_size; la.left_pad = left_pad; la.M = Mq; la.eps = c.ln_eps;
+            ProfScope ps(PROF_LN, 16.0 * Mq * (double)D, s);
+            if ((rc = launch_ln_fsmn_ln(la, s))) return rc;
+        } else {
+            if ((rc = layernorm(t2, D, w.n2g, w.n2b, t1, D, Mq, D, D, c.ln_eps, s))) return rc;
+            FsmnArgs fa{};
+            fa.in = t1; fa.ldin = D; fa.w = w.fsmn_w; fa.R = x; fa.ldr = D; fa.out = x; fa.ldo = D;
+            fa.lens = d->tok_lens.as<int>(); fa.B = B; fa.T = N; fa.C = D; fa.K = c.kernel_size; fa.left_pad = left_pad;
+            fa.offs = offs_dev;
+            if ((rc = fsmn(fa, s))) return rc;
+        }
         if (x2) {
             unsigned short* t2p = d->t16.as<unsigned short>();
-            {
+            if (!fused_rows) {
                 ProfScope ps(PROF_LN, 8.0 * Mq * (double)D, s);
                 if ((rc = launch_layernorm(x, D, w.n3g, w.n3b, reinterpret_cast<float*>(t2p), D, Mq, D, D, c.ln_eps, s, 3, 0,
                                            (size_t)Mq * D, pow2f(w.e_n3)))) return rc;
diff --git a/funasr_amd/csrc/engine_internal.h b/funasr_amd/csrc/engine_internal.h
--- a/funasr_amd/csrc/engine_internal.h
+++ b/funasr_amd/csrc/engine_internal.h
@@ -458,6 +458,7 @@
     unsigned long long resolved_for = TensorTable::NOT_PREPARED, x2_for = TensorTable::NOT_PREPARED;
     DevBuf x, t1, t2, ffn, ffn2, q, kv, ctx, mem_lens, tok_lens, pval, pidx, hid;
     int precision = 0;
+    int fuse_rows = 1;
     DevBuf t16, ffn16, ffn2_16, q16, kv16, ctx16, mem16, hid16;
     DevBuf dsc;
     DevBuf dscl, dlb;
diff --git a/funasr_amd/csrc/engine_kernels.hip b/funasr_amd/csrc/engine_kernels.hip
--- a/funasr_amd/csrc/engine_kernels.hip
+++ b/funasr_amd/csrc/engine_kernels.hip
@@ -297,6 +297,22 @@
     fa.in = in; fa.ldin = ldin; fa.w = w; fa.R = R; fa.ldr = ldr; fa.out = out; fa.ldo = ldo; fa.lens = lens_dev;
     fa.B = B; fa.T = T; fa.C = C; fa.K = K; fa.left_pad = left_pad;
     return fsmn(fa, reinterpret_cast<hipStream_t>(stream));
+}
+int pf_k_ln_fsmn_ln(const float* in, int32_t ldin, const float* g2, const float* b2, const float* w, const float* R, int32_t ldr,
+                    float* out, int32_t ldo, const float* g3, const float* b3, void* y2, int32_t ldy, int64_t y_plane, float yscale,
+                    const int32_t* lens_dev, const int32_t* offs_dev, int32_t B, int32_t T, int32_t M, int32_t C, int32_t K,
+                    int32_t left_pad, float eps, int32_t iters, float* ms_out, void* stream) {
+    hipStream_t s = reinterpret_cast<hipStream_t>(stream);
+    LnFsmnLnArgs la{};
+    la.in = in; la.ldin = ldin; la.g2 = g2; la.b2 = b2; la.w = w; la.R = R; la.ldr = ldr; la.out = out; la.ldo = ldo;
+    la.g3 = g3; la.b3 = b3; la.y2 = reinterpret_cast<unsigned short*>(y2); la.ldy = ldy; la.y_plane = (size_t)y_plane; la.yscale = yscale;
+    la.lens = lens_dev; la.offs = offs_dev; la.B = B; la.T = T; la.C = C; la.K = K; la.left_pad = left_pad; la.M = M; la.eps = eps;
+    if (iters <= 0 || !ms_out) return launch_ln_fsmn_ln(la, s);
+    return time_launches([&] { return launch_ln_fsmn_ln(la, s); }, iters, ms_out, s);
+}
+int pf_k_absmax(const float* x, int64_t n, float* out_dev, void* stream) {
+    PF_REQUIRE(n > 0, "absmax: n > 0");
+    return launch_absmax(x, (size_t)n, out_dev, reinterpret_cast<hipStream_t>(stream));
 }
 int pf_k_attention_f32(const float* Q, int32_t ldq, const float* K, int32_t ldk, const float* V, int32_t ldv,
                        float* O, int32_t ldo, const int32_t* klens_dev, int32_t B, int32_t H, int32_t Tq, int32_t Tk,
diff --git a/funasr_amd/csrc/gemm_f16x2.hip b/funasr_amd/csrc/gemm_f16x2.hip
--- a/funasr_amd/csrc/gemm_f16x2.hip
+++ b/funasr_amd/csrc/gemm_f16x2.hip
@@ -310,10 +310,31 @@
 }
 
 __global__ __launch_bounds__(256) void absmax_kernel(const float* __restrict__ x, size_t n, unsigned* __restrict__ out) {
+    __shared__ float wmax[4];
+    size_t head = ((16 - ((uintptr_t)x & 15)) & 15) / sizeof(float);
+    if (head > n) head = n;
+    const size_t n4 = (n - head) / 4, tail0 = head + 4 * n4;
+    const float4* x4 = reinterpret_cast<const float4*>(x + head);
+    const size_t stride = (size_t)gridDim.x * 256;
     float m = 0.f;
-    for (size_t i = (size_t)blockIdx.x * 256 + threadIdx.x; i < n; i += (size_t)gridDim.x * 256) m = fmaxf(m, fabsf(x[i]));
+    auto fold = [&](const float4 v) { m = fmaxf(m, fmaxf(fmaxf(fabsf(v.x), fabsf(v.y)), fmaxf(fabsf(v.z), fabsf(v.w)))); };
+    size_t i = (size_t)blockIdx.x * 256 + threadIdx.x;
+    for (; i + 3 * stride < n4; i += 4 * stride) {
+        const float4 a = x4[i], b = x4[i + stride], c = x4[i + 2 * stride], d = x4[i + 3 * stride];
+        fold(a); fold(b); fold(c); fold(d);
+    }
+    for (; i < n4; i += stride) fold(x4[i]);
+    if (blockIdx.x == 0) {
+        if (threadIdx.x < head) m = fmaxf(m, fabsf(x[threadIdx.x]));
+        if (tail0 + threadIdx.x < n) m = fmaxf(m, fabsf(x[tail0 + threadIdx.x]));
+    }
     m = wave_max(m);
-    if ((threadIdx.x & 63) == 0) atomicMax(out, __builtin_bit_cast(unsigned, m));
+    if ((threadIdx.x & 63) == 0) wmax[threadIdx.x >> 6] = m;
+    __syncthreads();
+    if (threadIdx.x == 0) {
+        m = fmaxf(fmaxf(wmax[0], wmax[1]), fmaxf(wmax[2], wmax[3]));
+        atomicMax(out, __builtin_bit_cast(unsigned, m));
+    }
 }
 
 __global__ __launch_bounds__(256) void rowl1_bound_kernel(const float* __restrict__ W, int rows, int cols, int ld,
@@ -475,7 +496,9 @@
 
 int launch_absmax(const float* x, size_t n, float* out_dev, hipStream_t stream) {
     PF_HIP_TRY(hipMemsetAsync(out_dev, 0, sizeof(float), stream));
-    const unsigned blocks = (unsigned)((n + 255) / 256 < 2048 ? (n + 255) / 256 : 2048);
+    PF_REQUIRE(x && out_dev && ((uintptr_t)x & 3) == 0, "absmax: null / unaligned input");
+    const size_t want = (n * sizeof(float) + 16383) / 16384, cap = 2 * (size_t)device_cu_count();
+    const unsigned blocks = (unsigned)(want < cap ? want : cap);
     hipLaunchKernelGGL(absmax_kernel, dim3(blocks ? blocks : 1), dim3(256), 0, stream, x, n, reinterpret_cast<unsigned*>(out_dev));
     PF_HIP_TRY(hipGetLastError());
     return 0;
diff --git a/funasr_amd/csrc/rowwise.hip b/funasr_amd/csrc/rowwise.hip
--- a/funasr_amd/csrc/rowwise.hip
+++ b/funasr_amd/csrc/rowwise.hip
@@ -310,6 +310,172 @@
                 o.x = r.x + o.x; o.y = r.y + o.y; o.z = r.z + o.z; o.w = r.w + o.w;
             }
             *reinterpret_cast<float4*>(p.out + row * p.ldo + c4 * 4) = o;
+        }
+    }
+}
+
+constexpr int LFL_TT = 8;
+template <int N>
+__device__ __forceinline__ void ln_stats2_rows(const float4 (&v)[N][2], float eps, int lane, float (&mean)[N], float (&rstd)[N]) {
+    static_assert(N <= 64, "one lane per row");
+    float sv = 0.f;
+#pragma unroll
+    for (int i = 0; i < N; ++i) {
+        float s = 0.f;
+        s += ln_sum4(v[i][0]);
+        s += ln_sum4(v[i][1]);
+        s = wave_sum(s);
+        sv = lane == i ? s : sv;
+    }
+    const float mv = ln_mean(sv, 512);
+#pragma unroll
+    for (int i = 0; i < N; ++i) mean[i] = __builtin_bit_cast(float, __builtin_amdgcn_readlane(__builtin_bit_cast(int, mv), i));
+    float qv = 0.f;
+#pragma unroll
+    for (int i = 0; i < N; ++i) {
+        float q = 0.f;
+        q += ln_sqdev4(v[i][0], mean[i]);
+        q += ln_sqdev4(v[i][1], mean[i]);
+        q = wave_sum(q);
+        qv = lane == i ? q : qv;
+    }
+    const float rv = ln_rstd(qv, 512, eps);
+#pragma unroll
+    for (int i = 0; i < N; ++i) rstd[i] = __builtin_bit_cast(float, __builtin_amdgcn_readlane(__builtin_bit_cast(int, rv), i));
+}
+template <int KS, int LP>
+__global__ __launch_bounds__(256) void ln_fsmn_ln_kernel(LnFsmnLnArgs p) {
+    constexpr int TT = LFL_TT, NW = TT + KS - 1;
+    const int lane = threadIdx.x & 63;
+    const int slot = __builtin_amdgcn_readfirstlane(blockIdx.x * 4 + (threadIdx.x >> 6));
+    int b, t0;
+    if (p.offs) {
+        int cnt = 0;
+        for (int b0 = 0; b0 < p.B; b0 += 64) {
+            const int bb = b0 + lane;
+            const bool le = bb < p.B && p.offs[bb] / TT + bb <= slot;
+            cnt += __popcll(__ballot(le));
+        }
+        b = cnt - 1;
+        if (b < 0) return;
+        t0 = (slot - (p.offs[b] / TT + b)) * TT;
+    } else {
+        const int per = (p.T + TT - 1) / TT;
+        b = slot / per;
+        if (b >= p.B) return;
+        t0 = (slot - b * per) * TT;
+    }
+    const int len = p.lens[b];
+    const size_t base = p.offs ? (size_t)p.offs[b] : (size_t)b * p.T;
+    const int rows = p.offs ? p.offs[b + 1] - p.offs[b] : p.T;
+    if (t0 >= rows) return;
+    constexpr bool R_EARLY = TT <= 4;
+    float4 win[NW][2];
+#pragma unroll
+    for (int i = 0; i < NW; ++i) {
+        const int tt = t0 - LP + i, tc = tt < 0 ? 0 : (tt < rows ? tt : rows - 1);
+        const float* src = p.in + (base + tc) * p.ldin;
+        win[i][0] = *reinterpret_cast<const float4*>(src + 4 * lane);
+        win[i][1] = *reinterpret_cast<const float4*>(src + 4 * (lane + 64));
+    }
+    float4 xs[TT][2];
+    auto load_r = [&](const int j) {
+#pragma unroll
+        for (int i = 0; i < TT; ++i) {
+            const int t = t0 + i, tc = t < rows ? t : rows - 1;
+            xs[i][j] = *reinterpret_cast<const float4*>(p.R + (base + tc) * p.ldr + 4 * (lane + 64 * j));
+        }
+    };
+    float4 w[KS];
+    auto load_w = [&](const int j) {
+        float wf[4 * KS];
+        const float4* wp = reinterpret_cast<const float4*>(p.w + (size_t)(lane + 64 * j) * 4 * KS);
+#pragma unroll
+        for (int k = 0; k < KS; ++k) {
+            const float4 t = wp[k];
+            wf[4 * k] = t.x; wf[4 * k + 1] = t.y; wf[4 * k + 2] = t.z; wf[4 * k + 3] = t.w;
+        }
+#pragma unroll
+        for (int k = 0; k < KS; ++k) w[k] = make_float4(wf[k], wf[KS + k], wf[2 * KS + k], wf[3 * KS + k]);
+    };
+    load_r(0);
+    if (R_EARLY) load_r(1);
+    {
+        float4 g[2], be[2];
+#pragma unroll
+        for (int j = 0; j < 2; ++j) {
+            g[j] = *reinterpret_cast<const float4*>(p.g2 + 4 * (lane + 64 * j));
+            be[j] = *reinterpret_cast<const float4*>(p.b2 + 4 * (lane + 64 * j));
+        }
+        float mean[NW], rstd[NW];
+        ln_stats2_rows<NW>(win, p.eps, lane, mean, rstd);
+        load_w(0);
+#pragma unroll
+        for (int i = 0; i < NW; ++i) {
+            const int tt = t0 - LP + i;
+            const bool valid = tt >= 0 && tt < p.T && tt < len;
+#pragma unroll
+            for (int j = 0; j < 2; ++j) {
+                const float4 n = ln_apply4(win[i][j], mean[i], rstd[i], g[j], be[j]);
+                win[i][j] = make_float4(valid ? n.x : 0.f, valid ? n.y : 0.f, valid ? n.z : 0.f, valid ? n.w : 0.f);
+            }
+        }
+    }
+#pragma unroll
+    for (int j = 0; j < 2; ++j) {
+        const int c = lane + 64 * j;
+        if (j == 1) {
+            if (!R_EARLY) load_r(1);
+            load_w(1);
+        }
+#pragma unroll
+        for (int i = 0; i < TT; ++i) {
+            const int t = t0 + i;
+            float4 acc = make_float4(0.f, 0.f, 0.f, 0.f);
+#pragma unroll
+            for (int k = 0; k < KS; ++k) {
+                acc.x = fmaf(w[k].x, win[i + k][j].x, acc.x);
+                acc.y = fmaf(w[k].y, win[i + k][j].y, acc.y);
+                acc.z = fmaf(w[k].z, win[i + k][j].z, acc.z);
+                acc.w = fmaf(w[k].w, win[i + k][j].w, acc.w);
+            }
+            const float4 ce = win[i + LP][j];
+            const bool in_len = t < len;
+            float4 o;
+            o.x = in_len ? acc.x + ce.x : 0.f; o.y = in_len ? acc.y + ce.y : 0.f;
+            o.z = in_len ? acc.z + ce.z : 0.f; o.w = in_len ? acc.w + ce.w : 0.f;
+            const float4 r = xs[i][j];
+            o.x = r.x + o.x; o.y = r.y + o.y; o.z = r.z + o.z; o.w = r.w + o.w;
+            xs[i][j] = o;
+            if (t < rows) *reinterpret_cast<float4*>(p.out + (base + t) * p.ldo + 4 * c) = o;
+        }
+    }
+    if (!p.g3) return;
+    float4 g[2], be[2];
+#pragma unroll
+    for (int j = 0; j < 2; ++j) {
+        g[j] = *reinterpret_cast<const float4*>(p.g3 + 4 * (lane + 64 * j));
+        be[j] = *reinterpret_cast<const float4*>(p.b3 + 4 * (lane + 64 * j));
+    }
+    float mean[TT], rstd[TT];
+    ln_stats2_rows<TT>(xs, p.eps, lane, mean, rstd);
+#pragma unroll
+    for (int i = 0; i < TT; ++i) {
+        const int t = t0 + i;
+        if (t < rows) {
+            unsigned short* yb = p.y2 + (base + t) * p.ldy;
+#pragma unroll
+            for (int j = 0; j < 2; ++j) {
+                const int c = lane + 64 * j;
+                const float4 o = ln_apply4(xs[i][j], mean[i], rstd[i], g[j], be[j]);
+                unsigned h0, l0, h1, l1;
+                split2_pk(o.x * p.yscale, o.y * p.yscale, h0, l0);
+                split2_pk(o.z * p.yscale, o.w * p.yscale, h1, l1);
+                const bool odd = (lane & 1) != 0;
+                const unsigned r0 = dpp_swap1(odd ? h0 : l0), r1 = dpp_swap1(odd ? h1 : l1);
+                *reinterpret_cast<uint4*>(odd ? yb + 4 * c - 4 + p.y_plane : yb + 4 * c) =
+                    odd ? make_uint4(r0, r1, l0, l1) : make_uint4(h0, h1, r0, r1);
+            }
         }
     }
 }
@@ -471,4 +637,23 @@
     return 0;
 }
 
-}
+bool ln_fsmn_ln_applicable(int C, int K, int left_pad) { return C == 512 && K == 11 && (left_pad == 5 || left_pad == 10); }
+
+int launch_ln_fsmn_ln(const LnFsmnLnArgs& a, hipStream_t stream) {
+    PF_REQUIRE(ln_fsmn_ln_applicable(a.C, a.K, a.left_pad), "ln_fsmn_ln: built for 512 columns, kernel_size 11, left padding 5 or 10");
+    PF_REQUIRE(a.in && a.g2 && a.b2 && a.w && a.R && a.out && a.lens && a.B > 0 && a.T > 0 && a.in != a.out, "ln_fsmn_ln: null / aliased input");
+    PF_REQUIRE(a.ldin % 4 == 0 && a.ldr % 4 == 0 && a.ldo % 4 == 0 && a.ldin >= a.C && a.ldr >= a.C && a.ldo >= a.C, "ln_fsmn_ln: strides % 4");
+    PF_REQUIRE((((uintptr_t)a.in | (uintptr_t)a.g2 | (uintptr_t)a.b2 | (uintptr_t)a.w | (uintptr_t)a.R | (uintptr_t)a.out) & 15) == 0,
+               "ln_fsmn_ln: operands must be 16-B aligned");
+    PF_REQUIRE(!a.g3 || (a.b3 && a.y2 && a.ldy % 8 == 0 && a.y_plane % 8 == 0 && a.ldy >= a.C && (((uintptr_t)a.g3 | (uintptr_t)a.b3 | (uintptr_t)a.y2) & 15) == 0),
+               "ln_fsmn_ln: plane output needs g3, b3, y2 16-B aligned, ldy % 8, y_plane % 8");
+    PF_REQUIRE(!a.offs || a.M > 0, "ln_fsmn_ln: packed layout needs its row count");
+    const int slots = a.offs ? a.M / LFL_TT + a.B : a.B * ceil_div(a.T, LFL_TT);
+    dim3 grid(ceil_div(slots, 4)), block(256);
+    if (a.left_pad == 5) hipLaunchKernelGGL((ln_fsmn_ln_kernel<11, 5>), grid, block, 0, stream, a);
+    else hipLaunchKernelGGL((ln_fsmn_ln_kernel<11, 10>), grid, block, 0, stream, a);
+    PF_HIP_TRY(hipGetLastError());
+    return 0;
+}
+
+}
diff --git a/funasr_amd/ops.py b/funasr_amd/ops.py
--- a/funasr_amd/ops.py
+++ b/funasr_amd/ops.py
@@ -489,6 +489,38 @@
     return (y, float(ms.value)) if time_iters > 0 else y
 
 
+LN_FSMN_LN_RUN = 8
+
+
+def ln_fsmn_ln(t2: torch.Tensor, g2, b2, w: torch.Tensor, lens: torch.Tensor, left_pad: int, residual: torch.Tensor, eps: float,
+               g3=None, b3=None, scale_exp: int = 0, T: int | None = None, offs: torch.Tensor | None = None, out=None,
+               time_iters: int = 0):
+    lib = _lib.load()
+    _f32c(t2, "t2")
+    M, D = t2.shape
+    B = lens.numel()
+    assert t2.stride(1) == 1 and residual.stride(1) == 1 and residual.shape == t2.shape
+    assert (offs is None) != (T is None) and (offs is not None or M == B * T)
+    w2 = w.reshape(D, -1).contiguous()
+    out = torch.empty(M, D, device=t2.device, dtype=torch.float32) if out is None else out
+    y = torch.empty(2, M, D, device=t2.device, dtype=torch.float16) if g3 is not None else None
+    ms = C.c_float(0)
+    _lib.check(lib.pf_k_ln_fsmn_ln(_ptr(t2), t2.stride(0), _ptr(g2), _ptr(b2), _ptr(w2), _ptr(residual), residual.stride(0), _ptr(out),
+                                   out.stride(0), _ptr(g3), _ptr(b3), _ptr(y), D, M * D, float(2.0 ** scale_exp), _ptr(lens), _ptr(offs),
+                                   B, T if T is not None else M, M, D, w2.shape[1], left_pad, float(eps), int(time_iters), C.byref(ms),
+                                   _stream()), "pf_k_ln_fsmn_ln")
+    return (out, y, float(ms.value)) if time_iters > 0 else (out, y)
+
+
+def absmax(x: torch.Tensor) -> torch.Tensor:
+    lib = _lib.load()
+    _f32c(x, "x")
+    assert x.is_contiguous()
+    out = torch.empty(1, device=x.device, dtype=torch.float32)
+    _lib.check(lib.pf_k_absmax(_ptr(x), x.numel(), _ptr(out), _stream()), "pf_k_absmax")
+    return out
+
+
 def vt_columns(m: torch.Tensor) -> torch.Tensor:
     return (m & ~12) | ((m & 4) << 1) | ((m & 8) >> 1)
 
diff --git a/funasr_amd/paraformer_decoder.py b/funasr_amd/paraformer_decoder.py
--- a/funasr_amd/paraformer_decoder.py
+++ b/funasr_amd/paraformer_decoder.py
@@ -87,6 +87,12 @@
         self._precision = mode
         return self
 
+    def set_option(self, key: str, value: int):
+        if not hasattr(self, "_options"):
+            self._options = {}
+        self._options[str(key)] = int(value)
+        return self
+
     def _make_config(self):
         return _lib.pf_decoder_config(self.vocab_size if self.output_layer is not None else 0, self.d_model, self.attention_heads, self.linear_units,
                                       self.att_layer_num, self.kernel_size, self.sanm_shfit, 1e-12)
@@ -99,6 +105,8 @@
         lib, h = self._ensure_handle()
         _lib.check(lib.pf_decoder_set_precision(h, {"fp32": 0, "bf16": 1, "bf16x3": 2, "f16x2": 3}[self._mode()]),
                    "pf_decoder_set_precision")
+        for key, value in getattr(self, "_options", {}).items():
+            _lib.check(lib.pf_decoder_set_option(h, key.encode(), int(value)), "pf_decoder_set_option")
         return lib, h
 
     def _run(self, hs_pad, hlens, ys_in_pad, ys_in_lens, want_logits: bool, want_ids: bool, want_hidden: bool = False):
diff --git a/include/paraformer_hip.h b/include/paraformer_hip.h
--- a/include/paraformer_hip.h
+++ b/include/paraformer_hip.h
@@ -134,6 +134,7 @@
 int pf_decoder_set_tensor(pf_decoder* d, const char* name, const float* data, int64_t numel);
 int pf_decoder_missing(const pf_decoder* d);
 int pf_decoder_set_precision(pf_decoder* d, int32_t mode);
+int pf_decoder_set_option(pf_decoder* d, const char* key, int32_t value);
 int pf_decoder_forward(pf_decoder* d, const float* memory_dev, const int32_t* mem_lens_host,
                        const float* embeds_dev, const int32_t* tok_lens_host, int32_t B, int32_t T, int32_t N,
                        float* logits_dev, int32_t* ids_dev, float* hidden_dev, void* stream);
@@ -387,6 +388,11 @@
                    int32_t M, int32_t D, int32_t Dpad, float eps, void* stream);
 int pf_k_fsmn(const float* in, int32_t ldin, const float* w, const float* R, int32_t ldr, float* out, int32_t ldo,
               const int32_t* lens_dev, int32_t B, int32_t T, int32_t C, int32_t K, int32_t left_pad, void* stream);
+int pf_k_ln_fsmn_ln(const float* in, int32_t ldin, const float* g2, const float* b2, const float* w, const float* R, int32_t ldr,
+                    float* out, int32_t ldo, const float* g3, const float* b3, void* y2, int32_t ldy, int64_t y_plane, float yscale,
+                    const int32_t* lens_dev, const int32_t* offs_dev, int32_t B, int32_t T, int32_t M, int32_t C, int32_t K,
+                    int32_t left_pad, float eps, int32_t iters, float* ms_out, void* stream);
+int pf_k_absmax(const float* x, int64_t n, float* out_dev, void* stream);
 int pf_k_attention_f32(const float* Q, int32_t ldq, const float* K, int32_t ldk, const float* V, int32_t ldv,
                        float* O, int32_t ldo, const int32_t* klens_dev, int32_t B, int32_t H, int32_t Tq,
                        int32_t Tk, float scale, void* stream);
```

Result: no change. 38140 (-0.0%).
